# QWTforGithub/CDSegNet

Measured on AMD Instinct MI355X. Metric: points/sec/node (ScanNet ~120k-pt scenes, 1-step), higher is better.
Workload: dtype f16

## Files before the change

### cdsegnet_amd/_lib.py

```python
import ctypes
import os
import threading
from ctypes import POINTER, Structure, c_char_p, c_float, c_int, c_int32, c_int64, c_long, c_size_t, c_uint64, c_void_p

HERE = os.path.dirname(os.path.abspath(__file__))
LIB_PATH = os.path.join(HERE, "libcdseg_hip.so")
LIB_PATH_F16 = os.path.join(HERE, "libcdseg_hip_f16.so")

F32, BF16 = 0, 1
ACT_NONE, ACT_GELU, ACT_SWISH = 0, 1, 2
ORDER_IDS = {"z": 0, "z-trans": 1, "hilbert": 2, "hilbert-trans": 3}
ERRORS = {-1: "CDSEG_ERR_ARG", -2: "CDSEG_ERR_LAUNCH", -3: "CDSEG_ERR_WORKSPACE", -4: "CDSEG_ERR_UNSUPPORTED"}


class CdsegError(RuntimeError):
    pass


class DuplicateVoxelsError(CdsegError):

    def __init__(self, msg, count):
        super().__init__(msg)
        self.count = int(count)


class GemmArgs(Structure):
    _fields_ = [
        ("A", c_void_p), ("W", c_void_p), ("bias", c_void_p), ("scale", c_void_p), ("shift", c_void_p),
        ("res", c_void_p), ("add_src", c_void_p), ("add_idx", c_void_p), ("nbr", c_void_p), ("out_idx", c_void_p),
        ("out", c_void_p), ("out2", c_void_p),
        ("M", c_long),
        ("N", c_int), ("K", c_int), ("kvol", c_int),
        ("lda", c_int), ("ldo", c_int), ("ldo2", c_int), ("ldres", c_int), ("ldadd", c_int),
        ("a_dtype", c_int), ("compute_dtype", c_int), ("out_dtype", c_int), ("out2_dtype", c_int),
        ("act", c_int), ("out2_pre_add", c_int),
        ("ws", c_void_p), ("ws_bytes", c_size_t),
        ("colbias", c_void_p), ("ln_pre_g", c_void_p), ("ln_pre_b", c_void_p), ("ln_post_g", c_void_p),
        ("ln_post_b", c_void_p), ("ln_out", c_void_p), ("ldln", c_int), ("ln_out_dtype", c_int), ("ln_eps", c_float),
        ("nbr_kmajor", c_int),
    ]


class BlockDesc(Structure):
    _fields_ = [
        ("dtype", c_int), ("channels", c_int), ("heads", c_int), ("hidden", c_int),
        ("attn_scale", c_float), ("ln_eps", c_float),
        ("cpe_conv_w", c_void_p), ("cpe_conv_b", c_void_p), ("cpe_lin_w", c_void_p), ("cpe_lin_b", c_void_p),
        ("cpe_ln_g", c_void_p), ("cpe_ln_b", c_void_p), ("norm1_g", c_void_p), ("norm1_b", c_void_p),
        ("qkv_w", c_void_p), ("qkv_b", c_void_p), ("proj_w", c_void_p), ("proj_b", c_void_p),
        ("norm2_g", c_void_p), ("norm2_b", c_void_p), ("fc1_w", c_void_p), ("fc1_b", c_void_p),
        ("fc2_w", c_void_p), ("fc2_b", c_void_p), ("cpe_conv_wimg", c_void_p),
        ("head_img", c_void_p), ("tail_img", c_void_p),
        ("attn_flags", c_int),
    ]


class BlockIO(Structure):
    _fields_ = [
        ("n", c_long), ("x", c_void_p), ("xc_in", c_void_p), ("xc_out", c_void_p), ("tbias", c_void_p),
        ("nbr", c_void_p), ("gidx", c_void_p), ("widx", c_void_p), ("patch_start", c_void_p),
        ("num_patches", c_int), ("max_len", c_int), ("scratch", c_void_p), ("scratch_bytes", c_size_t),
        ("sat_counter", c_void_p),
    ]


class TrainBlockDesc(Structure):
    _fields_ = [
        ("channels", c_int), ("heads", c_int), ("hidden", c_int),
        ("attn_scale", c_float), ("eps_cpe", c_float), ("eps_norm1", c_float), ("eps_norm2", c_float),
        ("mm_dtype", c_int), ("attn_dtype", c_int), ("deterministic", c_int),
        ("param", c_void_p * 18), ("shadow16", c_void_p * 6),
        ("derived", c_void_p), ("derived_bytes", c_size_t),
    ]


class TrainBlockIO(Structure):
    _fields_ = [
        ("n", c_long), ("x_in", c_void_p), ("x_conv", c_void_p), ("t_rows", c_void_p), ("scene_offs", c_void_p),
        ("num_scenes", c_int), ("mask1", c_void_p), ("mask2", c_void_p),
        ("nbr", c_void_p), ("gidx", c_void_p), ("widx", c_void_p), ("patch_start", c_void_p),
        ("num_patches", c_int), ("max_len", c_int), ("num_slots", c_long),
        ("tape", c_void_p), ("tape_bytes", c_size_t), ("scratch", c_void_p), ("scratch_bytes", c_size_t),
        ("x_out", c_void_p),
        ("n_conv", c_long), ("row_vox", c_void_p), ("row_start", c_void_p),
    ]


class PlanSpec(Structure):
    _fields_ = [
        ("nlev", c_int), ("cum", c_int * 9), ("ncurve", c_int), ("curve_rows", c_int * 3),
        ("nslot_curve", c_int), ("slot_curve", c_int * 4),
        ("nlink", c_int), ("link_a", c_int * 16), ("link_b", c_int * 16),
        ("npad", c_int), ("pad_patch", c_int * 4), ("pad_flash", c_int * 4),
    ]


class PlanBeginIO(Structure):
    _fields_ = [
        ("grid", c_void_p), ("grid_elem_bytes", c_int), ("offset", c_void_p), ("nb", c_int), ("n", c_long),
        ("depth", c_int), ("end_bit", c_int), ("i32", c_void_p), ("i64", c_void_p), ("ws", c_void_p),
        ("ws_bytes", c_size_t), ("gmax_host", c_void_p), ("meta_host", c_void_p),
    ]


class PlanFinishIO(Structure):
    _fields_ = [
        ("n", c_long), ("nb", c_int), ("depth", c_int), ("m_host", POINTER(c_long)), ("offs_host", POINTER(c_int)),
        ("grid0", c_void_p), ("bat0", c_void_p), ("code0", c_void_p), ("cluster", c_void_p), ("seg", c_void_p),
        ("orders0", c_void_p), ("i32", c_void_p), ("i64", c_void_p), ("ws", c_void_p), ("ws_bytes", c_size_t),
        ("pads_host", c_void_p),
    ]


class OptTensor(Structure):
    _fields_ = [("p", c_void_p), ("g", c_void_p), ("m", c_void_p), ("v", c_void_p), ("p16", c_void_p), ("step", c_void_p),
                ("n", c_long), ("group", c_int), ("flags", c_int)]


class OptGroup(Structure):
    _fields_ = [("lr", ctypes.c_double), ("beta1", ctypes.c_double), ("beta2", ctypes.c_double), ("eps", ctypes.c_double),
                ("weight_decay", ctypes.c_double)]


OPT_CLIP, OPT_SKIP = 1, 2

SIGNATURES = {
    "cdseg_abi_version": (c_int, []),
    "cdseg_build_info": (c_char_p, []),
    "cdseg_grid_max": (c_int, [c_void_p, c_int, c_long, c_void_p, c_void_p]),
    "cdseg_offset2batch": (c_int, [c_void_p, c_int, c_long, c_void_p, c_void_p]),
    "cdseg_encode": (c_int, [c_void_p, c_int, c_void_p, c_int, c_long, c_int, c_int, c_void_p, c_void_p]),
    "cdseg_encode4": (c_int, [c_void_p, c_void_p, c_long, c_int, c_void_p, c_void_p]),
    "cdseg_sort_ws_bytes": (c_size_t, [c_long]),
    "cdseg_sort_pairs": (c_int, [c_void_p, c_void_p, c_void_p, c_void_p, c_long, c_int, c_void_p, c_size_t, c_void_p]),
    "cdseg_sort_curves_ws_bytes": (c_size_t, [c_long, c_int]),
    "cdseg_sort_curves": (c_int, [c_void_p, POINTER(c_int), c_int, c_long, c_int, c_void_p, c_void_p, c_size_t, c_void_p]),
    "cdseg_invert_perm": (c_int, [c_void_p, c_long, c_void_p, c_void_p]),
    "cdseg_widen_i32": (c_int, [c_void_p, c_long, c_void_p, c_void_p]),
    "cdseg_gather_rows": (c_int, [c_void_p, c_void_p, c_long, c_int, c_void_p, c_void_p]),
    "cdseg_scatter_rows": (c_int, [c_void_p, c_void_p, c_long, c_int, c_void_p, c_void_p]),
    "cdseg_gather_i32": (c_int, [c_void_p, c_void_p, c_long, c_void_p, c_void_p]),
    "cdseg_plan_gather_grid": (c_int, [c_void_p, c_int, c_void_p, c_void_p, c_long, c_int, c_void_p, c_void_p, c_void_p]),
    "cdseg_pool_level": (c_int, [c_void_p, c_long, c_int, c_void_p, c_void_p, c_void_p, c_void_p, c_size_t, c_void_p]),
    "cdseg_pool_gather": (c_int, [c_void_p, c_long, c_long, c_int, c_void_p, c_void_p, c_void_p, c_void_p, c_void_p,
                                  c_void_p, c_void_p]),
    "cdseg_pool_levels_ws_bytes": (c_size_t, [c_long, c_int]),
    "cdseg_pool_levels": (c_int, [c_void_p, c_long, POINTER(c_int), c_int, c_void_p, c_int, c_void_p, c_void_p, c_void_p,
                                  c_void_p, c_size_t, c_void_p]),
    "cdseg_link_derive": (c_int, [c_void_p, c_void_p, c_long, c_void_p, c_void_p, c_long, c_void_p, c_void_p, c_void_p]),
    "cdseg_coarse_orders_ws_bytes": (c_size_t, [c_long, c_int, c_int]),
    "cdseg_coarse_orders": (c_int, [POINTER(c_void_p), c_int, POINTER(c_void_p), c_int, c_long, c_void_p, c_void_p,
                                    c_size_t, c_void_p]),
    "cdseg_nbr_table": (c_int, [c_void_p, c_void_p, c_void_p, c_long, c_int, c_int, c_int, c_void_p, c_void_p]),
    "cdseg_nbr_table_from_parent": (c_int, [c_void_p, c_void_p, c_void_p, c_void_p, c_void_p, c_long, c_long, c_int, c_int,
                                            c_int, c_void_p, c_void_p]),
    "cdseg_nbr_table_from_info": (c_int, [c_void_p, c_void_p, c_void_p, c_void_p, c_long, c_long, c_int, c_int, c_int, c_void_p,
                                          c_void_p]),
    "cdseg_pad_plan": (c_int, [c_void_p, c_void_p, c_void_p, c_int, c_int, c_long, c_void_p, c_void_p, c_void_p]),
    "cdseg_pad_plan_batch": (c_int, [c_int, POINTER(c_void_p), POINTER(c_void_p), POINTER(c_void_p), POINTER(c_int),
                                     POINTER(c_long), c_int, c_void_p, c_void_p, c_void_p]),
    "cdseg_slots_select": (c_int, [POINTER(c_void_p), POINTER(c_void_p), c_int, c_void_p, c_int, c_char_p, c_long, c_void_p,
                                   c_void_p, c_void_p]),
    "cdseg_plan_begin_layout": (c_int, [POINTER(PlanSpec), c_long, c_int, POINTER(c_long), POINTER(c_long)]),
    "cdseg_plan_begin": (c_int, [POINTER(PlanSpec), POINTER(PlanBeginIO), c_int, c_void_p]),
    "cdseg_plan_finish_layout": (c_int, [POINTER(PlanSpec), c_long, c_int, POINTER(c_long), POINTER(c_int), POINTER(c_long),
                                         POINTER(c_long)]),
    "cdseg_plan_finish": (c_int, [POINTER(PlanSpec), POINTER(PlanFinishIO), c_void_p]),
    "cdseg_voxelize": (c_int, [c_void_p, ctypes.c_double, c_long, c_void_p, c_void_p, c_void_p, c_void_p]),
    "cdseg_voxelize_f64": (c_int, [c_void_p, ctypes.c_double, c_long, c_void_p, c_void_p, c_void_p, c_void_p]),
    "cdseg_center_shift": (c_int, [c_void_p, c_int, c_long, c_int, c_void_p, c_void_p, c_void_p]),
    "cdseg_tta_apply": (c_int, [c_void_p, c_long, POINTER(ctypes.c_double), ctypes.c_double, c_int, c_int, c_void_p, c_void_p]),
    "cdseg_div_add": (c_int, [c_void_p, c_float, c_float, c_long, c_void_p, c_void_p]),
    "cdseg_collect_feat": (c_int, [c_void_p, c_int, c_void_p, c_int, c_int, c_long, c_void_p, c_void_p]),
    "cdseg_max_run": (c_int, [c_void_p, c_long, c_void_p, c_void_p]),
    "cdseg_fragment_select": (c_int, [c_void_p, c_void_p, c_long, c_int, c_void_p, c_void_p]),
    "cdseg_softmax_vote": (c_int, [c_void_p, c_int, c_void_p, c_long, c_int, c_void_p, c_int, c_void_p]),
    "cdseg_argmax_rows": (c_int, [c_void_p, c_int, c_long, c_int, c_void_p, c_void_p]),
    "cdseg_fragments_build_ws_bytes": (c_size_t, [c_int]),
    "cdseg_fragments_build": (c_int, [c_void_p, c_void_p, c_long, c_int, c_long, c_void_p, c_void_p, c_int, c_void_p, c_int, c_int,
                                      c_void_p, c_void_p, c_void_p, c_void_p, c_void_p, c_size_t, c_void_p]),
    "cdseg_softmax_vote_fragments": (c_int, [c_void_p, c_int, c_void_p, c_long, c_int, c_int, c_void_p, c_int, c_long, c_void_p]),
    "cdseg_voxel_inverse": (c_int, [c_void_p, c_void_p, c_long, c_void_p, c_void_p]),
    "cdseg_tt_bbox": (c_int, [c_void_p, c_int, c_long, c_void_p, c_void_p]),
    "cdseg_tt_affine": (c_int, [c_void_p, c_int, c_long, c_int, POINTER(ctypes.c_double), c_void_p, POINTER(ctypes.c_double), c_int,
                                ctypes.c_double, c_int, c_int, c_int, c_void_p, c_int, c_void_p]),
    "cdseg_tt_jitter": (c_int, [c_void_p, c_void_p, c_int, ctypes.c_double, ctypes.c_double, c_long, c_void_p]),
    "cdseg_tt_blur3": (c_int, [c_void_p, c_int, c_int, c_int, c_int, c_void_p, c_void_p]),
    "cdseg_tt_elastic": (c_int, [c_void_p, c_long, c_void_p, POINTER(c_int), POINTER(ctypes.c_double), POINTER(ctypes.c_double),
                                 POINTER(ctypes.c_double), ctypes.c_double, c_void_p]),
    "cdseg_tt_color": (c_int, [c_void_p, c_long, c_void_p, ctypes.c_double, c_int, POINTER(ctypes.c_double), c_void_p, c_int,
                               ctypes.c_double, c_void_p]),
    "cdseg_tt_voxel_pick": (c_int, [c_void_p, c_void_p, c_long, c_void_p, c_void_p, c_void_p]),
    "cdseg_tt_dist_key": (c_int, [c_void_p, c_long, c_long, c_void_p, c_void_p]),
    "cdseg_rand_int": (c_int, [c_void_p, c_long, c_uint64, c_uint64, c_void_p, ctypes.c_uint32, c_void_p]),
    "cdseg_knn": (c_int, [c_void_p, c_void_p, c_long, c_void_p, c_void_p, c_long, c_int, c_int, POINTER(c_float), c_float,
                          c_void_p, c_void_p, c_void_p, c_size_t, c_void_p]),
    "cdseg_knn1_ws_bytes": (c_size_t, [c_long]),
    "cdseg_knn1": (c_int, [c_void_p, c_void_p, c_long, c_void_p, c_void_p, c_long, c_int, POINTER(c_float), c_float,
                           c_void_p, c_void_p, c_void_p, c_size_t, c_void_p]),
    "cdseg_iou_counts": (c_int, [c_void_p, c_void_p, c_void_p, c_long, c_int, c_int, c_void_p, c_void_p]),
    "cdseg_gemm": (c_int, [POINTER(GemmArgs), c_void_p]),
    "cdseg_gemm_ws_bytes": (c_size_t, [c_long, c_int, c_int, c_int]),
    "cdseg_mlp_fused": (c_int, [c_void_p, c_int, c_void_p, c_void_p, c_void_p, c_void_p, c_void_p, c_int, c_void_p, c_int,
                                c_long, c_int, c_int, c_void_p]),
    "cdseg_attn_tail_fused": (c_int, [c_void_p, c_int, c_void_p, c_void_p, c_void_p, c_void_p, c_float, c_void_p, c_void_p,
                                      c_void_p, c_void_p, c_void_p, c_int, c_void_p, c_int, c_long, c_int, c_int, c_void_p]),
    "cdseg_cpe_head_fused": (c_int, [c_void_p, c_int, c_void_p, c_void_p, c_void_p, c_void_p, c_void_p, c_int, c_void_p,
                                     c_void_p, c_void_p, c_float, c_void_p, c_void_p, c_void_p, c_int, c_long, c_int, c_int,
                                     c_int, c_void_p]),
    "cdseg_subm_conv3_wimg_bytes": (c_size_t, [c_int]),
    "cdseg_subm_conv3_pack": (c_int, [c_void_p, c_int, c_void_p, c_void_p]),
    "cdseg_subm_conv3": (c_int, [c_void_p, c_int, c_void_p, c_void_p, c_void_p, c_long, c_int, c_void_p, c_int, c_void_p]),
    "cdseg_child_info": (c_int, [c_void_p, c_void_p, c_long, c_void_p, c_void_p]),
    "cdseg_stem5_wimg_bytes": (c_size_t, []),
    "cdseg_stem5_pack": (c_int, [c_void_p, c_void_p, c_void_p]),
    "cdseg_stem5": (c_int, [c_void_p, c_void_p, c_void_p, c_void_p, c_void_p, c_void_p, c_void_p, c_void_p, c_long, c_long,
                            c_int, c_void_p, c_void_p, c_void_p]),
    "cdseg_block_rr_img_bytes": (c_size_t, [c_int, c_int]),
    "cdseg_block_rr_pack": (c_int, [c_int, c_void_p, c_void_p, c_void_p, c_void_p, c_void_p, c_void_p, c_void_p, c_void_p]),
    "cdseg_cpe_head_rr": (c_int, [c_void_p, c_int, c_void_p, c_void_p, c_void_p, c_void_p, c_void_p, c_int, c_void_p, c_void_p,
                                  c_void_p, c_float, c_void_p, c_void_p, c_int, c_long, c_int, c_int, c_void_p]),
    "cdseg_attn_tail_rr": (c_int, [c_void_p, c_int, c_void_p, c_void_p, c_void_p, c_void_p, c_float, c_void_p, c_void_p,
                                   c_void_p, c_int, c_void_p, c_int, c_long, c_int, c_void_p]),
    "cdseg_cpe_head_rr2": (c_int, [c_void_p, c_int, c_void_p, c_void_p, c_void_p, c_void_p, c_void_p, c_int, c_void_p, c_int,
                                   c_void_p, c_void_p, c_void_p, c_float, c_void_p, c_void_p, c_int, c_long, c_int, c_int, c_void_p]),
    "cdseg_attn_tail_rr2": (c_int, [c_void_p, c_int, c_void_p, c_void_p, c_void_p, c_void_p, c_float, c_void_p, c_void_p,
                                    c_void_p, c_int, c_void_p, c_int, c_void_p, c_int, c_long, c_int, c_void_p, c_size_t, c_void_p]),
    "cdseg_block_scratch_bytes": (c_size_t, [POINTER(BlockDesc), c_long]),
    "cdseg_block_forward": (c_int, [POINTER(BlockDesc), POINTER(BlockIO), c_void_p]),
    "cdseg_layernorm": (c_int, [c_void_p, c_int, c_int, c_void_p, c_void_p, c_float, c_void_p, c_int, c_void_p,
                                c_void_p, c_int, c_int, c_void_p, c_int, c_int, c_long, c_int, c_void_p]),
    "cdseg_attention": (c_int, [c_void_p, c_void_p, c_void_p, c_int, c_int, c_int, c_void_p, c_void_p, c_void_p,
                                c_void_p, c_int, c_int, c_int, c_float, c_void_p, c_int, c_int, c_void_p]),
    "cdseg_attention_ex": (c_int, [c_void_p, c_void_p, c_void_p, c_int, c_int, c_int, c_void_p, c_void_p, c_void_p,
                                   c_void_p, c_int, c_int, c_int, c_float, c_void_p, c_int, c_int, c_int, c_void_p]),
    "cdseg_attention_schedule": (c_long, [c_int, c_int, c_int, c_int, c_void_p, c_long]),
    "cdseg_attention_bwd_ws_bytes": (c_size_t, [c_long, c_int]),
    "cdseg_attention_bwd": (c_int, [c_void_p, c_void_p, c_void_p, c_int, c_int, c_int, c_void_p, c_void_p, c_void_p, c_void_p,
                                    c_int, c_int, c_long, c_int, c_float, c_void_p, c_int, c_void_p, c_void_p, c_void_p,
                                    c_int, c_int, c_int, c_int, c_void_p, c_size_t, c_void_p]),
    "cdseg_attention_drop": (c_int, [c_void_p, c_void_p, c_void_p, c_int, c_int, c_int, c_void_p, c_void_p, c_void_p, c_void_p,
                                     c_int, c_int, c_int, c_float, c_void_p, c_int, c_int, ctypes.c_double, c_uint64, c_uint64,
                                     c_void_p]),
    "cdseg_attention_drop_bwd": (c_int, [c_void_p, c_void_p, c_void_p, c_int, c_int, c_int, c_void_p, c_void_p, c_void_p, c_void_p,
                                         c_int, c_int, c_long, c_int, c_float, c_void_p, c_int, c_void_p, c_void_p, c_void_p,
                                         c_int, c_int, c_int, c_int, c_void_p, c_size_t, ctypes.c_double, c_uint64, c_uint64,
                                         c_void_p]),
    "cdseg_dropout": (c_int, [c_void_p, c_int, c_void_p, c_int, c_long, c_int, ctypes.c_double, c_uint64, c_uint64, c_void_p]),
    "cdseg_layernorm_bwd": (c_int, [c_void_p, c_int, c_void_p, c_float, c_void_p, c_int, c_void_p, c_int, c_int, c_void_p,
                                    c_void_p, c_long, c_int, c_void_p]),
    "cdseg_gelu_bwd": (c_int, [c_void_p, c_void_p, c_void_p, c_long, c_void_p]),
    "cdseg_conv_wgrad": (c_int, [c_void_p, c_int, c_void_p, c_int, c_void_p, c_int, c_long, c_int, c_int, c_void_p, c_void_p,
                                 c_void_p]),
    "cdseg_linear_wgrad": (c_int, [c_void_p, c_int, c_void_p, c_void_p, c_int, c_long, c_int, c_int, c_void_p, c_int, c_void_p,
                                   c_void_p]),
    "cdseg_conv_wgrad16": (c_int, [c_void_p, c_int, c_void_p, c_int, c_void_p, c_int, c_long, c_int, c_int, c_void_p, c_void_p,
                                   c_void_p]),
    "cdseg_linear_wgrad16": (c_int, [c_void_p, c_int, c_void_p, c_void_p, c_int, c_long, c_int, c_int, c_void_p, c_int, c_void_p,
                                     c_void_p]),
    "cdseg_wgrad_partition": (c_int, [c_long, c_int, c_int, c_int, c_int, POINTER(c_long), POINTER(c_int)]),
    "cdseg_wgrad_det_ws_bytes": (c_size_t, [c_long, c_int, c_int, c_int, c_int]),
    "cdseg_linear_wgrad_det": (c_int, [c_void_p, c_int, c_void_p, c_void_p, c_int, c_long, c_int, c_int, c_void_p, c_int, c_void_p,
                                       c_int, c_void_p, c_size_t, c_void_p]),
    "cdseg_conv_wgrad_det": (c_int, [c_void_p, c_int, c_void_p, c_int, c_void_p, c_int, c_long, c_int, c_int, c_void_p, c_void_p,
                                     c_int, c_void_p, c_size_t, c_void_p]),
    "cdseg_layernorm_bwd_det_ws_bytes": (c_size_t, [c_long, c_int]),
    "cdseg_layernorm_bwd_det": (c_int, [c_void_p, c_int, c_void_p, c_float, c_void_p, c_int, c_void_p, c_int, c_int, c_void_p,
                                        c_void_p, c_long, c_int, c_void_p, c_size_t, c_void_p]),
    "cdseg_segment_sum": (c_int, [c_void_p, c_int, c_void_p, c_long, c_int, c_void_p, c_int, c_void_p]),
    "cdseg_seg_loss_ws_bytes": (c_size_t, [c_long, c_int]),
    "cdseg_seg_loss_fwd": (c_int, [c_void_p, c_int, c_void_p, c_long, c_int, c_long, c_int, c_void_p, POINTER(c_int32), c_void_p,
                                   c_void_p, c_void_p, c_size_t, c_void_p]),
    "cdseg_seg_loss_bwd": (c_int, [c_void_p, c_int, c_void_p, c_long, c_int, c_long, POINTER(c_int32), c_void_p, c_void_p,
                                   c_void_p, c_void_p, c_int, c_void_p]),
    "cdseg_bn_partition": (c_int, [c_long, c_int, POINTER(c_long), POINTER(c_int)]),
    "cdseg_bn_ws_bytes": (c_size_t, [c_long, c_int]),
    "cdseg_bn_stats": (c_int, [c_void_p, c_int, c_long, c_int, c_void_p, c_void_p, c_size_t, c_void_p]),
    "cdseg_bn_finish": (c_int, [c_void_p, c_int, ctypes.c_double, ctypes.c_double, c_void_p, c_void_p, c_void_p, c_void_p,
                                c_void_p]),
    "cdseg_bn_gelu_fwd": (c_int, [c_void_p, c_int, c_long, c_int, c_void_p, c_void_p, c_void_p, c_void_p, c_void_p, c_int,
                                  c_void_p]),
    "cdseg_bn_gelu_bwd_sums": (c_int, [c_void_p, c_int, c_void_p, c_int, c_long, c_int, c_void_p, c_void_p, c_void_p, c_void_p,
                                       c_void_p, c_void_p, c_size_t, c_void_p]),
    "cdseg_bn_gelu_bwd_dx": (c_int, [c_void_p, c_int, c_void_p, c_int, c_long, c_int, c_void_p, c_void_p, c_void_p, c_void_p,
                                     c_void_p, c_void_p, c_void_p, c_int, c_void_p]),
    "cdseg_segment_max_arg": (c_int, [c_void_p, c_int, c_void_p, c_long, c_int, c_void_p, c_int, c_void_p, c_int, c_void_p]),
    "cdseg_segment_max_bwd": (c_int, [c_void_p, c_int, c_void_p, c_int, c_void_p, c_long, c_int, c_void_p, c_int, c_void_p]),
    "cdseg_fuse_gate_ws_bytes": (c_size_t, [c_long, c_int]),
    "cdseg_fuse_gate_fwd": (c_int, [c_void_p, c_void_p, c_void_p, c_void_p, c_void_p, c_void_p, c_long, c_int, c_void_p]),
    "cdseg_fuse_gate_bwd": (c_int, [c_void_p, c_void_p, c_void_p, c_void_p, c_void_p, c_void_p, c_void_p, c_void_p, c_void_p,
                                    c_long, c_int, c_void_p, c_size_t, c_void_p]),
    "cdseg_skip_partition": (c_int, [c_long, c_int, POINTER(c_long), POINTER(c_int)]),
    "cdseg_skip_stats_ws_bytes": (c_size_t, [c_long, c_int]),
    "cdseg_skip_stats": (c_int, [c_void_p, c_int, c_int, c_long, c_int, c_void_p, c_long, c_void_p, c_void_p, c_size_t, c_void_p]),
    "cdseg_skip_fold": (c_int, [c_void_p, c_int, c_int, c_int, c_int, c_void_p, c_void_p, c_void_p]),
    "cdseg_skip_merge": (c_int, [c_void_p, c_int, c_long, c_int, c_void_p, c_int, ctypes.c_double, c_long, ctypes.c_double,
                                 c_void_p, c_void_p, c_int, c_void_p, c_long, c_void_p]),
    "cdseg_opt_chunks": (c_int, [POINTER(c_long), c_int, POINTER(c_int32), POINTER(c_long)]),
    "cdseg_opt_ws_bytes": (c_size_t, [c_int, c_long]),
    "cdseg_grad_norm": (c_int, [POINTER(OptTensor), c_int, c_void_p, c_long, c_void_p, c_float, c_void_p, c_void_p, c_size_t,
                                c_void_p]),
    "cdseg_adamw_step": (c_int, [POINTER(OptTensor), c_int, POINTER(OptGroup), c_int, c_void_p, c_long, c_void_p, c_void_p,
                                 c_void_p, c_void_p, c_size_t, c_void_p]),
    "cdseg_route_enable": (c_int, [c_int]),
    "cdseg_route_clear": (None, []),
    "cdseg_route_read": (c_int, [POINTER(c_int32), c_int]),
    "cdseg_route_catalog": (c_int, [ctypes.c_char_p, c_size_t]),
    "cdseg_route_note": (c_int, [POINTER(c_int32)]),
    "cdseg_prof_enable": (c_int, [c_int]),
    "cdseg_prof_summary": (c_int, [POINTER(ctypes.c_double), POINTER(c_long)]),
    "cdseg_prof_summary_class": (c_int, [c_int, POINTER(ctypes.c_double), POINTER(c_long)]),
    "cdseg_segment_max": (c_int, [c_void_p, c_int, c_int, c_void_p, c_long, c_int, c_void_p, c_void_p, c_int,
                                  c_void_p, c_int, c_void_p, c_int, c_int, c_void_p]),
    "cdseg_segment_mean": (c_int, [c_void_p, c_int, c_void_p, c_long, c_int, c_void_p, c_int, c_void_p]),
    "cdseg_pool_fused_fold": (c_int, [c_int]),
    "cdseg_pool_fused_n": (c_int, [c_void_p, c_int, c_long, c_void_p, c_void_p, c_void_p, c_long, c_void_p, c_void_p, c_int, c_void_p,
                                   c_int, c_void_p, c_int, c_int, c_int, c_void_p]),
    "cdseg_unpool_fused_img_bytes": (c_size_t, [c_int, c_int]),
    "cdseg_unpool_fused_pack": (c_int, [c_void_p, c_int, c_int, c_void_p, c_void_p]),
    "cdseg_unpool_fused": (c_int, [c_void_p, c_int, c_void_p, c_void_p, c_void_p, c_void_p, c_void_p, c_int, c_void_p, c_void_p,
                                   c_void_p, c_void_p, c_void_p, c_long, c_int, c_void_p, c_int, c_void_p, c_int, c_int, c_int,
                                   c_int, c_void_p]),
    "cdseg_pool_fused_img_bytes": (c_size_t, [c_int, c_int]),
    "cdseg_pool_fused_pack": (c_int, [c_void_p, c_int, c_int, c_void_p, c_void_p]),
    "cdseg_pool_fused": (c_int, [c_void_p, c_int, c_void_p, c_void_p, c_void_p, c_long, c_void_p, c_void_p, c_int, c_void_p, c_int,
                                 c_void_p, c_int, c_int, c_int, c_void_p]),
    "cdseg_gemv": (c_int, [c_void_p, c_void_p, c_void_p, c_int, c_int, c_int, c_void_p, c_void_p]),
    "cdseg_randn": (c_int, [c_void_p, c_long, c_uint64, c_uint64, c_void_p]),
    "cdseg_cast": (c_int, [c_void_p, c_int, c_void_p, c_int, c_long, c_void_p]),
    "cdseg_gather_pad_cast": (c_int, [c_void_p, c_int, c_void_p, c_long, c_int, c_int, c_void_p, c_int, c_void_p]),
    "cdseg_ddim_update": (c_int, [c_void_p, c_void_p, c_float, c_float, c_float, c_float, c_int, c_void_p, c_long,
                                  c_void_p]),
    "cdseg_axpy": (c_int, [c_void_p, c_void_p, c_float, c_void_p, c_long, c_void_p]),
    "cdseg_msi_step": (c_int, [c_void_p, c_void_p, c_long, c_float, c_float, c_float, c_float, c_int, c_void_p, c_void_p, c_long,
                               c_int, c_float, c_void_p]),
    "cdseg_count_saturated": (c_int, [c_void_p, c_long, c_int, c_int, c_void_p, c_void_p]),
    "cdseg_subm_conv3_f32": (c_int, [c_void_p, c_int, c_void_p, c_void_p, c_void_p, c_long, c_int, c_void_p, c_int, c_float, c_int,
                                     c_void_p]),
    "cdseg_split16": (c_int, [c_void_p, c_int, c_long, c_int, c_void_p, c_void_p, c_int, c_float, c_void_p]),
    "cdseg_train_block_bytes": (c_int, [POINTER(TrainBlockDesc), c_long, c_long, POINTER(c_size_t), POINTER(c_size_t),
                                        POINTER(c_size_t), POINTER(c_size_t)]),
    "cdseg_train_block_grad_offsets": (c_int, [POINTER(TrainBlockDesc), POINTER(c_size_t)]),
    "cdseg_train_block_prepare": (c_int, [POINTER(TrainBlockDesc), c_void_p]),
    "cdseg_train_block_forward": (c_int, [POINTER(TrainBlockDesc), POINTER(TrainBlockIO), c_void_p]),
    "cdseg_train_block_backward": (c_int, [POINTER(TrainBlockDesc), POINTER(TrainBlockIO), c_void_p, c_void_p, c_void_p, c_void_p,
                                           c_void_p, c_void_p]),
    "cdseg_residual": (c_int, [c_void_p, c_void_p, c_void_p, c_void_p, c_void_p, c_int, c_void_p, c_long, c_int, c_void_p]),
    "cdseg_gather_first": (c_int, [c_void_p, c_void_p, c_void_p, c_int, c_long, c_int, c_void_p]),
    "cdseg_residual_rows": (c_int, [c_void_p, c_void_p, c_void_p, c_void_p, c_void_p, c_int, c_void_p, c_long, c_int, c_void_p]),
    "cdseg_run_sum": (c_int, [c_void_p, c_void_p, c_void_p, c_long, c_int, c_void_p]),
    "cdseg_scatter_first": (c_int, [c_void_p, c_void_p, c_void_p, c_void_p, c_int, c_long, c_int, c_void_p]),
    "cdseg_scale_cast": (c_int, [c_void_p, c_void_p, c_void_p, c_int, c_long, c_int, c_void_p]),
    "cdseg_add_layernorm": (c_int, [c_void_p, c_void_p, c_void_p, c_void_p, c_void_p, c_float, c_void_p, c_void_p, c_int, c_long,
                                    c_int, c_void_p]),
    "cdseg_gelu_fwd": (c_int, [c_void_p, c_void_p, c_int, c_long, c_void_p]),
    "cdseg_gelu_bwd_cast": (c_int, [c_void_p, c_void_p, c_void_p, c_int, c_long, c_void_p]),
}

_libs = {}
_tls = threading.local()
VARIANTS = ("bf16", "f16")


def active():
    return getattr(_tls, "variant", "bf16")


class use:

    def __init__(self, variant):
        if variant not in VARIANTS:
            raise ValueError(variant)
        self.variant = variant

    def __enter__(self):
        self.prev = active()
# ... 37 lines not shown
```

### cdsegnet_amd/build.py

```python
import os
import subprocess
import sys

HERE = os.path.dirname(os.path.abspath(__file__))
CSRC = os.path.join(HERE, "csrc")
LIB = os.path.join(HERE, "libcdseg_hip.so")
LIB_F16 = os.path.join(HERE, "libcdseg_hip_f16.so")
VARIANTS = [(LIB, "_build", []), (LIB_F16, "_build_f16", ["-DCDSEG_LP_F16"])]
SOURCES = ["serialize.hip", "plan.hip", "gemm.hip", "elementwise.hip", "attention.hip", "attention_drop.hip", "conv.hip", "stem.hip", "mlp.hip", "blockrr.hip", "deep.hip", "pool.hip", "runtime.hip", "testtime.hip", "traintime.hip", "train.hip", "trainblock.hip", "loss.hip", "norm.hip", "fusion.hip", "skip.hip", "optim.hip", "prof.hip", "route.hip", "abi.hip"]
HEADERS = ["common.h", "curves.h", "prof.h", "route.h", "deep.h", "wgrad_partition.h", "workspace.h", "attn_train.h", os.path.join("..", "..", "include", "cdseg.h")]
ARCH = "gfx950"


def _stale():
    deps = [os.path.join(CSRC, f) for f in SOURCES + HEADERS] + [os.path.abspath(__file__)]
    for lib, _, _ in VARIANTS:
        if not os.path.exists(lib):
            return True
        t = os.path.getmtime(lib)
        if any(os.path.getmtime(d) > t for d in deps):
            return True
    return False


def build_library(force=False, verbose=True):
    if not force and not _stale():
        return LIB
    hipcc = os.environ.get("HIPCC", "/opt/rocm/bin/hipcc")
    procs, links = [], []
    for lib, bdir, defs in VARIANTS:
        build_dir = os.path.join(HERE, "csrc", bdir)
        os.makedirs(build_dir, exist_ok=True)
        objs = []
        for src in SOURCES:
            obj = os.path.join(build_dir, src.replace(".hip", ".o"))
            objs.append(obj)
            cmd = [hipcc, f"--offload-arch={ARCH}", "-O3", "-std=c++20", "-fPIC"] + defs + ["-c", os.path.join(CSRC, src), "-o", obj]
            if verbose:
                print(" ".join(cmd), flush=True)
            procs.append((src, subprocess.Popen(cmd, stdout=subprocess.PIPE, stderr=subprocess.STDOUT, text=True)))
        links.append([hipcc, f"--offload-arch={ARCH}", "-shared", "-fPIC", "-o", lib] + objs)
    for src, p in procs:
        out, _ = p.communicate()
        if p.returncode != 0:
            sys.stderr.write(out)
            raise RuntimeError(f"hipcc failed on {src}")
    for cmd in links:
        if verbose:
            print(" ".join(cmd), flush=True)
        subprocess.check_call(cmd)
    return LIB


if __name__ == "__main__":
    print(build_library(force="--force" in sys.argv))
```

### cdsegnet_amd/csrc/blockrr.hip

```cpp
#include <cstdlib>

#include <atomic>

#include "common.h"
#include "deep.h"
#include "route.h"

namespace {

constexpr int RR_WAVES = 8;

enum { OUT_P = 0, OUT_NAT = 1 };
enum { IN_P = 0, IN_HID = 1 };

struct PackP {
  const bf16_t* w;
  uint4* img;
  int nout, k, out_mode, in_mode;
};

__global__ void rr_pack_kernel(PackP p) {
  const int KS = p.k / 32;
  const int u = blockIdx.x * blockDim.x + threadIdx.x;
  if (u >= (p.nout / 16) * KS * 64) return;
  const int lane = u & 63, s = (u >> 6) % KS, ot = (u >> 6) / KS;
  const int q = lane >> 4, i = lane & 15;
  const int row = p.out_mode == OUT_P ? (i >> 2) * (p.nout / 4) + ot * 4 + (i & 3) : 16 * ot + i;
  union { uint4 v; bf16_t h[8]; } o;
#pragma unroll
  for (int e = 0; e < 8; ++e) {
    const int col = p.in_mode == IN_P ? q * (p.k / 4) + 8 * s + e : 32 * s + (e < 4 ? 4 * q + e : 16 + 4 * q + (e - 4));
    o.h[e] = p.w[(long)row * p.k + col];
  }
  p.img[u] = o.v;
}

template <int C>
struct RRCfg {
  static constexpr int KS = C / 32, CT = C / 16, Q = C / 4;
  static constexpr int HEAD_W = 4 * C * C * 2, HEAD_P = 9 * C * 4;
  static constexpr int TAIL_W = 9 * C * C * 2, TAIL_P = 8 * C * 4;
};

__device__ __forceinline__ bf16x8_t pack8(const f32x4_t& a, const f32x4_t& b) {
  union { bf16x8_t v; uint32_t u[4]; } r;
  r.u[0] = pack_bf16x2(a[0], a[1]); r.u[1] = pack_bf16x2(a[2], a[3]);
  r.u[2] = pack_bf16x2(b[0], b[1]); r.u[3] = pack_bf16x2(b[2], b[3]);
  return r.v;
}

template <int CT>
__device__ __forceinline__ void ln_stats(const f32x4_t (&v)[CT], float inv_c, float eps, float& mean, float& rstd) {
  float s = 0.f;
#pragma unroll
  for (int t = 0; t < CT; ++t) s += (v[t][0] + v[t][1]) + (v[t][2] + v[t][3]);
  s += __shfl_xor(s, 16, 64);
  s += __shfl_xor(s, 32, 64);
  mean = s * inv_c;
  float q = 0.f;
#pragma unroll
  for (int t = 0; t < CT; ++t) {
    const float a = v[t][0] - mean, b = v[t][1] - mean, c = v[t][2] - mean, d = v[t][3] - mean;
    q += (a * a + b * b) + (c * c + d * d);
  }
  q += __shfl_xor(q, 16, 64);
  q += __shfl_xor(q, 32, 64);
  rstd = 1.0f / sqrtf(q * inv_c + eps);
}

struct HeadRR {
  const bf16_t* y; const uint4* wimg; const float* bl; const float* lnp_g; const float* lnp_b; float* x;
  const float* colbias; const float* ln1_g; const float* ln1_b; const float* bqkv; bf16_t* qkv;
  long n; int ldy, ldx, ldqkv; float eps;
};

template <int C>
__global__ __launch_bounds__(RR_WAVES * 64, 4) void head_rr_kernel(HeadRR p) {
  using K = RRCfg<C>;
  constexpr int KS = K::KS, CT = K::CT, Q = K::Q, OT = 3 * C / 16, QQ = 3 * C / 4;
  extern __shared__ __attribute__((aligned(16))) char smem[];
  const int tid = threadIdx.x, lane0 = tid & 63;
  const int wave = __builtin_amdgcn_readfirstlane(tid >> 6);
  const int j = lane0 & 15, q = lane0 >> 4;
  {
    uint4* d = reinterpret_cast<uint4*>(smem);
    for (int u = tid; u < K::HEAD_W / 16; u += RR_WAVES * 64) d[u] = p.wimg[u];
    float* pr = reinterpret_cast<float*>(smem + K::HEAD_W);
    for (int c = tid; c < C; c += RR_WAVES * 64) {
      pr[c] = p.bl[c]; pr[C + c] = p.lnp_g[c]; pr[2 * C + c] = p.lnp_b[c]; pr[3 * C + c] = p.colbias ? p.colbias[c] : 0.f;
      pr[4 * C + c] = p.ln1_g[c]; pr[5 * C + c] = p.ln1_b[c];
    }
    for (int c = tid; c < 3 * C; c += RR_WAVES * 64) pr[6 * C + c] = p.bqkv[c];
  }
  __syncthreads();
  const uint4* Wl = reinterpret_cast<const uint4*>(smem);
  const uint4* Wq = reinterpret_cast<const uint4*>(smem + C * C * 2);
  const float* pr = reinterpret_cast<const float*>(smem + K::HEAD_W);
  const float inv_c = 1.0f / C;

  const long tiles = (p.n + 31) / 32;
  for (long tile = (long)blockIdx.x * RR_WAVES + wave; tile < tiles; tile += (long)gridDim.x * RR_WAVES) {
#pragma unroll 1
    for (int g = 0; g < 2; ++g) {
      const long row = tile * 32 + g * 16 + j;
      const bool ok = row < p.n;
      const long rr = ok ? row : p.n - 1;
      int lane = lane0;
      asm volatile("" : "+v"(lane));
      bf16x8_t yf[KS];
#pragma unroll
      for (int s = 0; s < KS; ++s) yf[s] = *reinterpret_cast<const bf16x8_t*>(p.y + rr * p.ldy + q * Q + 8 * s);
      f32x4_t xr[CT];
#pragma unroll
      for (int t = 0; t < CT; ++t) xr[t] = *reinterpret_cast<const f32x4_t*>(p.x + rr * p.ldx + q * Q + 4 * t);
      f32x4_t v[CT];
      {
        uint4 wl[CT][KS];
#pragma unroll
        for (int t = 0; t < CT; ++t)
#pragma unroll
          for (int s = 0; s < KS; ++s) wl[t][s] = Wl[(t * KS + s) * 64 + lane];
#pragma unroll
        for (int t = 0; t < CT; ++t) {
          v[t] = *reinterpret_cast<const f32x4_t*>(pr + q * Q + 4 * t);
#pragma unroll
          for (int s = 0; s < KS; ++s)
            v[t] = mfma_16x16x32_bf16(__builtin_bit_cast(bf16x8_t, wl[t][s]), yf[s], v[t]);
        }
      }
      float mean, rstd;
      ln_stats<CT>(v, inv_c, p.eps, mean, rstd);
#pragma unroll
      for (int t = 0; t < CT; ++t) {
        const f32x4_t ga = *reinterpret_cast<const f32x4_t*>(pr + C + q * Q + 4 * t);
        const f32x4_t be = *reinterpret_cast<const f32x4_t*>(pr + 2 * C + q * Q + 4 * t);
        const f32x4_t tb = *reinterpret_cast<const f32x4_t*>(pr + 3 * C + q * Q + 4 * t);
#pragma unroll
        for (int r = 0; r < 4; ++r) v[t][r] = ((v[t][r] - mean) * rstd * ga[r] + be[r]) + xr[t][r] + tb[r];
        if (ok) *reinterpret_cast<f32x4_t*>(p.x + row * p.ldx + q * Q + 4 * t) = v[t];
      }
      ln_stats<CT>(v, inv_c, p.eps, mean, rstd);
#pragma unroll
      for (int t = 0; t < CT; ++t) {
        const f32x4_t ga = *reinterpret_cast<const f32x4_t*>(pr + 4 * C + q * Q + 4 * t);
        const f32x4_t be = *reinterpret_cast<const f32x4_t*>(pr + 5 * C + q * Q + 4 * t);
#pragma unroll
        for (int r = 0; r < 4; ++r) v[t][r] = (v[t][r] - mean) * rstd * ga[r] + be[r];
      }
      bf16x8_t hf[KS];
#pragma unroll
      for (int s = 0; s < KS; ++s) hf[s] = pack8(v[2 * s], v[2 * s + 1]);
      uint4 wq[2][2][KS];
#pragma unroll
      for (int s = 0; s < KS; ++s) {
        wq[0][0][s] = Wq[(0 * KS + s) * 64 + lane];
        wq[0][1][s] = Wq[(1 * KS + s) * 64 + lane];
      }
#pragma unroll
      for (int ot = 0; ot < OT; ot += 2) {
        const int cur = (ot >> 1) & 1;
        if (ot + 2 < OT) {
#pragma unroll
          for (int s = 0; s < KS; ++s) {
            wq[cur ^ 1][0][s] = Wq[((ot + 2) * KS + s) * 64 + lane];
            wq[cur ^ 1][1][s] = Wq[((ot + 3) * KS + s) * 64 + lane];
          }
        }
        f32x4_t a0 = *reinterpret_cast<const f32x4_t*>(pr + 6 * C + q * QQ + 4 * ot);
        f32x4_t a1 = *reinterpret_cast<const f32x4_t*>(pr + 6 * C + q * QQ + 4 * ot + 4);
#pragma unroll
        for (int s = 0; s < KS; ++s) {
          a0 = mfma_16x16x32_bf16(__builtin_bit_cast(bf16x8_t, wq[cur][0][s]), hf[s], a0);
          a1 = mfma_16x16x32_bf16(__builtin_bit_cast(bf16x8_t, wq[cur][1][s]), hf[s], a1);
        }
        if (ok) *reinterpret_cast<bf16x8_t*>(p.qkv + row * p.ldqkv + q * QQ + 4 * ot) = pack8(a0, a1);
      }
    }
  }
}

struct TailRR {
  const bf16_t* o; const uint4* wimg; const float* bp; const float* ln_g; const float* ln_b; const float* b1;
  const float* b2; float* x; bf16_t* xc;
  long n; int ldo, ldx, ldxc; float eps;
};

template <int C>
__global__ __launch_bounds__(RR_WAVES * 64, 4) void tail_rr_kernel(TailRR p) {
  using K = RRCfg<C>;
  constexpr int KS = K::KS, CT = K::CT, Q = K::Q, HU = 4 * C / 32;
  extern __shared__ __attribute__((aligned(16))) char smem[];
  const int tid = threadIdx.x, lane0 = tid & 63;
  const int wave = __builtin_amdgcn_readfirstlane(tid >> 6);
  const int j = lane0 & 15, q = lane0 >> 4;
  {
    uint4* d = reinterpret_cast<uint4*>(smem);
    for (int u = tid; u < K::TAIL_W / 16; u += RR_WAVES * 64) d[u] = p.wimg[u];
    float* pr = reinterpret_cast<float*>(smem + K::TAIL_W);
    for (int c = tid; c < C; c += RR_WAVES * 64) {
      pr[c] = p.bp[c]; pr[C + c] = p.ln_g[c]; pr[2 * C + c] = p.ln_b[c]; pr[3 * C + c] = p.b2[c];
    }
    for (int c = tid; c < 4 * C; c += RR_WAVES * 64) pr[4 * C + c] = p.b1[c];
  }
  __syncthreads();
  const uint4* Wp = reinterpret_cast<const uint4*>(smem);
  const uint4* W1 = reinterpret_cast<const uint4*>(smem + C * C * 2);
  const uint4* W2 = reinterpret_cast<const uint4*>(smem + 5 * C * C * 2);
  const float* pr = reinterpret_cast<const float*>(smem + K::TAIL_W);
  const float inv_c = 1.0f / C;

  const long tiles = (p.n + 31) / 32;
  for (long tile = (long)blockIdx.x * RR_WAVES + wave; tile < tiles; tile += (long)gridDim.x * RR_WAVES) {
#pragma unroll 1
    for (int g = 0; g < 2; ++g) {
      const long row = tile * 32 + g * 16 + j;
      const bool ok = row < p.n;
      const long rr = ok ? row : p.n - 1;
      int lane = lane0;
      asm volatile("" : "+v"(lane));
      bf16x8_t of[KS];
#pragma unroll
      for (int s = 0; s < KS; ++s) of[s] = *reinterpret_cast<const bf16x8_t*>(p.o + rr * p.ldo + q * Q + 8 * s);
      f32x4_t x1[CT];
      {
        uint4 wp[CT][KS];
#pragma unroll
        for (int t = 0; t < CT; ++t)
#pragma unroll
          for (int s = 0; s < KS; ++s) wp[t][s] = Wp[(t * KS + s) * 64 + lane];
#pragma unroll
        for (int t = 0; t < CT; ++t) {
          f32x4_t a = *reinterpret_cast<const f32x4_t*>(pr + q * Q + 4 * t);
#pragma unroll
          for (int s = 0; s < KS; ++s)
            a = mfma_16x16x32_bf16(__builtin_bit_cast(bf16x8_t, wp[t][s]), of[s], a);
          const f32x4_t r = *reinterpret_cast<const f32x4_t*>(p.x + rr * p.ldx + q * Q + 4 * t);
          x1[t] = a + r;
        }
      }
      float mean, rstd;
      ln_stats<CT>(x1, inv_c, p.eps, mean, rstd);
      bf16x8_t hf[KS];
      {
        f32x4_t h[CT];
#pragma unroll
        for (int t = 0; t < CT; ++t) {
          const f32x4_t ga = *reinterpret_cast<const f32x4_t*>(pr + C + q * Q + 4 * t);
          const f32x4_t be = *reinterpret_cast<const f32x4_t*>(pr + 2 * C + q * Q + 4 * t);
#pragma unroll
          for (int r = 0; r < 4; ++r) h[t][r] = (x1[t][r] - mean) * rstd * ga[r] + be[r];
        }
#pragma unroll
        for (int s = 0; s < KS; ++s) hf[s] = pack8(h[2 * s], h[2 * s + 1]);
      }
      f32x4_t acc2[CT];
#pragma unroll
      for (int t = 0; t < CT; ++t) acc2[t] = f32x4_t{0.f, 0.f, 0.f, 0.f};
#pragma unroll 1
      for (int u = 0; u < HU; ++u) {
        uint4 w1[2][KS], w2[CT];
#pragma unroll
        for (int s = 0; s < KS; ++s) {
          w1[0][s] = W1[((2 * u) * KS + s) * 64 + lane];
          w1[1][s] = W1[((2 * u + 1) * KS + s) * 64 + lane];
        }
#pragma unroll
        for (int t = 0; t < CT; ++t) w2[t] = W2[(t * HU + u) * 64 + lane];
        f32x4_t h0 = *reinterpret_cast<const f32x4_t*>(pr + 4 * C + 32 * u + 4 * q);
        f32x4_t h1 = *reinterpret_cast<const f32x4_t*>(pr + 4 * C + 32 * u + 16 + 4 * q);
#pragma unroll
        for (int s = 0; s < KS; ++s) {
          h0 = mfma_16x16x32_bf16(__builtin_bit_cast(bf16x8_t, w1[0][s]), hf[s], h0);
          h1 = mfma_16x16x32_bf16(__builtin_bit_cast(bf16x8_t, w1[1][s]), hf[s], h1);
        }
        gelu_lp4(h0);
        gelu_lp4(h1);
        const bf16x8_t Hf = pack8(h0, h1);
#pragma unroll
        for (int t = 0; t < CT; ++t)
          acc2[t] = mfma_16x16x32_bf16(__builtin_bit_cast(bf16x8_t, w2[t]), Hf, acc2[t]);
      }
      if (ok) {
#pragma unroll
        for (int t = 0; t < CT; ++t) {
          const f32x4_t b2 = *reinterpret_cast<const f32x4_t*>(pr + 3 * C + q * Q + 4 * t);
          acc2[t] = acc2[t] + (b2 + x1[t]);
          *reinterpret_cast<f32x4_t*>(p.x + row * p.ldx + q * Q + 4 * t) = acc2[t];
        }
        if (p.xc) {
#pragma unroll
          for (int t = 0; t < CT; t += 2)
            *reinterpret_cast<bf16x8_t*>(p.xc + row * p.ldxc + q * Q + 4 * t) = pack8(acc2[t], acc2[t + 1]);
        }
      }
    }
  }
}

int pack_one(const void* w, int nout, int k, int out_mode, int in_mode, void* img, hipStream_t s) {
  PackP p;
  p.w = (const bf16_t*)w; p.img = (uint4*)img; p.nout = nout; p.k = k; p.out_mode = out_mode; p.in_mode = in_mode;
  const int units = (nout / 16) * (k / 32) * 64;
  hipLaunchKernelGGL(rr_pack_kernel, dim3((units + 255) / 256), dim3(256), 0, s, p);
  return hipGetLastError() == hipSuccess ? CDSEG_OK : CDSEG_ERR_LAUNCH;
}

int rr_grid(long n, int lds_bytes) {
  const long tiles = (n + 31) / 32;
  const int per_cu = lds_bytes > 80 * 1024 ? 1 : (lds_bytes > 40 * 1024 ? 2 : 3);
  long blocks = (tiles + RR_WAVES - 1) / RR_WAVES;
  if (blocks > 256 * per_cu) blocks = 256 * per_cu;
  return (int)blocks;
}

}

extern "C" size_t cdseg_block_rr_img_bytes(int channels, int which) {
  if (channels != 32 && channels != 64 && !deep_supported(channels)) return 0;
  return (size_t)(which == 0 ? 4 : 9) * channels * channels * 2;
}

extern "C" int cdseg_block_rr_pack(int channels, const void* wl, const void* wqkv, void* head_img, const void* wp,
                                   const void* w1, const void* w2, void* tail_img, void* stream) {
  if (deep_supported(channels)) return deep_pack(channels, wl, wqkv, head_img, wp, w1, w2, tail_img, (hipStream_t)stream);
  if (channels != 32 && channels != 64) return CDSEG_ERR_UNSUPPORTED;
  const int C = channels;
  hipStream_t s = (hipStream_t)stream;
  int rc;
  if (head_img) {
    if (!wl || !wqkv) return CDSEG_ERR_ARG;
    if ((rc = pack_one(wl, C, C, OUT_P, IN_P, head_img, s)) != CDSEG_OK) return rc;
    if ((rc = pack_one(wqkv, 3 * C, C, OUT_P, IN_P, (char*)head_img + C * C * 2, s)) != CDSEG_OK) return rc;
  }
  if (tail_img) {
    if (!wp || !w1 || !w2) return CDSEG_ERR_ARG;
    if ((rc = pack_one(wp, C, C, OUT_P, IN_P, tail_img, s)) != CDSEG_OK) return rc;
    if ((rc = pack_one(w1, 4 * C, C, OUT_NAT, IN_P, (char*)tail_img + C * C * 2, s)) != CDSEG_OK) return rc;
    if ((rc = pack_one(w2, C, 4 * C, OUT_P, IN_HID, (char*)tail_img + 5 * C * C * 2, s)) != CDSEG_OK) return rc;
  }
  return CDSEG_OK;
}

extern "C" int cdseg_cpe_head_rr(const void* y, int ldy, const void* head_img, const float* bl, const float* lnp_g,
                                 const float* lnp_b, float* x, int ldx, const float* colbias, const float* ln1_g,
                                 const float* ln1_b, float eps, const float* bqkv, void* qkv, int ldqkv, long n,
                                 int channels, int qkv_flags, void* stream) {
  if (n <= 0) return CDSEG_OK;
  if (qkv_flags & ~CDSEG_ATTN_V_BF16) return CDSEG_ERR_ARG;
  if (qkv_flags && !deep_supported(channels)) return CDSEG_ERR_UNSUPPORTED;
  if (!y || !head_img || !bl || !lnp_g || !lnp_b || !x || !ln1_g || !ln1_b || !bqkv || !qkv) return CDSEG_ERR_ARG;
  if (channels != 32 && channels != 64 && !deep_supported(channels)) return CDSEG_ERR_UNSUPPORTED;
  if ((ldy & 7) || (ldx & 3) || (ldqkv & 7) || (((uintptr_t)y | (uintptr_t)x | (uintptr_t)qkv | (uintptr_t)head_img) & 15))
    return CDSEG_ERR_ARG;
  if (deep_supported(channels))
    return deep_head(y, ldy, head_img, bl, lnp_g, lnp_b, x, ldx, x, ldx, colbias, ln1_g, ln1_b, eps, bqkv, qkv, ldqkv, n,
                     channels, qkv_flags, (hipStream_t)stream);
  HeadRR p;
  p.y = (const bf16_t*)y; p.wimg = (const uint4*)head_img; p.bl = bl; p.lnp_g = lnp_g; p.lnp_b = lnp_b; p.x = x;
  p.colbias = colbias; p.ln1_g = ln1_g; p.ln1_b = ln1_b; p.bqkv = bqkv; p.qkv = (bf16_t*)qkv;
  p.n = n; p.ldy = ldy; p.ldx = ldx; p.ldqkv = ldqkv; p.eps = eps;
  hipStream_t s = (hipStream_t)stream;
  if (channels == 32) {
    constexpr int lds = RRCfg<32>::HEAD_W + RRCfg<32>::HEAD_P;
    cdseg_route_rec(CDSEG_RK_HEAD_RR_32, 0, 0, 1, 0, 0, 0, 0);
    hipLaunchKernelGGL(head_rr_kernel<32>, dim3(rr_grid(n, lds)), dim3(RR_WAVES * 64), lds, s, p);
  } else {
    constexpr int lds = RRCfg<64>::HEAD_W + RRCfg<64>::HEAD_P;
    cdseg_route_rec(CDSEG_RK_HEAD_RR_64, 0, 0, 1, 0, 0, 0, 0);
    hipLaunchKernelGGL(head_rr_kernel<64>, dim3(rr_grid(n, lds)), dim3(RR_WAVES * 64), lds, s, p);
  }
  CDSEG_CHECK_LAUNCH();
  return CDSEG_OK;
}

extern "C" int cdseg_attn_tail_rr(const void* o, int ldo, const void* tail_img, const float* bp, const float* ln_g,
                                  const float* ln_b, float eps, const float* b1, const float* b2, float* x, int ldx,
                                  void* xc, int ldxc, long n, int channels, void* stream) {
  if (n <= 0) return CDSEG_OK;
  if (!o || !tail_img || !bp || !ln_g || !ln_b || !b1 || !b2 || !x) return CDSEG_ERR_ARG;
  if (channels != 32 && channels != 64 && !deep_supported(channels)) return CDSEG_ERR_UNSUPPORTED;
  if ((ldo & 7) || (ldx & 3) || (xc && (ldxc & 7)) || (((uintptr_t)o | (uintptr_t)x | (uintptr_t)xc | (uintptr_t)tail_img) & 15))
    return CDSEG_ERR_ARG;
  if (deep_supported(channels))
    return deep_tail(o, ldo, tail_img, bp, ln_g, ln_b, eps, b1, b2, x, ldx, x, ldx, xc, ldxc, n, channels, nullptr, 0,
                     (hipStream_t)stream);
  TailRR p;
  p.o = (const bf16_t*)o; p.wimg = (const uint4*)tail_img; p.bp = bp; p.ln_g = ln_g; p.ln_b = ln_b; p.b1 = b1; p.b2 = b2;
  p.x = x; p.xc = (bf16_t*)xc; p.n = n; p.ldo = ldo; p.ldx = ldx; p.ldxc = ldxc; p.eps = eps;
  hipStream_t s = (hipStream_t)stream;
  if (channels == 32) {
    constexpr int lds = RRCfg<32>::TAIL_W + RRCfg<32>::TAIL_P;
    cdseg_route_rec(CDSEG_RK_TAIL_RR_32, 0, 0, 1, 0, 0, 0, 0);
    hipLaunchKernelGGL(tail_rr_kernel<32>, dim3(rr_grid(n, lds)), dim3(RR_WAVES * 64), lds, s, p);
  } else {
    constexpr int lds = RRCfg<64>::TAIL_W + RRCfg<64>::TAIL_P;
    static std::atomic<bool> attr_done{false};
    if (!attr_done) {
      if (hipFuncSetAttribute((const void*)tail_rr_kernel<64>, hipFuncAttributeMaxDynamicSharedMemorySize, lds) != hipSuccess)
        return CDSEG_ERR_LAUNCH;
      attr_done = true;
    }
    cdseg_route_rec(CDSEG_RK_TAIL_RR_64, 0, 0, 1, 0, 0, 0, 0);
    hipLaunchKernelGGL(tail_rr_kernel<64>, dim3(rr_grid(n, lds)), dim3(RR_WAVES * 64), lds, s, p);
  }
  CDSEG_CHECK_LAUNCH();
  return CDSEG_OK;
}

extern "C" int cdseg_cpe_head_rr2(const void* y, int ldy, const void* head_img, const float* bl, const float* lnp_g,
                                  const float* lnp_b, const float* x, int ldx, float* x_out, int ldx_out, const float* colbias,
                                  const float* ln1_g, const float* ln1_b, float eps, const float* bqkv, void* qkv, int ldqkv,
                                  long n, int channels, int qkv_flags, void* stream) {
  if (n <= 0) return CDSEG_OK;
  if (qkv_flags & ~CDSEG_ATTN_V_BF16) return CDSEG_ERR_ARG;
  if (!deep_supported(channels)) return CDSEG_ERR_UNSUPPORTED;
  if (!y || !head_img || !bl || !lnp_g || !lnp_b || !x || !x_out || !ln1_g || !ln1_b || !bqkv || !qkv) return CDSEG_ERR_ARG;
  if ((ldy & 7) || (ldx & 3) || (ldx_out & 3) || (ldqkv & 7) ||
      (((uintptr_t)y | (uintptr_t)x | (uintptr_t)x_out | (uintptr_t)qkv | (uintptr_t)head_img) & 15))
    return CDSEG_ERR_ARG;
  return deep_head(y, ldy, head_img, bl, lnp_g, lnp_b, x, ldx, x_out, ldx_out, colbias, ln1_g, ln1_b, eps, bqkv, qkv, ldqkv, n,
                   channels, qkv_flags, (hipStream_t)stream);
}

extern "C" int cdseg_attn_tail_rr2(const void* o, int ldo, const void* tail_img, const float* bp, const float* ln_g,
                                   const float* ln_b, float eps, const float* b1, const float* b2, const float* x_in, int ldx_in,
                                   float* x, int ldx, void* xc, int ldxc, long n, int channels, void* ws, size_t ws_bytes,
                                   void* stream) {
  if (n <= 0) return CDSEG_OK;
  if (!deep_supported(channels)) return CDSEG_ERR_UNSUPPORTED;
  if (!o || !tail_img || !bp || !ln_g || !ln_b || !b1 || !b2 || !x || !x_in) return CDSEG_ERR_ARG;
  if ((ldo & 7) || (ldx & 3) || (ldx_in & 3) || (xc && (ldxc & 7)) ||
      (((uintptr_t)o | (uintptr_t)x | (uintptr_t)x_in | (uintptr_t)xc | (uintptr_t)tail_img) & 15))
    return CDSEG_ERR_ARG;
  return deep_tail(o, ldo, tail_img, bp, ln_g, ln_b, eps, b1, b2, x_in, ldx_in, x, ldx, xc, ldxc, n, channels, ws, ws_bytes,
                   (hipStream_t)stream);
}
```

### cdsegnet_amd/csrc/runtime.hip

```cpp
#include <algorithm>
#include <cstdlib>
#include <cstring>

#include "common.h"
#include "deep.h"
#include "workspace.h"

namespace {

constexpr int FUSE_LN_MAX_C = 512;

inline int storage_dtype(int dtype) { return dtype == CDSEG_F32X3 ? CDSEG_F32 : dtype; }

struct Layout {
  void *y, *h, *qkv, *o, *u, *y2, *ws, *xs;
  size_t ws_bytes, total;
};

Layout carve(const cdseg_block_desc* d, long n, void* scratch) {
  Carver c{(char*)scratch, 0};
  const size_t e = esz(d->dtype);
  const size_t C = d->channels;
  Layout L;
  L.y = c.take(n * C * e);
  L.h = c.take(n * C * e);
  L.qkv = c.take(n * 3 * C * e);
  L.o = c.take(n * C * e);
  L.u = c.take(n * (size_t)d->hidden * e);
  L.y2 = d->channels > FUSE_LN_MAX_C ? c.take(n * C * 4) : nullptr;
  const long wide = std::max<long>(3 * C, d->hidden);
  L.ws_bytes = std::min(GEMM_WS_CAP, std::max(gemm_ws_rule(n, C, wide, false, true), gemm_ws_rule(n, C, C, true, false)));
  L.ws = L.ws_bytes ? c.take(L.ws_bytes) : nullptr;
  L.xs = (d->dtype == CDSEG_BF16 && C >= 128 && d->head_img && d->tail_img) ? c.take(n * C * 4) : nullptr;
  L.total = align_up(c.off, 256);
  return L;
}

cdseg_gemm_args base_args(const cdseg_block_desc* d, const Layout& L, long n) {
  cdseg_gemm_args a;
  std::memset(&a, 0, sizeof(a));
  a.M = n;
  a.kvol = 1;
  a.a_dtype = storage_dtype(d->dtype);
  a.compute_dtype = d->dtype;
  a.ws = L.ws;
  a.ws_bytes = L.ws_bytes;
  a.ln_eps = d->ln_eps;
  return a;
}

}

extern "C" size_t cdseg_block_scratch_bytes(const cdseg_block_desc* d, long n) {
  if (!d || n <= 0) return 0;
  return carve(d, n, nullptr).total;
}

static int block_forward_impl(const cdseg_block_desc* d, const cdseg_block_io* io, void* stream);

extern "C" int cdseg_block_forward(const cdseg_block_desc* d, const cdseg_block_io* io, void* stream) {
  const int rc = block_forward_impl(d, io, stream);
  if (rc != CDSEG_OK || !io->sat_counter || io->n <= 0 || d->dtype != CDSEG_BF16) return rc;
  const Layout L = carve(d, io->n, io->scratch);
  const int C = d->channels;
  int r;
  if ((r = cdseg_count_saturated(L.y, io->n, C, C, io->sat_counter, stream)) != CDSEG_OK) return r;
  if ((r = cdseg_count_saturated(L.qkv, io->n, 2 * C, 3 * C, io->sat_counter, stream)) != CDSEG_OK) return r;
  if ((r = cdseg_count_saturated(L.o, io->n, C, C, io->sat_counter, stream)) != CDSEG_OK) return r;
  if ((const void*)io->xc_out != (const void*)io->x)
    if ((r = cdseg_count_saturated(io->xc_out, io->n, C, C, io->sat_counter, stream)) != CDSEG_OK) return r;
  return CDSEG_OK;
}

static int block_forward_impl(const cdseg_block_desc* d, const cdseg_block_io* io, void* stream) {
  if (!d || !io || !io->x || !io->xc_in || !io->xc_out || !io->nbr || !io->gidx || !io->widx || !io->patch_start)
    return CDSEG_ERR_ARG;
  const long n = io->n;
  if (n <= 0) return CDSEG_OK;
  const int C = d->channels, T = storage_dtype(d->dtype);
  if (C != d->heads * CDSEG_HEAD_DIM) return CDSEG_ERR_UNSUPPORTED;
  const Layout L = carve(d, n, io->scratch);
  if (!io->scratch || io->scratch_bytes < L.total) return CDSEG_ERR_WORKSPACE;
  const bool fuse = C <= FUSE_LN_MAX_C;
  int rc;
  int attn_flags = d->attn_flags & CDSEG_ATTN_Q_PRESCALED;

  const bool conv_fits = n * 27 * 4 < (1l << 31) && n * (long)C * 2 < (1l << 31) - 65536;
  const bool deep_head_next = cdseg_knob("CDSEG_DEEP_FUSED", 1) != 0 && T == CDSEG_BF16 && (C == 128 || C == 256) &&
                              d->hidden == 4 * C && d->head_img;
  int ysplits = 1;
  const float* ypart = nullptr;
  if (d->cpe_conv_wimg && T == CDSEG_BF16 && (C == 32 || C == 64) && conv_fits) {
    rc = cdseg_subm_conv3(io->xc_in, C, d->cpe_conv_wimg, (const float*)d->cpe_conv_b, io->nbr, n, C, L.y, C, stream);
    if (rc != CDSEG_OK) return rc;
  } else {
    cdseg_gemm_args a = base_args(d, L, n);
    a.A = io->xc_in; a.lda = C; a.W = d->cpe_conv_w; a.bias = d->cpe_conv_b; a.nbr = io->nbr; a.nbr_kmajor = 1; a.kvol = 27;
    a.N = C; a.K = C; a.out = L.y; a.ldo = C; a.out_dtype = T;
    static const bool partials_on = cdseg_knob("CDSEG_CONV_PARTIALS", 1) != 0;
    if (partials_on && deep_head_next && (C == 128 || C == 256) && !io->sat_counter && a.ws && a.bias) {
      if ((rc = gemm_leave_partials(&a, &ysplits, stream)) != CDSEG_OK) return rc;
      if (ysplits > 1) ypart = (const float*)a.ws;
    } else if ((rc = cdseg_gemm(&a, stream)) != CDSEG_OK) {
      return rc;
    }
  }
  static const bool fused_head = cdseg_knob("CDSEG_FUSED_HEAD", 1) != 0;
  static const bool deep_on = cdseg_knob("CDSEG_DEEP_FUSED", 1) != 0;
  static const long deep512_min = cdseg_knob("CDSEG_DEEP512_MIN_ROWS", CDSEG_DEEP512_MIN_ROWS);
  static const bool deep512_split = cdseg_knob("CDSEG_DEEP_SPLIT", 1) != 0;
  const bool deep = deep_on && T == CDSEG_BF16 &&
                    (C == 128 || C == 256 || (C == 512 && (n >= deep512_min || (deep512_split && L.xs)))) && d->hidden == 4 * C;
  const bool head = (fused_head && T == CDSEG_BF16 && (C == 32 || C == 64)) || (deep && d->head_img);
  const bool pingpong = deep && d->head_img && d->tail_img && L.xs;
  if (ypart) {
    float* xo = pingpong ? (float*)L.xs : (float*)io->x;
    if ((rc = deep_head(L.y, C, d->head_img, (const float*)d->cpe_lin_b, (const float*)d->cpe_ln_g, (const float*)d->cpe_ln_b,
                        (const float*)io->x, C, xo, C, (const float*)io->tbias, (const float*)d->norm1_g,
                        (const float*)d->norm1_b, d->ln_eps, (const float*)d->qkv_b, L.qkv, 3 * C, n, C, CDSEG_ATTN_V_BF16,
                        (hipStream_t)stream, ypart, ysplits, (const float*)d->cpe_conv_b)) != CDSEG_OK)
      return rc;
    attn_flags |= CDSEG_ATTN_V_BF16;
  } else if (pingpong) {
    if ((rc = cdseg_cpe_head_rr2(L.y, C, d->head_img, (const float*)d->cpe_lin_b, (const float*)d->cpe_ln_g,
                                 (const float*)d->cpe_ln_b, (const float*)io->x, C, (float*)L.xs, C, (const float*)io->tbias,
                                 (const float*)d->norm1_g, (const float*)d->norm1_b, d->ln_eps, (const float*)d->qkv_b, L.qkv,
                                 3 * C, n, C, CDSEG_ATTN_V_BF16, stream)) != CDSEG_OK)
      return rc;
    attn_flags |= CDSEG_ATTN_V_BF16;
  } else if (head && d->head_img) {
    if ((rc = cdseg_cpe_head_rr(L.y, C, d->head_img, (const float*)d->cpe_lin_b, (const float*)d->cpe_ln_g,
                                (const float*)d->cpe_ln_b, (float*)io->x, C, (const float*)io->tbias,
                                (const float*)d->norm1_g, (const float*)d->norm1_b, d->ln_eps, (const float*)d->qkv_b, L.qkv,
                                3 * C, n, C, deep ? CDSEG_ATTN_V_BF16 : 0, stream)) != CDSEG_OK)
      return rc;
    if (deep) attn_flags |= CDSEG_ATTN_V_BF16;
  } else if (head) {
    if ((rc = cdseg_cpe_head_fused(L.y, C, d->cpe_lin_w, (const float*)d->cpe_lin_b, (const float*)d->cpe_ln_g,
                                   (const float*)d->cpe_ln_b, (float*)io->x, C, (const float*)io->tbias,
                                   (const float*)d->norm1_g, (const float*)d->norm1_b, d->ln_eps, d->qkv_w,
                                   (const float*)d->qkv_b, L.qkv, 3 * C, n, C, T, CDSEG_ATTN_V_BF16, stream)) != CDSEG_OK)
      return rc;
    attn_flags |= CDSEG_ATTN_V_BF16;
  } else if (fuse) {
    cdseg_gemm_args a = base_args(d, L, n);
    a.A = L.y; a.lda = C; a.W = d->cpe_lin_w; a.bias = d->cpe_lin_b; a.N = C; a.K = C;
    a.ln_pre_g = d->cpe_ln_g; a.ln_pre_b = d->cpe_ln_b; a.res = io->x; a.ldres = C; a.colbias = io->tbias;
    a.out = io->x; a.ldo = C; a.out_dtype = CDSEG_F32;
    a.ln_post_g = d->norm1_g; a.ln_post_b = d->norm1_b; a.ln_out = L.h; a.ldln = C; a.ln_out_dtype = T;
    if ((rc = cdseg_gemm(&a, stream)) != CDSEG_OK) return rc;
  } else {
    cdseg_gemm_args a = base_args(d, L, n);
    a.A = L.y; a.lda = C; a.W = d->cpe_lin_w; a.bias = d->cpe_lin_b; a.N = C; a.K = C;
    a.out = L.y2; a.ldo = C; a.out_dtype = CDSEG_F32;
    if ((rc = cdseg_gemm(&a, stream)) != CDSEG_OK) return rc;
    if ((rc = cdseg_layernorm(L.y2, CDSEG_F32, C, d->cpe_ln_g, d->cpe_ln_b, d->ln_eps, io->x, C, io->tbias, io->x,
                              CDSEG_F32, C, nullptr, 0, 0, n, C, stream)) != CDSEG_OK)
      return rc;
    if ((rc = cdseg_layernorm(io->x, CDSEG_F32, C, d->norm1_g, d->norm1_b, d->ln_eps, nullptr, 0, nullptr, L.h, T, C,
                              nullptr, 0, 0, n, C, stream)) != CDSEG_OK)
      return rc;
  }
  if (!head) {
    cdseg_gemm_args a = base_args(d, L, n);
    a.A = L.h; a.lda = C; a.W = d->qkv_w; a.bias = d->qkv_b; a.N = 3 * C; a.K = C;
    a.out = L.qkv; a.ldo = 3 * C; a.out_dtype = T;
    if ((rc = cdseg_gemm(&a, stream)) != CDSEG_OK) return rc;
  }
  {
    const size_t e = esz(T);
    const char* q = (const char*)L.qkv;
    if ((rc = cdseg_attention_ex(q, q + (size_t)C * e, q + (size_t)2 * C * e, 3 * C, 3 * C, 3 * C, io->gidx, io->gidx,
                                 io->widx, io->patch_start, io->num_patches, d->heads, io->max_len, d->attn_scale, L.o, C,
                                 d->dtype, attn_flags, stream)) != CDSEG_OK)
      return rc;
  }
  static const bool fused_tail = cdseg_knob("CDSEG_FUSED_TAIL", 1) != 0 && cdseg_knob("CDSEG_FUSED_MLP", 1) != 0;
  if (pingpong) {
    void* xc = (const void*)io->xc_out != (const void*)io->x ? io->xc_out : nullptr;
    return cdseg_attn_tail_rr2(L.o, C, d->tail_img, (const float*)d->proj_b, (const float*)d->norm2_g, (const float*)d->norm2_b,
                               d->ln_eps, (const float*)d->fc1_b, (const float*)d->fc2_b, (const float*)L.xs, C, (float*)io->x,
                               C, xc, C, n, C, L.ws, L.ws_bytes, stream);
  }
  if (deep && d->tail_img) {
    void* xc = (const void*)io->xc_out != (const void*)io->x ? io->xc_out : nullptr;
    return cdseg_attn_tail_rr(L.o, C, d->tail_img, (const float*)d->proj_b, (const float*)d->norm2_g, (const float*)d->norm2_b,
                              d->ln_eps, (const float*)d->fc1_b, (const float*)d->fc2_b, (float*)io->x, C, xc, C, n, C, stream);
  }
  if (fused_tail && T == CDSEG_BF16 && (C == 32 || C == 64) && d->hidden == 4 * C) {
    void* xc = (const void*)io->xc_out != (const void*)io->x ? io->xc_out : nullptr;
    if (d->tail_img)
      return cdseg_attn_tail_rr(L.o, C, d->tail_img, (const float*)d->proj_b, (const float*)d->norm2_g,
                                (const float*)d->norm2_b, d->ln_eps, (const float*)d->fc1_b, (const float*)d->fc2_b,
                                (float*)io->x, C, xc, C, n, C, stream);
    return cdseg_attn_tail_fused(L.o, C, d->proj_w, (const float*)d->proj_b, (const float*)d->norm2_g,
                                 (const float*)d->norm2_b, d->ln_eps, d->fc1_w, (const float*)d->fc1_b, d->fc2_w,
                                 (const float*)d->fc2_b, (float*)io->x, C, xc, C, n, C, T, stream);
  }
  {
    cdseg_gemm_args a = base_args(d, L, n);
    a.A = L.o; a.lda = C; a.W = d->proj_w; a.bias = d->proj_b; a.N = C; a.K = C;
    a.res = io->x; a.ldres = C; a.out = io->x; a.ldo = C; a.out_dtype = CDSEG_F32;
    if (fuse) {
      a.ln_post_g = d->norm2_g; a.ln_post_b = d->norm2_b; a.ln_out = L.h; a.ldln = C; a.ln_out_dtype = T;
    }
    if ((rc = cdseg_gemm(&a, stream)) != CDSEG_OK) return rc;
    if (!fuse &&
        (rc = cdseg_layernorm(io->x, CDSEG_F32, C, d->norm2_g, d->norm2_b, d->ln_eps, nullptr, 0, nullptr, L.h, T, C,
                              nullptr, 0, 0, n, C, stream)) != CDSEG_OK)
      return rc;
  }
  static const bool fused_mlp = cdseg_knob("CDSEG_FUSED_MLP", 1) != 0;
  static const int fused_maxc = cdseg_knob("CDSEG_FUSED_MLP_MAXC", 128);
  if (fused_mlp && T == CDSEG_BF16 && (C == 32 || C == 64 || C == 128) && C <= fused_maxc && d->hidden == 4 * C) {
    void* xc = (const void*)io->xc_out != (const void*)io->x ? io->xc_out : nullptr;
    if ((rc = cdseg_mlp_fused(L.h, C, d->fc1_w, (const float*)d->fc1_b, d->fc2_w, (const float*)d->fc2_b, (float*)io->x, C,
                              xc, C, n, C, T, stream)) != CDSEG_OK)
      return rc;
    return CDSEG_OK;
  }
  {
    cdseg_gemm_args a = base_args(d, L, n);
    a.A = L.h; a.lda = C; a.W = d->fc1_w; a.bias = d->fc1_b; a.N = d->hidden; a.K = C; a.act = CDSEG_ACT_GELU;
    a.out = L.u; a.ldo = d->hidden; a.out_dtype = T;
    if ((rc = cdseg_gemm(&a, stream)) != CDSEG_OK) return rc;
  }
  {
    cdseg_gemm_args a = base_args(d, L, n);
    a.A = L.u; a.lda = d->hidden; a.W = d->fc2_w; a.bias = d->fc2_b; a.N = C; a.K = d->hidden;
    a.res = io->x; a.ldres = C; a.out = io->x; a.ldo = C; a.out_dtype = CDSEG_F32;
    if ((const void*)io->xc_out != (const void*)io->x) {
      a.out2 = io->xc_out; a.ldo2 = C; a.out2_dtype = T;
    }
    if ((rc = cdseg_gemm(&a, stream)) != CDSEG_OK) return rc;
  }
  return CDSEG_OK;
}
```

### cdsegnet_amd/engine.py

```python
import math
import struct
import os
import threading

import numpy as np
import torch

from . import _lib, ops
from ._lib import CdsegError, DuplicateVoxelsError
from .models import fusion_gate

CURVES = ("z", "z-trans", "hilbert", "hilbert-trans")
POOL_LONG_MIN_ROWS = 960_000


def _pooling_depth(stride):
    return (math.ceil(stride) - 1).bit_length()


class _ShareEvents(threading.local):
    on = False


SHARE_EVENTS = _ShareEvents()


def _shared(cache, key, build, force=False):
    ent = cache.get(key)
    cur = ops.current_stream_id()
    if ent is None:
        val = build()
        ent = cache[key] = (val, cur, ops.record_event() if (cur is not None and (SHARE_EVENTS.on or force)) else None)
    elif ent[1] != cur and ent[2] is not None:
        ops.wait_event(ent[2])
    return ent[0]


def _cut(lazy, cache, key):
    lz = lazy.pop(key, None)
    if lz is not None:
        sid, parts = lz
        vals = tuple(A[o:o + c] if shape is None else A[o:o + c].view(shape) for A, o, c, shape in parts)
        cache[key] = (vals[0] if len(vals) == 1 else vals, sid, None)


FUSED_CURVE_SORT = True

class Level:

    def __init__(self, cum, depth, n, grid, batch, code4, offs_host, lazy=None):
        self.cum, self.depth, self.n = cum, depth, n
        self._gbc = (grid, batch, code4) if lazy is None else None
        self._gbc_lazy = lazy
        self.offs_host = offs_host
        self.parent = None
        self.shared = False
        self._order = {}
        self._nbr = {}
        self._pad = {}
        self._slots = {}
        self._pad_lazy = {}
        self._slot_lazy = {}
        self._order_lazy = {}
        self._nbr_lazy = {}

    def _cut_gbc(self):
        A, go, bo, Q, co = self._gbc_lazy
        n = self.n
        self._gbc = (A[go:go + 3 * n].view(n, 3), A[bo:bo + n], Q[co:co + 4 * n].view(4, n))
        self._gbc_lazy = None
        return self._gbc

    @property
    def grid(self):
        return (self._gbc or self._cut_gbc())[0]

    @property
    def batch(self):
        return (self._gbc or self._cut_gbc())[1]

    @property
    def code4(self):
        return (self._gbc or self._cut_gbc())[2]

    def order(self, curve):
        if curve == 0:
            return None
        if self._order_lazy:
            _cut(self._order_lazy, self._order, curve)

        def build():
            nb = len(self.offs_host) - 1
            end_bit = min(64, 3 * self.depth + max(1, nb.bit_length()))
            return ops.sort_pairs(self.code4[curve], None, end_bit=end_bit)[1]
        return _shared(self._order, curve, build, self.shared)

    def ref_of_row(self, curve):
        order = self.order(curve)
        if order is None:
            return None
        return _shared(self._order, ("inverse", curve), lambda: ops.invert_perm(order), self.shared)

    def nbr(self, ksize, kmajor=False):
        if self._nbr_lazy:
            _cut(self._nbr_lazy, self._nbr, (ksize, kmajor))

        def build():
            if self.parent is not None:
                par, (cluster, seg) = self.parent
                return ops.nbr_table_from_info(self.grid, cluster, par.nbr(3, True), self.child_info(), par.n, self.depth,
                                               ksize, kmajor)
            return ops.nbr_table(self.code4[0], self.grid, self.batch, self.depth, ksize, kmajor)
        return _shared(self._nbr, (ksize, kmajor), build, self.shared)

    def child_info(self):
        if self._nbr_lazy:
            _cut(self._nbr_lazy, self._nbr, "child_info")

        def build():
            par, (_, seg) = self.parent
            return ops.child_info(self.code4[0], seg, par.n)
        return _shared(self._nbr, "child_info", build, self.shared)

    def pad_host_py(self, patch_size, enable_flash):
        offs = self.offs_host
        counts = [b - a for a, b in zip(offs[:-1], offs[1:])]
        K = int(patch_size) if enable_flash else int(min(min(counts), patch_size))
        offs_pad, patch_start = [0], []
        for c in counts:
            pc = (c + K - 1) // K * K if c > K else c
            patch_start.extend(range(offs_pad[-1], offs_pad[-1] + pc, K))
            offs_pad.append(offs_pad[-1] + pc)
        patch_start.append(offs_pad[-1])
        return K, offs, offs_pad, patch_start

    def pad_host(self, patch_size, enable_flash):
        K, offs, offs_pad, patch_start = self.pad_host_py(patch_size, enable_flash)
        return (K, np.asarray(offs, dtype=np.int32), np.asarray(offs_pad, dtype=np.int32),
                np.asarray(patch_start, dtype=np.int32))

    def set_pad(self, key, K, offs_pad, patch_start, offs_dev, offs_pad_dev, patch_start_dev):
        lens = [int(b) - int(a) for a, b in zip(patch_start[:-1], patch_start[1:])]
        self._pad[key] = (K, int(offs_pad[-1]), offs_dev, offs_pad_dev, patch_start_dev,
                          max(lens), float(sum(v * v for v in lens)))

    def pad(self, patch_size, enable_flash):
        key = (patch_size, enable_flash)
        lz = self._pad_lazy.pop(key, None) if self._pad_lazy else None
        if lz is not None:
            K, n_pad, max_len, sum_l2, A, oo, op, ot, nb, npatch = lz
            self._pad[key] = (K, n_pad, A[oo:oo + nb + 1], A[op:op + nb + 1], A[ot:ot + npatch + 1], max_len, sum_l2)
        if key not in self._pad:
            K, offs, offs_pad, patch_start = self.pad_host(patch_size, enable_flash)
            dev = self.grid.device
            up = torch.tensor(np.concatenate([offs, offs_pad, patch_start]), device=dev)
            a, b = len(offs), len(offs) + len(offs_pad)
            self.set_pad(key, K, offs_pad, patch_start, up[:a], up[a:b], up[b:])
        return self._pad[key]

    def attn_l2(self, patch_size, enable_flash):
        K, n_pad, _, _, _, _, sum_l2 = self.pad(patch_size, enable_flash)
        return sum_l2 - float(K) * (n_pad - self.n)

    def slots(self, curve, patch_size, enable_flash):
        if isinstance(curve, tuple):
            if len(curve) != len(self.offs_host) - 1:
# ... 8 lines not shown
                return ops.slots_select(srcs, offs_pad, curve, n_pad)
            return _shared(self._slots, (curve, patch_size, enable_flash), compose, self.shared)
        lz = self._slot_lazy.pop((curve, patch_size, enable_flash), None) if self._slot_lazy else None
        if lz is not None:
            A, go, wo, n_pad, sid = lz
            self._slots[(curve, patch_size, enable_flash)] = ((A[go:go + n_pad], A[wo:wo + n_pad]), sid, None)

        def build():
            K, n_pad, offs, offs_pad = self.pad(patch_size, enable_flash)[:4]
            return ops.pad_plan(self.order(curve), offs, offs_pad, K, n_pad)
        return _shared(self._slots, (curve, patch_size, enable_flash), build, self.shared)


class RowLevel(Level):

    def __init__(self, voxels, keys, offs_host):
        n, nv = int(keys.numel()), voxels.n
        row_vox, perm_rows = ops.sort_pairs(keys, None, end_bit=max(1, nv.bit_length()))
        _, seg, _ = ops.pool_level(row_vox, 0)
        idx = row_vox
        super().__init__(0, voxels.depth, n, voxels.grid[idx], voxels.batch[idx], voxels.code4[:, idx].contiguous(), offs_host)
        self.voxels, self.perm_rows = voxels, perm_rows
        self.row_vox, self.row_start = row_vox.to(torch.int32), seg[:nv + 1]

    def nbr(self, ksize, kmajor=False):
        raise CdsegError("the row level of a Mix3D batch has no kernel map: sparse convs run on its voxel level (RowLevel.voxels)")

    def child_info(self):
        raise CdsegError("the row level of a Mix3D batch has no kernel map: sparse convs run on its voxel level (RowLevel.voxels)")


class Plan:
    def __init__(self):
        self.levels = {}
        self.links = {}
        self.rows = None
        self._row_links = {}
        self._finish = None
        self._link_lazy = {}
        self.shared = False
        self.ready = self.stream = self.source = None
        self._waited = set()

    def share(self, source):
        self.shared = True
        for lv in self.levels.values():
            lv.shared = True
        self.source = source
        self.stream = ops.current_stream_id()
        self.ready = ops.record_event() if self.stream is not None else None

    def join(self):
        cur = ops.current_stream_id()
        if self.ready is not None and cur != self.stream and cur not in self._waited:
            ops.wait_event(self.ready)
            self._waited.add(cur)

    def finish_pads(self):
        fin, self._finish = self._finish, None
        if fin is not None:
            fin()

    def link(self, a, b):
        if self._link_lazy:
            _cut(self._link_lazy, self.links, (a, b))

        def build():
            la, lb = self.levels[a], self.levels[b]
            if a > 0 and (0, a) in self.links and (0, b) in self.links:
                (cl0a, seg0a), (cl0b, seg0b) = self.link(0, a), self.link(0, b)
                return ops.link_derive(cl0a, seg0a, la.n, cl0b, seg0b, lb.n)
            cluster, seg, _ = ops.pool_level(la.code4[0], 3 * (lb.cum - la.cum))
            return (cluster, seg)
        return _shared(self.links, (a, b), build, self.shared)

    def link_from(self, fine, b):
        if fine is not self.rows:
            return self.link(fine.cum, b)

        def build():
            cluster, seg = self.link(0, b)
            m = self.levels[b].n
            return (cluster[fine.row_vox.long()], fine.row_start[seg[:m + 1].long()])
        return _shared(self._row_links, b, build, self.shared)


def skip_modules(bb):
    for name in ("_n_dec", "_c_dec"):
        if hasattr(bb, name):
            for dec in getattr(bb, name)._modules.values():
                yield dec.up


def _per_element(perm):
    return perm is not None and len(perm) > 0 and hasattr(perm[0], "__len__") and np.ndim(perm[0]) == 1


def reshuffle_curves(curves, perm, nb):
    if perm is None:
        return curves
    if not _per_element(perm):
        return [curves[int(j)] for j in perm]
    if len(perm) != nb:
        raise ValueError(f"{len(perm)} permutations for a batch of {nb} elements")
    return [tuple(c[b] if isinstance(c, tuple) else c for b, c in ((b, curves[int(perm[b][i])]) for b in range(nb)))
            for i in range(len(curves))]


class State:

    def __init__(self, level, x, xc, curves):
        self.level, self.x, self.xc, self.curves = level, x, xc, curves
        self.parent = None


class _HeadsInFp32:
    T = torch.float32

    def __init__(self, eng):
        bb, self.device, self.w = eng.model.backbone, eng.device, {}
        for name in ("n_head", "c_head"):
            mod = getattr(bb, "_" + name, None)
            if isinstance(mod, torch.nn.Linear):
                self.w[name + ".w"] = mod.weight.detach().to(device=eng.device, dtype=torch.float32).contiguous()
                self.w[name + ".b"] = (mod.bias.detach().to(device=eng.device, dtype=torch.float32).contiguous()
                                       if mod.bias is not None else None)

    def prepare(self, device):
        assert device == self.device

    def _fit(self, st, exact=False):
        return Engine._fit(self, st, exact)


class Engine:
    PRECISIONS = ("bf16", "bf16+head", "fp16", "fp16+head", "fp32", "fp32x3")

    def __init__(self, model, precision="bf16", variant=None):
        if precision not in self.PRECISIONS:
            raise ValueError(precision)
        self.model, self.precision = model, precision
        bb = model.backbone
        if getattr(bb, "condition", False) and not (bb.c_num_stages == 3 and bb.n_num_stages == 5):
            raise ValueError(f"conditional PT-v3m1 needs 3 c-branch and 5 n-branch stages (ptv3.py:1785-1794), got "
                             f"{bb.c_num_stages} / {bb.n_num_stages}")
        self.variant = variant or ("f16" if precision.startswith("fp16") or precision == "fp32x3" else "bf16")
        self.x3 = precision == "fp32x3"
        self.T = torch.float32 if precision in ("fp32", "fp32x3") else ops.LP_DTYPES[self.variant]
        self.device = None
        self.w = None
        self.rng_offset = 0
        self._rng_seed = None
        self.use_native_blocks = True
        self.fold_attn_scale = True
        self.speculate_depth = True
        self._depth_hint = {}
        self.count_saturation = False
        self.saturation_count = None
        self.saturation_checked = 0
        self._sat = None
        self.exact_attention_core = False
        self._pad_keys = None
        self.plans_built = 0
        self.native_plan = True
        self._plan_specs = {}
        self._tb_cache = {}
        self.eager_kernel_maps = True
        self._side = {}
        self.fork_stage = int(os.environ["CDSEG_FORK_STAGE"]) if os.environ.get("CDSEG_FORK_STAGE") else 2
        self._work_lock = threading.Lock()
        self._tls = threading.local()
        self.attn_work = 0.0
        self.conv_bytes = 0.0
        self.conv_deep_bytes = 0.0
        self.attn_bytes = 0.0
        self.hi = frozenset(("n_head", "c_head")) if precision.endswith("+head") else frozenset()
        self._twin = None

    def prepare(self, device):
        if self.w is not None and self.device == device:
            return
        with _lib.use(self.variant):
            self._prepare(device)

    def _prepare(self, device):
        self.device = device
        T = self.T
        w = {}
        self._blocks_to_describe = []

        def f32(t):
            return t.detach().to(device=device, dtype=torch.float32).contiguous()

        def lin(mod, pre):
            w[pre + ".w"] = mod.weight.detach().to(device=device, dtype=T).contiguous()
            w[pre + ".b"] = f32(mod.bias) if mod.bias is not None else None

        self.q_prescaled = T != torch.float32 and self.fold_attn_scale

        def lin_q(mod, pre, scale, rows):
            if not self.q_prescaled:
                return lin(mod, pre)
            f = float(scale) * 1.4426950408889634
            wt = mod.weight.detach().to(device=device, dtype=torch.float32).clone()
            wt[:rows] *= f
            w[pre + ".w"] = wt.to(T).contiguous()
            if mod.bias is not None:
                b = f32(mod.bias).clone()
                b[:rows] *= f
                w[pre + ".b"] = b
            else:
                w[pre + ".b"] = None

        def conv(mod, pre):
            w[pre + ".w"] = mod.weight.detach().reshape(mod.weight.shape[0], -1).to(device=device, dtype=T).contiguous()
            w[pre + ".b"] = f32(mod.bias) if mod.bias is not None else None
            if self.x3 and mod.kernel_size == 3 and hasattr(ops, "split16"):
                w[pre + ".w_hi"], w[pre + ".w_lo"] = ops.split16(w[pre + ".w"])
                cout = w[pre + ".w"].shape[0]
                if mod.in_channels == cout and cout in (32, 64) and hasattr(ops, "subm_conv3_f32"):
                    w[pre + ".wimg_hi"] = ops.subm_conv3_pack(w[pre + ".w_hi"])
                    w[pre + ".wimg_lo"] = ops.subm_conv3_pack(w[pre + ".w_lo"])
                if ("x3.scale", cout) not in w:
                    w[("x3.scale", cout)] = torch.full((cout,), 1.0 / 2048.0, dtype=torch.float32, device=device)
                    w[("x3.zero", cout)] = torch.zeros(cout, dtype=torch.float32, device=device)
            k, cin, cout = mod.kernel_size, mod.in_channels, mod.out_channels
            if (k == 3 and cin == cout and hasattr(ops, "subm_conv3_pack") and
                    ops.subm_conv3_ok(torch.empty((1, cin), dtype=T, device="meta"))):
                w[pre + ".wimg"] = ops.subm_conv3_pack(w[pre + ".w"])

        def ln(mod, pre):
            w[pre + ".g"], w[pre + ".b"] = f32(mod.weight), f32(mod.bias)

        def bn(mod, pre):
            scale = mod.weight.detach().double() / torch.sqrt(mod.running_var.detach().double() + mod.eps)
            shift = mod.bias.detach().double() - mod.running_mean.detach().double() * scale
            w[pre + ".scale"], w[pre + ".shift"] = f32(scale), f32(shift)

        self.block_desc = {}

        def block(mod, pre):
            self._blocks_to_describe.append((mod, pre))
            conv(mod.cpe[0], pre + ".cpe0")
            lin(mod.cpe[1], pre + ".cpe1")
            ln(mod.cpe[2], pre + ".cpe2")
            ln(mod.norm1[0], pre + ".norm1")
            lin_q(mod.attn.qkv, pre + ".qkv", mod.attn.scale, mod.channels)
            lin(mod.attn.proj, pre + ".proj")
            ln(mod.norm2[0], pre + ".norm2")
            lin(mod.mlp[0].fc1, pre + ".fc1")
            lin(mod.mlp[0].fc2, pre + ".fc2")

        def stem(mod, pre):
            cw = mod.stem.conv.weight.detach()
            cout, cin = cw.shape[0], cw.shape[-1]
            cpad = (cin + 7) // 8 * 8
            wp = torch.zeros(cout, cw.shape[1] ** 3, cpad, dtype=torch.float32)
            wp[:, :, :cin] = cw.reshape(cout, -1, cin).float().cpu()
            w[pre + ".w"] = wp.reshape(cout, -1).to(device=device, dtype=T).contiguous()
            w[pre + ".cpad"] = cpad
            if cw.shape[1] == 5 and cpad == 8 and hasattr(ops, "stem5_pack") and ops.stem5_ok(cout, T):
                w[pre + ".wimg"] = ops.stem5_pack(w[pre + ".w"])
            bn(mod.stem.norm, pre + ".bn")

        def pool(mod, pre):
            lin(mod.proj, pre + ".proj")
            bn(mod.norm[0], pre + ".bn")
            pw = w[pre + ".proj.w"]
            if hasattr(ops, "pool_fused_ok") and ops.pool_fused_ok(pw.shape[1], pw.shape[0], T):
                w[pre + ".proj.wimg"] = ops.pool_fused_pack(pw)

        def unpool(mod, pre):
            lin(mod.proj[0], pre + ".proj")
            bn(mod.proj[1], pre + ".proj_bn")
            lin(mod.proj_skip[0], pre + ".skip")
            bn(mod.proj_skip[1], pre + ".skip_bn")
            if mod.skip_connection_mode == "cat":
                f = mod.skip_scale
                wc = mod.proj_cat[0].weight.detach().float()
                c = wc.shape[0]
                w[pre + ".cat_a.w"] = (wc[:, :c] * f).to(device=device, dtype=T).contiguous()
                w[pre + ".cat_b.w"] = wc[:, c:].to(device=device, dtype=T).contiguous()
                w[pre + ".cat.b"] = f32(mod.proj_cat[0].bias)
            else:
                sw, pw = w[pre + ".skip.w"], w[pre + ".proj.w"]
                if hasattr(ops, "unpool_fused_ok") and ops.unpool_fused_ok(sw.shape[1], pw.shape[1], pw.shape[0], T, device):
                    w[pre + ".skip.wimg"] = ops.unpool_fused_pack(sw)
                    w[pre + ".proj.wimg"] = ops.unpool_fused_pack(pw)

        bb = self.model.backbone
        stem(bb._n_embedding, "n_emb")
        for s in range(bb.n_num_stages):
            enc = getattr(bb._n_enc, f"enc{s}")
            if s > 0:
                pool(enc.down, f"n_enc{s}.down")
            for name, mod in enc._modules.items():
                if name.startswith("block"):
                    block(mod, f"n_enc{s}.{name}")
        for s in range(bb.n_num_stages - 1):
            dec = getattr(bb._n_dec, f"dec{s}")
            unpool(dec.up, f"n_dec{s}.up")
            for name, mod in dec._modules.items():
                if name.startswith("block"):
                    block(mod, f"n_dec{s}.{name}")
        if isinstance(bb._n_head, torch.nn.Linear):
            lin(bb._n_head, "n_head")
# ... 469 lines not shown
            plan._finish = finish_pads
        else:
            finish_pads()
        return plan

    def shared_plan(self, input_dict):
        grid, offset = input_dict["grid_coord"], input_dict["offset"]
        dev = grid.device
        try:
            with _lib.use(self.variant):
                self.prepare(dev)
                if dev.type == "cuda" and hasattr(ops, "bind_stream"):
                    ops.bind_stream()
                n = grid.shape[0]
                offset_host = [int(v) for v in input_dict["offset_host"]] if "offset_host" in input_dict else None
                plan = self.build_plan(grid, offset.to(torch.int64), offset_host, n)
                share, SHARE_EVENTS.on = SHARE_EVENTS.on, False
                try:
                    self._touch_plan(plan)
                finally:
                    SHARE_EVENTS.on = share
                plan.share((grid, offset))
        finally:
            if hasattr(ops, "unbind_stream"):
                ops.unbind_stream()
        return plan

    def _touch_plan(self, plan):
        bb, w = self.model.backbone, self.w
        plan.finish_pads()
        curves = sorted({CURVES.index(o) for o in bb.order})
        lv0 = plan.levels[0]
        stems = ["n_emb"] + (["c_emb"] if bb.condition else [])
        if any((pre + ".wimg") in w for pre in stems) and lv0.parent is not None and lv0.n < (1 << 24):
            lv0.parent[0].nbr(3, True)
            lv0.child_info()
        if not all((pre + ".wimg") in w for pre in stems) or lv0.parent is None or lv0.n >= (1 << 24):
            lv0.nbr(5, True)

        def attn(lv, patch, flash):
            lv.pad(patch, flash)
            for c in curves:
                lv.slots(c, patch, flash)

        def stage(mods, lv):
            lv.nbr(3, True)
            for name, mod in mods._modules.items():
                if name.startswith("block"):
                    attn(lv, mod.attn.patch_size, mod.attn.enable_flash)

        for branch, cum, ns in (("n", plan.n_cum, bb.n_num_stages),) + ((("c", plan.c_cum, bb.c_num_stages),) if bb.condition else ()):
            for s in range(ns):
                if s > 0:
                    plan.link(cum[s - 1], cum[s])
                stage(getattr(getattr(bb, f"_{branch}_enc"), f"enc{s}"), plan.levels[cum[s]])
            for s in range(ns - 1):
                stage(getattr(getattr(bb, f"_{branch}_dec"), f"dec{s}"), plan.levels[cum[s]])
        if bb.condition:
            tm = bb._tm_dec0
            for cb in ([tm.cross_block1] if tm.tm_bidirectional else []) + [tm.cross_block2]:
                att = cb.attn
                for lv in (plan.levels[plan.n_cum[-1]], plan.levels[plan.c_cum[-1]]):
                    lv.nbr(3, True)
                    attn(lv, att.q_patch_size, att.enable_flash)

    def _check_plan(self, plan, input_dict, n, offset_host):
        lv0 = plan.levels[0]
        if lv0.n != n:
            raise CdsegError(f"the plan was built for {lv0.n} points, the input has {n}")
        if offset_host is not None and list(lv0.offs_host[1:]) != list(offset_host):
            raise CdsegError(f"the plan was built for batch offsets {list(lv0.offs_host[1:])}, the input has {list(offset_host)}")
        if getattr(self.model, "check_shared_geometry", False):
            if plan.source is None:
                raise CdsegError("check_shared_geometry: the plan does not come from shared_plan")
            grid, offset = input_dict["grid_coord"], input_dict["offset"]
            src_grid, src_offset = plan.source
            same = (grid.shape == src_grid.shape and offset.shape == src_offset.shape and
                    bool(torch.equal(grid.to(src_grid.dtype), src_grid)) and
                    bool(torch.equal(offset.to(src_offset.dtype), src_offset)))
            if not same:
                raise CdsegError("check_shared_geometry: grid_coord / offset differ from the ones the plan was built from")

    def _buf(self, rows, cols, dtype):
        return torch.empty((rows, cols), dtype=dtype, device=self.device)

    FUSE_LN_MAX_C = 512

    def _count_conv(self, n, c, esz):
        if c <= 64 and esz == 2:
            self.conv_bytes += 2.0 * n * c * esz + 27.0 * 4 * n + 27.0 * c * c * esz
        else:
            self.conv_deep_bytes += 2.0 * n * c * esz + 27.0 * 4 * n + 27.0 * c * c * esz

    def _conv3(self, xc, pre, lv, y):
        w = self.w
        self._count_conv(lv.n, xc.shape[1], xc.element_size())
        if (pre + ".w_hi") in w and y.dtype == torch.float32:
            cout = w[pre + ".w"].shape[0]
            sc, ze = w[("x3.scale", cout)], w[("x3.zero", cout)]
            xh, xl = ops.split16(xc)
            nbr = lv.nbr(3, True)
            if (pre + ".wimg_hi") in w and ops.subm_conv3_ok(xh) and y.stride(0) == y.shape[1]:
                ops.subm_conv3_f32(xh, w[pre + ".wimg_hi"], w[pre + ".b"], nbr, y)
                ops.subm_conv3_f32(xh, w[pre + ".wimg_lo"], None, nbr, y, out_scale=1.0 / 2048.0, accumulate=True)
                ops.subm_conv3_f32(xl, w[pre + ".wimg_hi"], None, nbr, y, out_scale=1.0 / 2048.0, accumulate=True)
                return
            ops.gemm(xh, w[pre + ".w_hi"], y, bias=w[pre + ".b"], nbr=nbr, nbr_kmajor=True, kvol=27)
            ops.gemm(xh, w[pre + ".w_lo"], y, scale=sc, shift=ze, res=y, nbr=nbr, nbr_kmajor=True, kvol=27)
            ops.gemm(xl, w[pre + ".w_hi"], y, scale=sc, shift=ze, res=y, nbr=nbr, nbr_kmajor=True, kvol=27)
            return
        if (pre + ".wimg") in w and ops.subm_conv3_ok(xc):
            ops.subm_conv3(xc, w[pre + ".wimg"], w[pre + ".b"], lv.nbr(3, True), y)
        else:
            ops.gemm(xc, w[pre + ".w"], y, bias=w[pre + ".b"], nbr=lv.nbr(3, True), nbr_kmajor=True, kvol=27)

    def _cpe(self, st, pre, xc, tbias=None, next_norm=None):
        w, lv = self.w, st.level
        c = st.x.shape[1]
        y = self._buf(lv.n, c, self.T)
        self._conv3(xc, pre + "0", lv, y)
        h = self._buf(lv.n, c, self.T) if next_norm else None
        if c <= self.FUSE_LN_MAX_C:
            ops.gemm(y, w[pre + "1.w"], st.x, bias=w[pre + "1.b"], ln_pre=(w[pre + "2.g"], w[pre + "2.b"]), res=st.x,
                     colbias=tbias, ln_post=(w[next_norm + ".g"], w[next_norm + ".b"]) if next_norm else None,
                     ln_out=h)
            return h
        y2 = self._buf(lv.n, c, torch.float32)
        ops.gemm(y, w[pre + "1.w"], y2, bias=w[pre + "1.b"])
        ops.layernorm(y2, w[pre + "2.g"], w[pre + "2.b"], st.x, res=st.x, colbias=tbias)
        if next_norm:
            ops.layernorm(st.x, w[next_norm + ".g"], w[next_norm + ".b"], h)
        return h

    def _mlp(self, st, pre_norm, pre_fc, h=None):
        w = self.w
        n, c = st.x.shape
        if h is None:
            h = self._buf(n, c, self.T)
            ops.layernorm(st.x, w[pre_norm + ".g"], w[pre_norm + ".b"], h)
        hid = w[pre_fc + "1.w"].shape[0]
        if ops.mlp_fused_ok(h, hid):
            st.xc = self._buf(n, c, self.T)
            ops.mlp_fused(h, w[pre_fc + "1.w"], w[pre_fc + "1.b"], w[pre_fc + "2.w"], w[pre_fc + "2.b"], st.x, st.xc)
            return
        u = self._buf(n, hid, self.T)
        ops.gemm(h, w[pre_fc + "1.w"], u, bias=w[pre_fc + "1.b"], act=ops.ACT_GELU)
        if self.T == torch.float32:
            ops.gemm(u, w[pre_fc + "2.w"], st.x, bias=w[pre_fc + "2.b"], res=st.x)
            st.xc = st.x
        else:
            st.xc = self._buf(n, c, self.T)
            ops.gemm(u, w[pre_fc + "2.w"], st.x, bias=w[pre_fc + "2.b"], res=st.x, out2=st.xc)

    def run_block(self, st, mod, pre, tbias=None):
        w, lv = self.w, st.level
        n, c = st.x.shape
        if self.native_blocks:
            att = mod.attn
            gidx, widx = lv.slots(st.curves[att.order_index], att.patch_size, att.enable_flash)
            _, _, _, _, patch_start, max_len, sum_l2 = lv.pad(att.patch_size, att.enable_flash)
            self.attn_work += 64.0 * att.num_heads * lv.attn_l2(att.patch_size, att.enable_flash)
            self.attn_bytes += 4.0 * n * c * st.xc.element_size()
            self._count_conv(n, c, st.xc.element_size())
            desc = self.block_desc[pre]
            xc_out = st.x if self.T == torch.float32 else self._buf(n, c, self.T)
            sb = self._scratch_bytes.get((pre, n))
            if sb is None:
                if len(self._scratch_bytes) > 4096:
                    self._scratch_bytes.clear()
                sb = self._scratch_bytes[(pre, n)] = ops.block_scratch_bytes(desc, n)
            ops.block_forward(desc, n, st.x, st.xc, xc_out, tbias, lv.nbr(3, True), gidx, widx, patch_start,
                              patch_start.numel() - 1, max_len, self.scratch(sb), sat_counter=self._sat)
            if self._sat is not None:
                self.saturation_checked += n * c * (5 if xc_out is not st.x else 4)
            st.xc = xc_out
            return
        qkv = self._buf(n, 3 * c, self.T)
        aflags = ops.ATTN_Q_PRESCALED if self.q_prescaled else 0
        deep_rr = ((pre + ".head_img") in w and (pre + ".tail_img") in w and not ops.cpe_head_fused_ok(st.xc)
                   and hasattr(ops, "cpe_head_rr2"))
        xs = None
        if deep_rr:
            y = self._buf(n, c, self.T)
            self._conv3(st.xc, pre + ".cpe0", lv, y)
            xs = self._buf(n, c, torch.float32)
            ops.cpe_head_rr2(y, w[pre + ".head_img"], w[pre + ".cpe1.b"], (w[pre + ".cpe2.g"], w[pre + ".cpe2.b"]), st.x, xs,
                             tbias, (w[pre + ".norm1.g"], w[pre + ".norm1.b"]), w[pre + ".qkv.b"], qkv,
                             qkv_flags=ops.ATTN_V_BF16)
            aflags |= ops.ATTN_V_BF16
        elif ops.cpe_head_fused_ok(st.xc):
            y = self._buf(n, c, self.T)
            self._conv3(st.xc, pre + ".cpe0", lv, y)
            if (pre + ".head_img") in w:
                ops.cpe_head_rr(y, w[pre + ".head_img"], w[pre + ".cpe1.b"], (w[pre + ".cpe2.g"], w[pre + ".cpe2.b"]), st.x,
                                tbias, (w[pre + ".norm1.g"], w[pre + ".norm1.b"]), w[pre + ".qkv.b"], qkv)
            else:
                ops.cpe_head_fused(y, w[pre + ".cpe1.w"], w[pre + ".cpe1.b"], (w[pre + ".cpe2.g"], w[pre + ".cpe2.b"]), st.x,
                                   tbias, (w[pre + ".norm1.g"], w[pre + ".norm1.b"]), w[pre + ".qkv.w"], w[pre + ".qkv.b"], qkv,
                                   qkv_flags=ops.ATTN_V_BF16)
                aflags |= ops.ATTN_V_BF16
        else:
            h = self._cpe(st, pre + ".cpe", st.xc, tbias, next_norm=pre + ".norm1")
            ops.gemm(h, w[pre + ".qkv.w"], qkv, bias=w[pre + ".qkv.b"])
        att = mod.attn
        curve = st.curves[att.order_index]
        gidx, widx = lv.slots(curve, att.patch_size, att.enable_flash)
        _, _, _, _, patch_start, max_len, sum_l2 = lv.pad(att.patch_size, att.enable_flash)
        work = 64.0 * att.num_heads * lv.attn_l2(att.patch_size, att.enable_flash)
        self._add_work(work, 4.0 * n * c * qkv.element_size())
        o = self._buf(n, c, self.T)
        if self.exact_attention_core and self.T != torch.float32:
            q32 = qkv.float()
            o32 = self._buf(n, c, torch.float32)
            if aflags & ops.ATTN_V_BF16 and self.T == torch.float16:
                q32[:, 2 * c:] = qkv[:, 2 * c:].view(torch.bfloat16).float()
            ops.attention(q32[:, :c], q32[:, c:2 * c], q32[:, 2 * c:], gidx, gidx, widx, patch_start, att.num_heads,
                          max_len, att.scale, o32, work=0.0, flags=aflags & ops.ATTN_Q_PRESCALED)
            o.copy_(o32)
        else:
            ops.attention(qkv[:, :c], qkv[:, c:2 * c], qkv[:, 2 * c:], gidx, gidx, widx, patch_start, att.num_heads,
                          max_len, att.scale, o, work=work, flags=aflags)
        hid = w[pre + ".fc1.w"].shape[0]
        if xs is not None:
            st.xc = self._buf(n, c, self.T)
            ops.attn_tail_rr2(o, w[pre + ".tail_img"], w[pre + ".proj.b"], w[pre + ".norm2.g"], w[pre + ".norm2.b"],
                              w[pre + ".fc1.b"], w[pre + ".fc2.b"], xs, st.x, st.xc, ws=self.scratch(4 * n * c * 4 + 256))
            return
        if ops.attn_tail_fused_ok(o, hid):
            st.xc = self._buf(n, c, self.T)
            if (pre + ".tail_img") in w:
                ops.attn_tail_rr(o, w[pre + ".tail_img"], w[pre + ".proj.b"], w[pre + ".norm2.g"], w[pre + ".norm2.b"],
                                 w[pre + ".fc1.b"], w[pre + ".fc2.b"], st.x, st.xc)
            else:
                ops.attn_tail_fused(o, w[pre + ".proj.w"], w[pre + ".proj.b"], w[pre + ".norm2.g"], w[pre + ".norm2.b"],
                                    w[pre + ".fc1.w"], w[pre + ".fc1.b"], w[pre + ".fc2.w"], w[pre + ".fc2.b"], st.x, st.xc)
            return
        if c <= self.FUSE_LN_MAX_C:
            h2 = self._buf(n, c, self.T)
            ops.gemm(o, w[pre + ".proj.w"], st.x, bias=w[pre + ".proj.b"], res=st.x,
                     ln_post=(w[pre + ".norm2.g"], w[pre + ".norm2.b"]), ln_out=h2)
        else:
            h2 = None
            ops.gemm(o, w[pre + ".proj.w"], st.x, bias=w[pre + ".proj.b"], res=st.x)
        self._mlp(st, pre + ".norm2", pre + ".fc", h2)

    def run_embedding(self, plan, feat, perm, pre, curves):
        w, lv = self.w, plan.levels[0]
        cout = w[pre + ".w"].shape[0]
        a = ops.gather_pad_cast(feat, perm, w[pre + ".cpad"], self.T)
        x = self._buf(lv.n, cout, torch.float32)
        xc = x if self.T == torch.float32 else self._buf(lv.n, cout, self.T)
        if (pre + ".wimg") in w and lv.parent is not None and lv.n < (1 << 24):
            par, (cluster, seg) = lv.parent
            ops.stem5(a, w[pre + ".wimg"], w[pre + ".bn.scale"], w[pre + ".bn.shift"], lv.grid, cluster, par.nbr(3, True),
                      lv.child_info(), lv.depth, x, None if xc is x else xc)
        else:
            ops.gemm(a, w[pre + ".w"], x, scale=w[pre + ".bn.scale"], shift=w[pre + ".bn.shift"], act=ops.ACT_GELU,
                     nbr=lv.nbr(5, True), nbr_kmajor=True, kvol=125, out2=None if xc is x else xc)
        self._sat_note(xc)
        return State(lv, x, xc, curves)

    def run_pooling(self, plan, st, pre, cum_to, perm):
        w = self.w
        fine, coarse = st.level, plan.levels[cum_to]
        _, seg = plan.link(fine.cum, cum_to)
        cout = w[pre + ".proj.w"].shape[0]
        x = self._buf(coarse.n, cout, torch.float32)
        xc = x if self.T == torch.float32 else self._buf(coarse.n, cout, self.T)
        if (pre + ".proj.wimg") in w and st.xc.stride(0) == st.xc.shape[1] and (
                fine.n <= 5 * coarse.n or fine.n >= POOL_LONG_MIN_ROWS):
            ops.pool_fused(st.xc, w[pre + ".proj.wimg"], w[pre + ".proj.b"], seg, coarse.n, w[pre + ".bn.scale"],
                           w[pre + ".bn.shift"], ops.ACT_GELU, x, xc)
        else:
            y = self._buf(fine.n, cout, self.T)
            ops.gemm(st.xc, w[pre + ".proj.w"], y, bias=w[pre + ".proj.b"])
            ops.segment_max(y, seg, coarse.n, w[pre + ".bn.scale"], w[pre + ".bn.shift"], ops.ACT_GELU, x,
                            None if xc is x else xc)
        self._sat_note(xc)
        curves = reshuffle_curves(st.curves, perm, len(coarse.offs_host) - 1)
        out = State(coarse, x, xc, curves)
        out.parent = st
        return out

    def _skip_ref(self, plan, parent):
        if parent.parent is None:
            return plan.perm0
        curve = parent.parent.curves[0]
        if isinstance(curve, tuple):
            if len(set(curve)) != 1:
                raise ValueError("a model that filters its skip features (s_factor != 1) has no per-fragment draws: the "
                                 "reference's filter runs over the rows of the whole batch in ONE order")
            curve = curve[0]
        return parent.level.ref_of_row(curve)

    def run_unpooling(self, plan, st, pre, mod):
        w = self.w
        parent = st.parent
        fine, coarse = parent.level, st.level
        cluster, seg = plan.link(fine.cum, coarse.cum)
        cout = w[pre + ".proj.w"].shape[0]
        f = mod.skip_scale
        s = mod.skip_filter
        x = self._buf(fine.n, cout, torch.float32)
        xc = self._buf(fine.n, cout, self.T)
        if (mod.skip_connection_mode == "add" and f == 1.0 and s is None and (pre + ".skip.wimg") in w and st.xc.is_cuda
                and parent.xc.stride(0) == parent.xc.shape[1] and st.xc.stride(0) == st.xc.shape[1]):
            ops.unpool_fused(parent.xc, w[pre + ".skip.wimg"], w[pre + ".skip.b"], w[pre + ".skip_bn.scale"],
                             w[pre + ".skip_bn.shift"], st.xc, w[pre + ".proj.wimg"], w[pre + ".proj.b"],
                             w[pre + ".proj_bn.scale"], w[pre + ".proj_bn.shift"], seg, coarse.n, ops.ACT_GELU, x, xc)
        elif mod.skip_connection_mode == "add":
            child = self._buf(coarse.n, cout, torch.float32)
            ops.gemm(st.xc, w[pre + ".proj.w"], child, bias=w[pre + ".proj.b"], scale=w[pre + ".proj_bn.scale"],
                     shift=w[pre + ".proj_bn.shift"], act=ops.ACT_GELU)
            if f == 1.0 and s is None:
                ops.gemm(parent.xc, w[pre + ".skip.w"], x, bias=w[pre + ".skip.b"], scale=w[pre + ".skip_bn.scale"],
                         shift=w[pre + ".skip_bn.shift"], act=ops.ACT_GELU, add_src=child, add_idx=cluster, out2=xc,
                         out2_pre_add=True)
            else:
                ops.gemm(parent.xc, w[pre + ".skip.w"], x, bias=w[pre + ".skip.b"], scale=w[pre + ".skip_bn.scale"],
                         shift=w[pre + ".skip_bn.shift"], act=ops.ACT_GELU, out2=xc)
                if s is None:
                    ops.skip_merge(x, f=f, child=child, cluster=cluster)
                else:
                    ref = self._skip_ref(plan, parent)
                    ops.skip_merge(x, ops.skip_stats(x, ref, fine.n), s, f, ref, fine.n, child, cluster)
        else:
            child = self._buf(coarse.n, cout, self.T)
            ops.gemm(st.xc, w[pre + ".proj.w"], child, bias=w[pre + ".proj.b"], scale=w[pre + ".proj_bn.scale"],
                     shift=w[pre + ".proj_bn.shift"], act=ops.ACT_GELU)
# ... 260 lines not shown
        self._tls.rng_frag = draws.get("rng_bases")
        per_fragment = draws.get("per_fragment") or (bb.shuffle_orders and any(_per_element(p) for p in draws["perms"]))
        if per_fragment and not input_dict.get("shared_geometry"):
            raise ValueError("per-fragment draws are defined for a batch whose elements share geometry (the fragments of one "
                             "test-time augmentation: TestScene.collated marks them)")
        feat = feat.float().contiguous()
        if noise_level is not None:
            fn = draws.get("feat_noise")
            fn = self._device_randn(tuple(feat.shape)) if fn is None else fn.to(dev, torch.float32)
            feat = ops.axpy(feat, fn.contiguous(), noise_level)
            input_dict["feat"] = feat
        perms = list(draws["perms"]) if bb.shuffle_orders else [None] * (per_call * n_backbone_calls)
        self.last_plan = plan
        return feat, draws, perms, plan, per_call

    def _t_bias(self, t):
        w = self.w
        if self.model.backbone.T_dim == -1 or "t.table" not in w:
            return {}
        ent = self._tb_cache.get(t)
        if ent is None:
            v = ops.gemv(w["t.fc1.w"], w["t.fc1.b"], w["t.table"][t + 1], ops.ACT_SWISH)
            v = ops.gemv(w["t.fc2.w"], w["t.fc2.b"], v, ops.ACT_SWISH)
            tall = ops.gemv(w["t.mlp.w"], w["t.mlp.b"], v, ops.ACT_NONE)
            if tall.is_cuda:
                torch.cuda.current_stream(tall.device).synchronize()
            ent = self._tb_cache[t] = {k: tall[a:b] for k, (a, b) in self.t_slices.items()}
        return ent

    def _sat_begin(self, dev):
        self._sat = None
        self.saturation_count, self.saturation_checked = None, 0
        if self.count_saturation and self.T == torch.float16:
            self._sat = torch.zeros(1, dtype=torch.int64, device=dev)

    def _sat_note(self, t):
        if self._sat is not None and t is not None and t.dtype == torch.float16:
            ops.count_saturated(t, self._sat)
            self.saturation_checked += t.numel()

    def _sat_end(self):
        if self._sat is not None:
            self.saturation_count = int(self._sat.item())
            self._sat = None

    def _inference(self, input_dict, noise_level=None, draws=None, plan=None):
        m, bb = self.model, self.model.backbone
        feat, draws, perms, plan, _ = self._setup(input_dict, noise_level, draws, 1, plan=plan)
        n, dev = feat.shape[0], feat.device
        c_ch = m.c_in_channels
        c_feat = c_perm = None
        t = 0
        if bb.condition:
            if m.dm and m.dm_input == "xt":
                nz = draws.get("noise")
                if nz is None:
                    c_feat, c_perm = self._device_randn((n, c_ch)), None
                else:
                    c_feat, c_perm = nz.to(dev, torch.float32).contiguous(), plan.perm0
                t = m.T - 1
            else:
                c_feat = feat if c_ch == feat.shape[1] else input_dict["coord"].float().contiguous()
                c_perm = plan.perm0
        self._sat_begin(dev)
        self._msi_begin()
        logits, _ = self.backbone(plan, feat, c_feat, c_perm, t, perms, want_c=False)
        self._msi_end()
        self._sat_end()
        return logits

    def _msi_begin(self):
        self._tls.msi = dict(backbone_calls=0, n_encoders=0, c_decoders=0)

    def _msi_count(self, key):
        st = getattr(self._tls, "msi", None)
        if st is not None:
            st[key] += 1

    def _msi_end(self):
        self.msi_stats, self._tls.msi = self._tls.msi, None

    def _inference_ddim(self, input_dict, step, mode, noise_level, draws, plan=None, reuse_encoder=False):
        m, bb = self.model, self.model.backbone
        if not bb.condition:
            return self._inference(input_dict, noise_level, draws, plan)
        if m.dm_target != "noise":
            raise NotImplementedError("dm_target other than 'noise'")
        schedule = np.linspace(-1, m.T - 1, num=step + 1, dtype=int)[::-1]
        feat, draws, perms, plan, per_call = self._setup(input_dict, noise_level, draws, len(schedule), always_noise=True,
                                                         plan=plan)
        n, dev = feat.shape[0], feat.device
        nz = draws.get("noise")
        c_xt = self._device_randn((n, m.c_in_channels)) if nz is None else \
            ops.gather_rows(nz.to(dev, torch.float32).contiguous(), plan.perm0)
        ab = m.Alpha_bar
        n_pred = None
        hoist = {} if reuse_encoder else None
        one_launch = hasattr(ops, "msi_step")
        self._msi_begin()
        for k, t in enumerate(schedule):
            t = int(t)
            last = t <= 0
            logits, eps = self.backbone(plan, feat, c_xt, None, t, perms[per_call * k:per_call * (k + 1)], want_c=not last,
                                        hoist=hoist)
            coef = None
            if not last:
                coef = (float(torch.sqrt(ab[t - 1])), float(torch.sqrt(1 - ab[t])), float(torch.sqrt(ab[t])),
                        float(torch.sqrt(1 - ab[t - 1])), False)
            if one_launch:
                acc = n_pred if (mode == "avg" and n_pred is not None) else None
                if coef is not None or acc is not None:
                    ops.msi_step(c_xt if coef else None, eps if coef else None, *(coef or (0.0, 0.0, 1.0, 0.0, False)),
                                 acc=acc, logits=logits if acc is not None else None,
                                 acc_mode=ops.MSI_MEAN if last else ops.MSI_ADD,
                                 scale=float(1.0 / len(schedule)) if last else 1.0)
                if acc is None:
                    n_pred = logits
                    if mode == "avg" and last:
                        n_pred = ops.axpy(torch.zeros_like(n_pred), n_pred, 1.0 / len(schedule))
            else:
                if coef is not None:
                    c_xt = ops.ddim_update(c_xt, eps, *coef[:4], final=coef[4])
                if mode == "avg":
                    n_pred = logits if n_pred is None else ops.axpy(n_pred, logits, 1.0)
                else:
                    n_pred = logits
            if last:
                break
        if mode == "avg" and not one_launch:
            n_pred = ops.axpy(torch.zeros_like(n_pred), n_pred, 1.0 / len(schedule))
        self._msi_end()
        return n_pred

    def backbone(self, plan, feat, c_feat, c_perm, t, perms, want_c, hoist=None):
        bb = self.model.backbone
        w = self.w
        cond = bb.condition
        n = feat.shape[0]
        dev = feat.device
        pi = iter(perms)
        base_curves = [CURVES.index(o) for o in bb.order]

        nb = len(plan.levels[0].offs_host) - 1

        def shuffled(perm):
            return reshuffle_curves(list(base_curves), perm, nb)

        n_cum, c_cum = plan.n_cum, plan.c_cum
        if cond:
            c_curves = shuffled(next(pi))
        n_curves = shuffled(next(pi))
        tb = self._t_bias(t) if cond else {}

        def enc_stage(st, branch, s, cum, perm):
            enc = getattr(getattr(bb, f"_{branch}_enc"), f"enc{s}")
            e = self._eng(f"{branch}_enc{s}")
            e._fit(st)
            if s > 0:
                st = e.run_pooling(plan, st, f"{branch}_enc{s}.down", cum[s], perm)
            for name, mod in enc._modules.items():
                if name.startswith("block"):
                    key = f"{branch}_enc{s}.{name}"
                    e.run_block(st, mod, key, tb.get(key))
            return st

        def dec_stage(st, branch, s):
            dec = getattr(getattr(bb, f"_{branch}_dec"), f"dec{s}")
            e = self._eng(f"{branch}_dec{s}")
            e._fit(st)
            e._fit(st.parent)
            st = e.run_unpooling(plan, st, f"{branch}_dec{s}.up", dec.up)
            for name, mod in dec._modules.items():
                if name.startswith("block"):
                    key = f"{branch}_dec{s}.{name}"
                    e.run_block(st, mod, key, tb.get(key))
            return st

        if cond:
            p_c1, p_n1, p_n2, p_c2, p_n3, p_n4 = (next(pi) for _ in range(6))
            n_perms = [None, p_n1, p_n2, p_n3, p_n4]

            def c_branch():
                st = self._eng("c_emb").run_embedding(plan, c_feat, c_perm, "c_emb", c_curves)
                st = enc_stage(st, "c", 0, c_cum, None)
                st = enc_stage(st, "c", 1, c_cum, p_c1)
                return enc_stage(st, "c", 2, c_cum, p_c2)

            fork = self.fork_stage if (dev.type == "cuda" and self.fork_stage is not None) else None
            if hoist:
                fork = None
            SHARE_EVENTS.on = fork is not None
            if fork is None:
                plan.finish_pads()
            cst = c_branch() if fork is None else None
            if hoist:
                nst = hoist["nst"]
            else:
                nst = self._eng("n_emb").run_embedding(plan, feat, plan.perm0, "n_emb", n_curves)
                plan.finish_pads()
                join = None
                for s in range(bb.n_num_stages):
                    if fork is not None and s == fork:
                        cst, join = self._on_side_stream(c_branch)
                    nst = enc_stage(nst, "n", s, n_cum, n_perms[s])
                if join is not None:
                    ops.wait_event(join)
                self._msi_count("n_encoders")
            if hoist is not None:
                hoist["nst"] = nst
                x = ops.gather_pad_cast(nst.x, None, nst.x.shape[1], torch.float32)
                work = State(nst.level, x, x if nst.xc is nst.x else nst.xc, nst.curves)
                work.parent = nst.parent
                nst = work
            e = self._eng("x")
            e._fit(nst)
            e._fit(cst)
            tm = bb._tm_dec0
            if tm.tm_bidirectional:
                e.run_cross_block(cst, nst, tm.cross_block1, "x1", keep_kv_x=True)
            e.run_cross_block(nst, cst, tm.cross_block2, "x")
        else:
            nst = self._eng("n_emb").run_embedding(plan, feat, plan.perm0, "n_emb", n_curves)
            plan.finish_pads()
            for s in range(bb.n_num_stages):
                nst = enc_stage(nst, "n", s, n_cum, next(pi) if s > 0 else None)
            self._msi_count("n_encoders")
        self.trace = {"n_bottleneck": nst.x}
        c_out = None
        self._msi_count("backbone_calls")
        if cond and want_c:
            self._msi_count("c_decoders")
            for s in reversed(range(bb.c_num_stages - 1)):
                cst = dec_stage(cst, "c", s)
            e = self._eng("c_head")
            e._fit(cst, exact=True)
            c_out = torch.empty((n, w["c_head.w"].shape[0]), dtype=torch.float32, device=dev)
            ops.gemm(cst.xc, e.w["c_head.w"], c_out, bias=e.w["c_head.b"])
        for s in reversed(range(bb.n_num_stages - 1)):
            nst = dec_stage(nst, "n", s)
        if "n_head.w" in w:
            e = self._eng("n_head")
            e._fit(nst, exact=True)
            logits = torch.empty((n, w["n_head.w"].shape[0]), dtype=torch.float32, device=dev)
            ops.gemm(nst.xc, e.w["n_head.w"], logits, bias=e.w["n_head.b"], out_idx=plan.perm0)
        else:
            logits = torch.empty((n, nst.x.shape[1]), dtype=torch.float32, device=dev)
            ops.scatter_rows(nst.x, plan.perm0, logits)
        return logits, c_out
```

### cdsegnet_amd/ops.py

```python
import collections
import ctypes
import math
import os
import threading

import torch

from . import _lib
from ._lib import ACT_GELU, ACT_NONE, ACT_SWISH, BF16, F32, GemmArgs, check

__all__ = ["ACT_NONE", "ACT_GELU", "ACT_SWISH", "F32", "BF16"]

LP_DTYPES = {"bf16": torch.bfloat16, "f16": torch.float16}


class _Dtypes:

    def __getitem__(self, dtype):
        if dtype == torch.float32:
            return F32
        if dtype == LP_DTYPES[_lib.active()]:
            return BF16
        raise _lib.CdsegError(f"{dtype} tensors do not belong to the active build of the library ({_lib.active()})")

# ... 560 lines not shown
        a.act = int(act)
        ent = (a, ctypes.byref(a), W)
        if cache:
            if len(cache_d) > 4096:
                cache_d.clear()
            cache_d[key] = ent
    a = ent[0]
    if (res is not None and res.dtype != torch.float32) or (add_src is not None and add_src.dtype != torch.float32):
        raise _lib.CdsegError("gemm residuals are float32")
    a.A = A.data_ptr()
    a.res, a.add_src, a.add_idx, a.nbr, a.out_idx = _dp(res), _dp(add_src), _dp(add_idx), _dp(nbr), _dp(out_idx)
    a.out, a.out2 = out.data_ptr(), _dp(out2)
    m = int(M if M is not None else (nbr.shape[1 if nbr_kmajor else 0] if nbr is not None else A.shape[0]))
    a.nbr_kmajor = 1 if nbr_kmajor else 0
    a.M = m
    a.lda = A.stride(0)
    a.ldo = out.stride(0)
    a.ldo2 = out2.stride(0) if out2 is not None else 0
    a.ldres = res.stride(0) if res is not None else 0
    a.ldadd = add_src.stride(0) if add_src is not None else 0
    a.a_dtype = _DT[A.dtype]
    a.out_dtype = _DT[out.dtype]
    a.out2_dtype = _DT[out2.dtype] if out2 is not None else 0
    a.out2_pre_add = 1 if out2_pre_add else 0
    a.colbias = _dp(colbias)
    if ln_pre is not None:
        a.ln_pre_g, a.ln_pre_b = ln_pre[0].data_ptr(), ln_pre[1].data_ptr()
    else:
        a.ln_pre_g = a.ln_pre_b = None
    if ln_post is not None:
        a.ln_post_g, a.ln_post_b = ln_post[0].data_ptr(), ln_post[1].data_ptr()
        a.ln_out, a.ldln, a.ln_out_dtype = ln_out.data_ptr(), ln_out.stride(0), _DT[ln_out.dtype]
    else:
        a.ln_post_g = a.ln_post_b = a.ln_out = None
    a.ln_eps = float(ln_eps)
    wkey = (m, a.N, nbr is not None, ln_pre is not None or ln_post is not None)
    want = _GEMM_WS_BYTES.get(wkey)
    if want is None:
        if len(_GEMM_WS_BYTES) > 4096:
            _GEMM_WS_BYTES.clear()
        want = _GEMM_WS_BYTES[wkey] = int(_lib.load().cdseg_gemm_ws_bytes(*wkey))
    if want:
        ws = workspace(want, out.device)
        a.ws, a.ws_bytes = ws.data_ptr(), ws.numel()
    else:
        a.ws, a.ws_bytes = None, 0
    tok = TIMER.begin("conv" if nbr is not None else "gemm") if TIMER is not None else None
    check(_lib.load().cdseg_gemm(ent[1], _stream()), "gemm")
    if tok is not None:
        TIMER.end(tok, 2.0 * a.M * a.N * a.K * a.kvol)
    return out


FUSED_MLP_CHANNELS = (32, 64, 128)


def mlp_fused_ok(h, hidden):
    c = h.shape[1]
    return (is_lp(h.dtype) and c in FUSED_MLP_CHANNELS and hidden == 4 * c and
            c <= 128)


def mlp_fused(h, w1, b1, w2, b2, x, xc=None):
    _need_gpu(h, x)
    check(_lib.load().cdseg_mlp_fused(_ptr(h), h.stride(0), _ptr(w1), _ptr(b1), _ptr(w2), _ptr(b2), _ptr(x), x.stride(0),
                                       _ptr(xc), xc.stride(0) if xc is not None else 0, h.shape[0], h.shape[1], _DT[h.dtype],
                                       _stream()), "mlp_fused")
    return x


def cpe_head_fused_ok(y):
    return is_lp(y.dtype) and y.shape[1] in (32, 64)


def cpe_head_fused(y, wl, bl, lnp, x, colbias, ln1, wqkv, bqkv, qkv, eps=1e-5, qkv_flags=0):
    _need_gpu(y, x)
    check(_lib.load().cdseg_cpe_head_fused(_ptr(y), y.stride(0), _ptr(wl), _ptr(bl), _ptr(lnp[0]), _ptr(lnp[1]), _ptr(x),
                                            x.stride(0), _ptr(colbias), _ptr(ln1[0]), _ptr(ln1[1]), float(eps), _ptr(wqkv),
                                            _ptr(bqkv), _ptr(qkv), qkv.stride(0), y.shape[0], y.shape[1], _DT[y.dtype],
                                            int(qkv_flags), _stream()), "cpe_head_fused")
    return qkv


def attn_tail_fused_ok(o, hidden):
    c = o.shape[1]
    return is_lp(o.dtype) and c in (32, 64) and hidden == 4 * c


def attn_tail_fused(o, wp, bp, ln_g, ln_b, w1, b1, w2, b2, x, xc=None, eps=1e-5):
    _need_gpu(o, x)
    check(_lib.load().cdseg_attn_tail_fused(_ptr(o), o.stride(0), _ptr(wp), _ptr(bp), _ptr(ln_g), _ptr(ln_b), float(eps),
                                             _ptr(w1), _ptr(b1), _ptr(w2), _ptr(b2), _ptr(x), x.stride(0), _ptr(xc),
                                             xc.stride(0) if xc is not None else 0, o.shape[0], o.shape[1], _DT[o.dtype],
                                             _stream()), "attn_tail_fused")
    return x


DEEP512_MIN_ROWS = int(os.environ.get("CDSEG_DEEP512_MIN_ROWS", 2560))
DEEP512_ROWS64_MIN = 256 * 32 + 1
DEEP_CHANNELS = (128, 256, 512)


def block_rr_ok(channels, dtype):
    return is_lp(dtype) and (channels in (32, 64) or channels in DEEP_CHANNELS)


def block_rr_head_on(channels=32):
    return channels in DEEP_CHANNELS


def block_rr_pack(channels, wl, wqkv, wp, w1, w2):
    _need_gpu(wl, wqkv, wp, w1, w2)
    lib = _lib.load()
    dev = wp.device
    head = _scratch(lib.cdseg_block_rr_img_bytes(channels, 0), dev) if wl is not None else None
    tail = _scratch(lib.cdseg_block_rr_img_bytes(channels, 1), dev)
    check(lib.cdseg_block_rr_pack(int(channels), _ptr(wl), _ptr(wqkv), _ptr(head), _ptr(wp), _ptr(w1), _ptr(w2), _ptr(tail),
                                  _stream()), "block_rr_pack")
    return head, tail


def cpe_head_rr(y, head_img, bl, lnp, x, colbias, ln1, bqkv, qkv, eps=1e-5, qkv_flags=0):
    check(_lib.load().cdseg_cpe_head_rr(_ptr(y), y.stride(0), _ptr(head_img), _ptr(bl), _ptr(lnp[0]), _ptr(lnp[1]), _ptr(x),
                                        x.stride(0), _ptr(colbias), _ptr(ln1[0]), _ptr(ln1[1]), float(eps), _ptr(bqkv),
                                        _ptr(qkv), qkv.stride(0), y.shape[0], y.shape[1], int(qkv_flags), _stream()),
          "cpe_head_rr")
    return qkv


def cpe_head_rr2(y, head_img, bl, lnp, x, x_out, colbias, ln1, bqkv, qkv, eps=1e-5, qkv_flags=0):
    check(_lib.load().cdseg_cpe_head_rr2(_ptr(y), y.stride(0), _ptr(head_img), _ptr(bl), _ptr(lnp[0]), _ptr(lnp[1]), _ptr(x),
                                         x.stride(0), _ptr(x_out), x_out.stride(0), _ptr(colbias), _ptr(ln1[0]), _ptr(ln1[1]),
                                         float(eps), _ptr(bqkv), _ptr(qkv), qkv.stride(0), y.shape[0], y.shape[1],
                                         int(qkv_flags), _stream()), "cpe_head_rr2")
    return qkv


def attn_tail_rr2(o, tail_img, bp, ln_g, ln_b, b1, b2, x_in, x, xc=None, ws=None, eps=1e-5):
    check(_lib.load().cdseg_attn_tail_rr2(_ptr(o), o.stride(0), _ptr(tail_img), _ptr(bp), _ptr(ln_g), _ptr(ln_b), float(eps),
                                          _ptr(b1), _ptr(b2), _ptr(x_in), x_in.stride(0), _ptr(x), x.stride(0), _ptr(xc),
                                          xc.stride(0) if xc is not None else 0, o.shape[0], o.shape[1], _ptr(ws),
                                          0 if ws is None else ws.numel() * ws.element_size(), _stream()), "attn_tail_rr2")
    return x


def attn_tail_rr(o, tail_img, bp, ln_g, ln_b, b1, b2, x, xc=None, eps=1e-5):
    check(_lib.load().cdseg_attn_tail_rr(_ptr(o), o.stride(0), _ptr(tail_img), _ptr(bp), _ptr(ln_g), _ptr(ln_b), float(eps),
                                         _ptr(b1), _ptr(b2), _ptr(x), x.stride(0), _ptr(xc),
                                         xc.stride(0) if xc is not None else 0, o.shape[0], o.shape[1], _stream()),
          "attn_tail_rr")
    return x


def _dp(t):
    return None if t is None else t.data_ptr()


def make_block_desc(dtype, channels, heads, hidden, attn_scale, ln_eps, tensors, attn_flags=0, x3=False):
    d = _lib.BlockDesc()
    d.dtype, d.channels, d.heads, d.hidden = (F32X3 if (x3 and dtype == torch.float32) else _DT[dtype]), int(channels), int(heads), int(hidden)
    d.attn_scale, d.ln_eps = float(attn_scale), float(ln_eps)
    d.attn_flags = int(attn_flags)
    for k, t in tensors.items():
        setattr(d, k, t.data_ptr())
    return (d, ctypes.byref(d), dict(tensors))


def block_scratch_bytes(desc, n):
    return _lib.load().cdseg_block_scratch_bytes(desc[1], int(n))


def count_saturated(x, counter):
    _need_gpu(x, counter)
    check(_lib.load().cdseg_count_saturated(_ptr(x), x.shape[0], x.shape[1], x.stride(0), _ptr(counter), _stream()),
          "count_saturated")


def split16(x, lo_scale=2048.0):
    _need_gpu(x)
    T = LP_DTYPES[_lib.active()]
    hi = torch.empty(x.shape, dtype=T, device=x.device)
    lo = torch.empty(x.shape, dtype=T, device=x.device)
    check(_lib.load().cdseg_split16(_ptr(x), x.stride(0), x.shape[0], x.shape[1], _ptr(hi), _ptr(lo), hi.stride(0),
                                    float(lo_scale), _stream()), "split16")
    return hi, lo


def block_forward(desc, n, x, xc_in, xc_out, tbias, nbr, gidx, widx, patch_start, num_patches, max_len, scratch,
                  sat_counter=None):
    if _TLS.block_io is None:
        io = _lib.BlockIO()
        _TLS.block_io = (io, ctypes.byref(io))
    io, ref = _TLS.block_io
    io.n = int(n)
    io.x, io.xc_in, io.xc_out, io.tbias = x.data_ptr(), xc_in.data_ptr(), xc_out.data_ptr(), _dp(tbias)
    io.nbr, io.gidx, io.widx, io.patch_start = nbr.data_ptr(), gidx.data_ptr(), widx.data_ptr(), patch_start.data_ptr()
    io.num_patches, io.max_len = int(num_patches), int(max_len)
    io.scratch, io.scratch_bytes = scratch.data_ptr(), scratch.numel()
    io.sat_counter = sat_counter.data_ptr() if sat_counter is not None else None
    check(_lib.load().cdseg_block_forward(desc[1], ref, _stream()), "block_forward")


def stem5_ok(cout, dtype):
    return cout == 32 and is_lp(dtype)


def child_info(zcode_sorted, seg_start, m):
    _need_gpu(zcode_sorted, seg_start)
    info = torch.empty(int(m), dtype=torch.int64, device=zcode_sorted.device)
    check(_lib.load().cdseg_child_info(_ptr(zcode_sorted), _ptr(seg_start), int(m), _ptr(info), _stream()), "child_info")
    return info


def stem5_pack(w):
    _need_gpu(w)
    assert is_lp(w.dtype) and tuple(w.shape) == (32, 1000)
    img = _scratch(_lib.load().cdseg_stem5_wimg_bytes(), w.device)
    check(_lib.load().cdseg_stem5_pack(_ptr(w), _ptr(img), _stream()), "stem5_pack")
    return img


def stem5(x8, wimg, scale, shift, grid, cluster, parent_nbr3, cinfo, depth, out, out2=None):
    _need_gpu(x8, wimg, grid, cluster, parent_nbr3, cinfo, out)
    n, m = x8.shape[0], cinfo.numel()
    check(_lib.load().cdseg_stem5(_ptr(x8), _ptr(wimg), _ptr(scale), _ptr(shift), _ptr(grid), _ptr(cluster),
                                  _ptr(parent_nbr3), _ptr(cinfo), n, m, int(depth), _ptr(out), _ptr(out2), _stream()), "stem5")
    return out


def subm_conv3_ok(x):
    n = x.shape[0]
    return (is_lp(x.dtype) and x.dim() == 2 and x.shape[1] in (32, 64) and x.stride(0) == x.shape[1] and
            n * 27 * 4 < 2 ** 31 and n * x.shape[1] * 2 < 2 ** 31 - 65536)


def subm_conv3_pack(w):
    _need_gpu(w)
    c = w.shape[0]
    img = _scratch(_lib.load().cdseg_subm_conv3_wimg_bytes(c), w.device)
    check(_lib.load().cdseg_subm_conv3_pack(_ptr(w), c, _ptr(img), _stream()), "subm_conv3_pack")
    return img


def subm_conv3(x, wimg, bias, nbr_kmajor, out):
    _need_gpu(x, wimg, nbr_kmajor, out)
    n, c = x.shape
    check(_lib.load().cdseg_subm_conv3(_ptr(x), x.stride(0), _ptr(wimg), _ptr(bias), _ptr(nbr_kmajor), n, c, _ptr(out),
                                       out.stride(0), _stream()), "subm_conv3")
    return out


def subm_conv3_f32(x, wimg, bias, nbr_kmajor, out, out_scale=1.0, accumulate=False):
    _need_gpu(x, wimg, nbr_kmajor, out)
    n, c = x.shape
    check(_lib.load().cdseg_subm_conv3_f32(_ptr(x), x.stride(0), _ptr(wimg), _ptr(bias), _ptr(nbr_kmajor), n, c, _ptr(out),
                                           out.stride(0), float(out_scale), 1 if accumulate else 0, _stream()),
          "subm_conv3_f32")
    return out


def layernorm(x, gamma, beta, out, *, eps=1e-5, res=None, colbias=None, out2=None):
    m, c = x.shape
    check(_lib.load().cdseg_layernorm(_ptr(x), dt(x), x.stride(0), _ptr(gamma), _ptr(beta), float(eps), _ptr(res),
                                      res.stride(0) if res is not None else 0, _ptr(colbias), _ptr(out), dt(out),
                                      out.stride(0), _ptr(out2), dt(out2) if out2 is not None else 0,
                                      out2.stride(0) if out2 is not None else 0, m, c, _stream()), "layernorm")
    return out


ATTN_Q_PRESCALED, ATTN_V_BF16 = 1, 2


def attention(q, k, v, q_gidx, kv_gidx, widx, patch_start, num_heads, max_len, scale, out, work=0.0, flags=0):
    num_patches = patch_start.numel() - 1
    if not (q.dtype == k.dtype == out.dtype) or (v.dtype != q.dtype and not (flags & ATTN_V_BF16)):
        raise _lib.CdsegError("attention: q, k, v, out must share a dtype")
    tok = TIMER.begin("attention") if TIMER is not None else None
    check(_lib.load().cdseg_attention_ex(_ptr(q), _ptr(k), _ptr(v), q.stride(0), k.stride(0), v.stride(0), _ptr(q_gidx),
                                         _ptr(kv_gidx), _ptr(widx), _ptr(patch_start), num_patches, int(num_heads),
                                         int(max_len), float(scale), _ptr(out), out.stride(0),
                                         F32X3 if (_TLS.f32x3 and q.dtype == torch.float32) else dt(q), int(flags), _stream()),
          "attention")
    if tok is not None:
        TIMER.end(tok, work)
    return out


def segment_max(y, seg_start, m, scale, shift, act, out, out2=None):
    c = y.shape[1]
    check(_lib.load().cdseg_segment_max(_ptr(y), dt(y), y.stride(0), _ptr(seg_start), m, c, _ptr(scale), _ptr(shift),
                                        int(act), _ptr(out), out.stride(0), _ptr(out2),
                                        dt(out2) if out2 is not None else 0, out2.stride(0) if out2 is not None else 0,
                                        _stream()), "segment_max")
    return out


def pool_fused_ok(cin, cout, dtype):
    return is_lp(dtype) and (int(cin), int(cout)) in ((32, 64), (64, 128))


def pool_fused_pack(w):
    _need_gpu(w)
    cout, cin = w.shape
    lib = _lib.load()
    img = _scratch(lib.cdseg_pool_fused_img_bytes(cin, cout), w.device)
    check(lib.cdseg_pool_fused_pack(_ptr(w), cin, cout, _ptr(img), _stream()), "pool_fused_pack")
    return img


def pool_fused(x, wimg, bias, seg_start, m, scale, shift, act, out, out2=None):
    _need_gpu(x, out)
    cin, cout = x.shape[1], out.shape[1]
    check(_lib.load().cdseg_pool_fused_n(_ptr(x), x.stride(0), x.shape[0], _ptr(wimg), _ptr(bias), _ptr(seg_start), int(m),
                                         _ptr(scale), _ptr(shift), int(act), _ptr(out), out.stride(0), _ptr(out2),
                                         out2.stride(0) if out2 is not None else 0, cin, cout, _stream()), "pool_fused")
    return out


POOL_FOLD_AUTO, POOL_FOLD_WALK, POOL_FOLD_SCAN = 0, 1, 2


class pool_fused_fold:

    def __init__(self, fold):
        self.fold, self.lib = int(fold), _lib.load()

    def __enter__(self):
        self.prev = self.lib.cdseg_pool_fused_fold(self.fold)
        if self.prev < 0:
            check(self.prev, "pool_fused_fold")
        return self

    def __exit__(self, *exc):
        self.lib.cdseg_pool_fused_fold(self.prev)
        return False


def unpool_fused_ok(k_skip, k_child, c, dtype, device):
    return (is_lp(dtype) and torch.device(device).type == "cuda"
            and (int(k_skip), int(k_child), int(c)) in ((32, 64, 64), (64, 128, 64)))


def unpool_fused_pack(w):
    _need_gpu(w)
    cout, cin = w.shape
    lib = _lib.load()
    img = _scratch(lib.cdseg_unpool_fused_img_bytes(cin, cout), w.device)
    check(lib.cdseg_unpool_fused_pack(_ptr(w), cin, cout, _ptr(img), _stream()), "unpool_fused_pack")
    return img


def unpool_fused(skip_x, wimg_skip, bias_skip, scale_skip, shift_skip, coarse_x, wimg_child, bias_child, scale_child, shift_child,
                 seg_start, m, act, out, out2):
    _need_gpu(skip_x, coarse_x, out, out2)
    check(_lib.load().cdseg_unpool_fused(_ptr(skip_x), skip_x.stride(0), _ptr(wimg_skip), _ptr(bias_skip), _ptr(scale_skip),
                                         _ptr(shift_skip), _ptr(coarse_x), coarse_x.stride(0), _ptr(wimg_child), _ptr(bias_child),
                                         _ptr(scale_child), _ptr(shift_child), _ptr(seg_start), int(m), int(act), _ptr(out),
                                         out.stride(0), _ptr(out2), out2.stride(0), skip_x.shape[1], coarse_x.shape[1],
                                         out.shape[1], _stream()), "unpool_fused")
    return out


def segment_mean(x, seg_start, m):
    out = torch.empty((m, x.shape[1]), dtype=torch.float32, device=x.device)
    check(_lib.load().cdseg_segment_mean(_ptr(x), x.stride(0), _ptr(seg_start), m, x.shape[1], _ptr(out),
                                         out.stride(0), _stream()), "segment_mean")
    return out


def gemv(w, b, x, act=ACT_NONE):
    n, k = w.shape
    y = torch.empty(n, dtype=torch.float32, device=w.device)
    check(_lib.load().cdseg_gemv(_ptr(w), _ptr(b), _ptr(x), n, k, int(act), _ptr(y), _stream()), "gemv")
    return y


def randn(shape, seed, offset, device, out=None):
    if out is None:
        out = torch.empty(shape, dtype=torch.float32, device=device)
    elif tuple(out.shape) != tuple(shape) or out.dtype != torch.float32 or not out.is_contiguous():
        raise _lib.CdsegError("randn: `out` is a contiguous float32 tensor of the requested shape")
    check(_lib.load().cdseg_randn(_ptr(out), out.numel(), int(seed) & (2 ** 64 - 1), int(offset), _stream()), "randn")
    return out


def cast(src, dtype):
    src = src.contiguous()
    out = torch.empty(src.shape, dtype=dtype, device=src.device)
    check(_lib.load().cdseg_cast(_ptr(src), dt(src), _ptr(out), _DT[dtype], src.numel(), _stream()), "cast")
    return out


def gather_pad_cast(src, idx, cpad, dtype):
    src = src.contiguous()
    n = idx.numel() if idx is not None else src.shape[0]
    out = torch.empty((n, cpad), dtype=dtype, device=src.device)
    check(_lib.load().cdseg_gather_pad_cast(_ptr(src), src.stride(0), _ptr(idx), n, src.shape[1], int(cpad), _ptr(out),
                                            _DT[dtype], _stream()), "gather_pad_cast")
    return out


def ddim_update(xt, eps, sqrt_ab_prev, sqrt_1m_ab, sqrt_ab, sqrt_1m_ab_prev, final=False):
    out = torch.empty_like(xt)
    check(_lib.load().cdseg_ddim_update(_ptr(xt), _ptr(eps), float(sqrt_ab_prev), float(sqrt_1m_ab), float(sqrt_ab),
                                 float(sqrt_1m_ab_prev), 1 if final else 0, _ptr(out), xt.numel(), _stream()),
          "ddim_update")
    return out


def axpy(a, b, alpha):
    out = torch.empty_like(a)
    check(_lib.load().cdseg_axpy(_ptr(a), _ptr(b), float(alpha), _ptr(out), a.numel(), _stream()), "axpy")
    return out


MSI_SET, MSI_ADD, MSI_MEAN = 0, 1, 2


def msi_step(c_xt=None, eps=None, sqrt_ab_prev=0.0, sqrt_1m_ab=0.0, sqrt_ab=1.0, sqrt_1m_ab_prev=0.0, final=False,
             acc=None, logits=None, acc_mode=MSI_ADD, scale=1.0):
    for name, a, b in (("c_xt / eps", c_xt, eps), ("acc / logits", acc, logits)):
        for t in (a, b):
            if t is not None:
# ... 984 lines not shown
```

### include/cdseg.h

```cpp
#ifndef CDSEG_H
#define CDSEG_H

#include <stddef.h>
#include <stdint.h>

#ifdef __cplusplus
extern "C" {
#endif

#define CDSEG_OK 0
#define CDSEG_ERR_ARG (-1)
#define CDSEG_ERR_LAUNCH (-2)
#define CDSEG_ERR_WORKSPACE (-3)
#define CDSEG_ERR_UNSUPPORTED (-4)

#define CDSEG_F32 0
#define CDSEG_BF16 1
#define CDSEG_F32X3 2

#define CDSEG_ORDER_Z 0
#define CDSEG_ORDER_Z_TRANS 1
#define CDSEG_ORDER_HILBERT 2
#define CDSEG_ORDER_HILBERT_TRANS 3

// ... 110 lines not shown
#define CDSEG_ATTN_V_BF16 2
int cdseg_attention_ex(const void* q, const void* k, const void* v, int ldq, int ldk, int ldv, const int32_t* q_gidx,
                       const int32_t* kv_gidx, const int32_t* widx, const int32_t* patch_start, int num_patches,
                       int num_heads, int max_len, float scale, void* out, int ldo, int dtype, int flags, void* stream);

long cdseg_attention_schedule(int num_patches, int num_heads, int max_len, int dtype, int32_t* table, long capacity);

#define CDSEG_ROUTE_WORDS 8
#define CDSEG_ROUTE_F_VEC_OK 1
#define CDSEG_ROUTE_F_GATHER 2
#define CDSEG_ROUTE_F_PARTIALS 4
#define CDSEG_ROUTE_F_KDIV 8
#define CDSEG_ROUTE_F_KSHIFT_LT6 16
#define CDSEG_ROUTE_F_CT_SHIFT 5
int cdseg_route_enable(int on);
void cdseg_route_clear(void);
int cdseg_route_read(int32_t* rec_host, int capacity);
int cdseg_route_catalog(char* buf_host, size_t bytes);
int cdseg_route_note(const int32_t* rec_host);

int cdseg_prof_enable(int on);
int cdseg_prof_summary(double* total_ms, long* launches);
#define CDSEG_PROF_ATTENTION 0
#define CDSEG_PROF_CONV 1
#define CDSEG_PROF_CONV_DEEP 2
int cdseg_prof_summary_class(int cls, double* total_ms, long* launches);

int cdseg_segment_max(const void* y, int y_dtype, int ldy, const int32_t* seg_start, long m, int c,
                      const float* scale, const float* shift, int act, float* out, int ldo, void* out2,
                      int out2_dtype, int ldo2, void* stream);
int cdseg_pool_fused_fold(int fold);
int cdseg_pool_fused_n(const void* x, int ldx, long n_fine, const void* wimg, const float* bias, const int32_t* seg_start, long m,
                       const float* scale, const float* shift, int act, float* out, int ldo, void* out2, int ldo2,
                       int cin, int cout, void* stream);
size_t cdseg_pool_fused_img_bytes(int cin, int cout);
int cdseg_pool_fused_pack(const void* w, int cin, int cout, void* wimg, void* stream);
int cdseg_pool_fused(const void* x, int ldx, const void* wimg, const float* bias, const int32_t* seg_start, long m,
                     const float* scale, const float* shift, int act, float* out, int ldo, void* out2, int ldo2,
                     int cin, int cout, void* stream);
size_t cdseg_unpool_fused_img_bytes(int cin, int cout);
int cdseg_unpool_fused_pack(const void* w, int cin, int cout, void* wimg, void* stream);
int cdseg_unpool_fused(const void* skip_x, int ld_skip, const void* wimg_skip, const float* bias_skip,
                       const float* scale_skip, const float* shift_skip, const void* coarse_x, int ld_coarse,
                       const void* wimg_child, const float* bias_child, const float* scale_child,
                       const float* shift_child, const int32_t* seg_start, long m, int act, float* out, int ldo,
                       void* out2, int ldo2, int k_skip, int k_child, int c, void* stream);
int cdseg_segment_mean(const float* x, int ldx, const int32_t* seg_start, long m, int c, float* out, int ldo,
                       void* stream);

int cdseg_gemv(const float* w, const float* b, const float* x, int n, int k, int act, float* y, void* stream);
int cdseg_randn(float* out, long n, uint64_t seed, uint64_t offset, void* stream);
int cdseg_cast(const void* src, int src_dtype, void* dst, int dst_dtype, long n, void* stream);
int cdseg_gather_pad_cast(const float* src, int ld_src, const int32_t* idx, long n, int cin, int cpad, void* dst,
                          int dst_dtype, void* stream);
int cdseg_ddim_update(const float* xt, const float* eps, float sqrt_ab_prev, float sqrt_1m_ab, float sqrt_ab,
                      float sqrt_1m_ab_prev, int final_step, float* out, long n, void* stream);
int cdseg_count_saturated(const void* x, long rows, int cols, int ld, unsigned long long* counter, void* stream);
int cdseg_subm_conv3_f32(const void* x, int ldx, const void* wimg, const float* bias, const int32_t* nbr_kmajor, long n,
                         int channels, float* yf, int ldyf, float out_scale, int accumulate, void* stream);
int cdseg_split16(const float* x, int ldx, long rows, int cols, void* hi, void* lo, int ld16, float lo_scale, void* stream);
int cdseg_axpy(const float* a, const float* b, float alpha, float* out, long n, void* stream);
int cdseg_msi_step(float* c_xt, const float* eps, long n_c, float sqrt_ab_prev, float sqrt_1m_ab, float sqrt_ab,
                   float sqrt_1m_ab_prev, int final_step, float* acc, const float* logits, long n_l, int acc_mode,
                   float scale, void* stream);

int cdseg_voxelize(const float* coord, double grid_size, long n, int32_t* grid, int64_t* key, int32_t* min3_dev,
                   void* stream);
int cdseg_voxelize_f64(const double* coord, double grid_size, long n, int32_t* grid, int64_t* key, int32_t* min3_dev,
                       void* stream);
int cdseg_center_shift(const void* xyz, int is_f64, long n, int apply_z, void* out, void* ws12, void* stream);
int cdseg_tta_apply(const float* in, long n, const double* rot9_host, double scale, int apply_scale, int flip, void* out,
                    void* stream);
int cdseg_div_add(const float* in, float div, float add, long n, float* out, void* stream);
int cdseg_collect_feat(const float* a, int ca, const void* b, int b_is_f64, int cb, long n, float* out, void* stream);
int cdseg_max_run(const int32_t* seg_start, long m, int32_t* out_dev, void* stream);
int cdseg_fragment_select(const int32_t* idx_sort, const int32_t* seg_start, long m, int frag, int32_t* idx_part,
                          void* stream);
int cdseg_softmax_vote(const float* logits, int ldl, const int32_t* idx, long m, int c, float* pred, int ldp,
                       void* stream);
int cdseg_argmax_rows(const float* x, int ldx, long n, int c, int32_t* out, void* stream);
size_t cdseg_fragments_build_ws_bytes(int F);
int cdseg_fragments_build(const int32_t* idx_sort, const int32_t* seg_start, long m, int F, long n, const int32_t* grid,
                          const float* feat, int c, const void* coord, int coord_f64, int center_shift, int32_t* index,
                          int32_t* grid_out, float* feat_out, float* coord_out, void* ws, size_t ws_bytes, void* stream);
int cdseg_softmax_vote_fragments(const float* logits, int ldl, const int32_t* index, long m, int k, int c, float* pred,
                                 int ldp, long n, void* stream);
int cdseg_voxel_inverse(const int32_t* idx_sort, const int32_t* cluster, long n, int32_t* inverse, void* stream);

#define CDSEG_TT_CENTER_NONE 0
#define CDSEG_TT_CENTER_HOST 1
#define CDSEG_TT_CENTER_BBOX 2
#define CDSEG_TT_CENTER_SHIFT_Z 3
#define CDSEG_TT_CENTER_SHIFT_XY 4
int cdseg_tt_bbox(const void* xyz, int is_f64, long n, void* ws12, void* stream);
int cdseg_tt_affine(const void* in, int in_f64, long n, int center, const double* center3_host, const double* bbox6_dev,
                    const double* rot9_host, int add_back, double scale, int apply_scale, int flipx, int flipy, void* out,
                    int out_f64, void* stream);
int cdseg_tt_jitter(double* coord, const void* z, int z_f64, double sigma, double clip, long n, void* stream);
int cdseg_tt_blur3(const float* in, int d0, int d1, int d2, int axis, float* out, void* stream);
int cdseg_tt_elastic(double* coord, long n, const float* noise, const int* dims3_host, const double* start3_host,
                     const double* step3_host, const double* stop3_host, double magnitude, void* stream);
int cdseg_tt_color(float* color, long n, const double* bbox6_dev, double blend, int contrast, const double* tr3_host,
                   const void* noise, int noise_f64, double noise_mul, void* stream);
int cdseg_tt_voxel_pick(const int32_t* idx_sort, const int32_t* seg_start, long m, const int64_t* r, int32_t* out,
                        void* stream);
int cdseg_tt_dist_key(const double* coord, long n, long center, int64_t* key, void* stream);
int cdseg_rand_int(int64_t* out, long n, uint64_t seed, uint64_t offset, const int32_t* bound_dev, uint32_t bound,
                   void* stream);

int cdseg_knn(const float* ref_xyz, const int32_t* ref_offset, long n, const float* qry_xyz, const int32_t* qry_offset,
              long m, int nb, int k, const float* origin, float cell, int32_t* idx, float* dist2, void* ws, size_t ws_bytes,
              void* stream);
size_t cdseg_knn1_ws_bytes(long n);
int cdseg_knn1(const float* ref_xyz, const int32_t* ref_offset, long n, const float* qry_xyz, const int32_t* qry_offset,
               long m, int nb, const float* origin, float cell, int32_t* idx, float* dist2, void* ws, size_t ws_bytes,
               void* stream);
int cdseg_iou_counts(const int32_t* pred, const int32_t* pred_idx, const int32_t* target, long n, int k, int ignore_index,
                     int64_t* out, void* stream);

int cdseg_mlp_fused(const void* h, int ldh, const void* w1, const float* b1, const void* w2, const float* b2, float* x,
                    int ldx, void* xc, int ldxc, long n, int channels, int dtype, void* stream);

int cdseg_attn_tail_fused(const void* o, int ldo, const void* wp, const float* bp, const float* ln_g, const float* ln_b,
                          float ln_eps, const void* w1, const float* b1, const void* w2, const float* b2, float* x, int ldx,
                          void* xc, int ldxc, long n, int channels, int dtype, void* stream);

int cdseg_cpe_head_fused(const void* y, int ldy, const void* wl, const float* bl, const float* lnp_g, const float* lnp_b,
                         float* x, int ldx, const float* colbias, const float* ln1_g, const float* ln1_b, float eps,
                         const void* wqkv, const float* bqkv, void* qkv, int ldqkv, long n, int channels, int dtype,
                         int qkv_flags, void* stream);

size_t cdseg_subm_conv3_wimg_bytes(int channels);
int cdseg_subm_conv3_pack(const void* w, int channels, void* wimg, void* stream);
int cdseg_subm_conv3(const void* x, int ldx, const void* wimg, const float* bias, const int32_t* nbr_kmajor, long n,
                     int channels, void* y, int ldy, void* stream);

int cdseg_child_info(const int64_t* zcode_sorted, const int32_t* seg_start, long m, int64_t* info, void* stream);
size_t cdseg_stem5_wimg_bytes(void);
int cdseg_stem5_pack(const void* w, void* wimg, void* stream);
int cdseg_stem5(const void* x8, const void* wimg, const float* scale, const float* shift, const int32_t* grid,
                const int32_t* cluster, const int32_t* parent_nbr3, const int64_t* child_info, long n, long m, int depth,
                float* out, void* out2, void* stream);

size_t cdseg_block_rr_img_bytes(int channels, int which);
int cdseg_block_rr_pack(int channels, const void* wl, const void* wqkv, void* head_img, const void* wp, const void* w1,
                        const void* w2, void* tail_img, void* stream);
int cdseg_cpe_head_rr(const void* y, int ldy, const void* head_img, const float* bl, const float* lnp_g, const float* lnp_b,
                      float* x, int ldx, const float* colbias, const float* ln1_g, const float* ln1_b, float eps,
                      const float* bqkv, void* qkv, int ldqkv, long n, int channels, int qkv_flags ,
                      void* stream);
int cdseg_attn_tail_rr(const void* o, int ldo, const void* tail_img, const float* bp, const float* ln_g, const float* ln_b,
                       float eps, const float* b1, const float* b2, float* x, int ldx, void* xc, int ldxc, long n,
                       int channels, void* stream);
int cdseg_cpe_head_rr2(const void* y, int ldy, const void* head_img, const float* bl, const float* lnp_g, const float* lnp_b,
                       const float* x, int ldx, float* x_out, int ldx_out, const float* colbias, const float* ln1_g,
                       const float* ln1_b, float eps, const float* bqkv, void* qkv, int ldqkv, long n, int channels,
                       int qkv_flags, void* stream);
int cdseg_attn_tail_rr2(const void* o, int ldo, const void* tail_img, const float* bp, const float* ln_g, const float* ln_b,
                        float eps, const float* b1, const float* b2, const float* x_in, int ldx_in, float* x, int ldx, void* xc,
                        int ldxc, long n, int channels, void* ws, size_t ws_bytes, void* stream);

typedef struct cdseg_block_desc {
  int dtype;
  int channels;
  int heads;
  int hidden;
  float attn_scale;
  float ln_eps;
  const void* cpe_conv_w;
  const float* cpe_conv_b;
  const void* cpe_lin_w;
  const float* cpe_lin_b;
  const float* cpe_ln_g;
  const float* cpe_ln_b;
  const float* norm1_g;
  const float* norm1_b;
  const void* qkv_w;
  const float* qkv_b;
  const void* proj_w;
  const float* proj_b;
  const float* norm2_g;
  const float* norm2_b;
  const void* fc1_w;
  const float* fc1_b;
  const void* fc2_w;
  const float* fc2_b;
  const void* cpe_conv_wimg;
  const void* head_img;
  const void* tail_img;
  int attn_flags;
} cdseg_block_desc;

typedef struct cdseg_block_io {
  long n;
  float* x;
  const void* xc_in;
  void* xc_out;
  const float* tbias;
  const int32_t* nbr;
  const int32_t* gidx;
  const int32_t* widx;
  const int32_t* patch_start;
  int num_patches;
  int max_len;
  void* scratch;
  size_t scratch_bytes;
  unsigned long long* sat_counter;
} cdseg_block_io;

size_t cdseg_block_scratch_bytes(const cdseg_block_desc* desc, long n);
int cdseg_block_forward(const cdseg_block_desc* desc, const cdseg_block_io* io, void* stream);

#define CDSEG_PLAN_MAX_LEVELS 8
#define CDSEG_PLAN_MAX_LINKS 16
#define CDSEG_PLAN_MAX_PADS 4
typedef struct cdseg_plan_spec {
  int nlev;
  int cum[9];
  int ncurve;
  int curve_rows[3];
  int nslot_curve;
  int slot_curve[4];
  int nlink;
  int link_a[CDSEG_PLAN_MAX_LINKS];
  int link_b[CDSEG_PLAN_MAX_LINKS];
  int npad;
  int pad_patch[CDSEG_PLAN_MAX_PADS];
  int pad_flash[CDSEG_PLAN_MAX_PADS];
} cdseg_plan_spec;

typedef struct cdseg_plan_begin_io {
  const void* grid;
  int grid_elem_bytes;
  const int64_t* offset;
  int nb;
  long n;
  int depth;
  int end_bit;
  int32_t* i32;
  int64_t* i64;
  void* ws;
  size_t ws_bytes;
  int64_t* gmax_host;
  int32_t* meta_host;
} cdseg_plan_begin_io;

int cdseg_plan_begin_layout(const cdseg_plan_spec* spec, long n, int nb, long* off_out, long* totals_out);
int cdseg_plan_begin(const cdseg_plan_spec* spec, const cdseg_plan_begin_io* io, int phase, void* stream);

typedef struct cdseg_plan_finish_io {
  long n;
  int nb;
  int depth;
  const long* m_host;
  const int* offs_host;
  const int32_t* grid0;
  const int32_t* bat0;
  const int64_t* code0;
  const int32_t* cluster;
  const int32_t* seg;
  const int32_t* orders0;
  int32_t* i32;
  int64_t* i64;
  void* ws;
  size_t ws_bytes;
  int32_t* pads_host;
} cdseg_plan_finish_io;

int cdseg_plan_finish_layout(const cdseg_plan_spec* spec, long n, int nb, const long* m_host, const int* offs_host,
                             long* off_out, long* info_out);
int cdseg_plan_finish(const cdseg_plan_spec* spec, const cdseg_plan_finish_io* io, void* stream);

size_t cdseg_attention_bwd_ws_bytes(long num_slots, int num_heads);
int cdseg_attention_bwd(const void* q, const void* k, const void* v, int ldq, int ldk, int ldv, const int32_t* q_gidx,
                        const int32_t* kv_gidx, const int32_t* widx, const int32_t* patch_start, int num_patches,
                        int num_heads, long num_slots, int max_len, float scale, const void* dout, int lddo, void* dq,
                        void* dk, void* dv, int lddq, int lddk, int lddv, int dtype, void* ws, size_t ws_bytes, void* stream);
int cdseg_layernorm_bwd(const float* x, int ldx, const float* gamma, float eps, const float* dy, int lddy, float* dx, int lddx,
                        int accumulate, float* dgamma, float* dbeta, long m, int c, void* stream);
int cdseg_gelu_bwd(const float* u, const float* dy, float* dx, long n, void* stream);
int cdseg_linear_wgrad(const float* x, int ldx, const int32_t* xidx, const float* dy, int lddy, long m, int k, int n, float* dw,
                       int lddw, float* db, void* stream);
int cdseg_conv_wgrad(const float* x, int ldx, const int32_t* nbr_kmajor, int kvol, const float* dy, int lddy, long m, int cin,
                     int cout, float* dw, float* db, void* stream);
int cdseg_linear_wgrad16(const void* x, int ldx, const int32_t* xidx, const void* dy, int lddy, long m, int k, int n, float* dw,
                         int lddw, float* db, void* stream);
int cdseg_conv_wgrad16(const void* x, int ldx, const int32_t* nbr_kmajor, int kvol, const void* dy, int lddy, long m, int cin,
                       int cout, float* dw, float* db, void* stream);

int cdseg_attention_drop(const void* q, const void* k, const void* v, int ldq, int ldk, int ldv, const int32_t* q_gidx,
                         const int32_t* kv_gidx, const int32_t* widx, const int32_t* patch_start, int num_patches, int num_heads,
                         int max_len, float scale, void* out, int ldo, int dtype, double rate, uint64_t seed, uint64_t offset,
                         void* stream);
int cdseg_attention_drop_bwd(const void* q, const void* k, const void* v, int ldq, int ldk, int ldv, const int32_t* q_gidx,
                             const int32_t* kv_gidx, const int32_t* widx, const int32_t* patch_start, int num_patches,
                             int num_heads, long num_slots, int max_len, float scale, const void* dout, int lddo, void* dq,
                             void* dk, void* dv, int lddq, int lddk, int lddv, int dtype, void* ws, size_t ws_bytes, double rate,
                             uint64_t seed, uint64_t offset, void* stream);
int cdseg_dropout(const float* x, int ldx, float* y, int ldy, long m, int c, double rate, uint64_t seed, uint64_t offset,
                  void* stream);

int cdseg_wgrad_partition(long m, int n, int k, int kvol, int dtype, long* rows_per_split, int* splits);
size_t cdseg_wgrad_det_ws_bytes(long m, int n, int k, int kvol, int dtype);
int cdseg_linear_wgrad_det(const void* x, int ldx, const int32_t* xidx, const void* dy, int lddy, long m, int k, int n, float* dw,
                           int lddw, float* db, int dtype, void* ws, size_t ws_bytes, void* stream);
int cdseg_conv_wgrad_det(const void* x, int ldx, const int32_t* nbr_kmajor, int kvol, const void* dy, int lddy, long m, int cin,
                         int cout, float* dw, float* db, int dtype, void* ws, size_t ws_bytes, void* stream);
size_t cdseg_layernorm_bwd_det_ws_bytes(long m, int c);
int cdseg_layernorm_bwd_det(const float* x, int ldx, const float* gamma, float eps, const float* dy, int lddy, float* dx, int lddx,
                            int accumulate, float* dgamma, float* dbeta, long m, int c, void* ws, size_t ws_bytes, void* stream);
int cdseg_segment_sum(const float* src, int ld, const int32_t* seg_start, long m, int c, float* out, int ldo, void* stream);

size_t cdseg_seg_loss_ws_bytes(long n, int c);
int cdseg_seg_loss_fwd(const float* logits, int ldl, const int64_t* labels, long n, int c, long ignore_index, int phase,
                       int32_t* hist, const int32_t* hist_host, float* out, float* coef, void* ws, size_t ws_bytes,
                       void* stream);
int cdseg_seg_loss_bwd(const float* logits, int ldl, const int64_t* labels, long n, int c, long ignore_index,
                       const int32_t* hist_host, const float* coef, const float* g_ce, const float* g_lovasz, float* dlogits,
                       int lddl, void* stream);

int cdseg_bn_partition(long m, int c, long* rows_per_block, int* blocks);
size_t cdseg_bn_ws_bytes(long m, int c);
int cdseg_bn_stats(const float* x, int ldx, long m, int c, double* stats, void* ws, size_t ws_bytes, void* stream);
int cdseg_bn_finish(const double* stats, int c, double eps, double momentum, float* mean, float* invstd, float* running_mean,
                    float* running_var, void* stream);
int cdseg_bn_gelu_fwd(const float* x, int ldx, long m, int c, const float* mean, const float* invstd, const float* gamma,
                      const float* beta, float* y, int ldy, void* stream);
int cdseg_bn_gelu_bwd_sums(const float* x, int ldx, const float* dy, int lddy, long m, int c, const float* mean,
                           const float* invstd, const float* gamma, const float* beta, double* gsums, void* ws, size_t ws_bytes,
                           void* stream);
int cdseg_bn_gelu_bwd_dx(const float* x, int ldx, const float* dy, int lddy, long m, int c, const float* mean, const float* invstd,
                         const float* gamma, const float* beta, const double* gsums, const double* count, float* dx, int lddx,
                         void* stream);
int cdseg_segment_max_arg(const float* y, int ldy, const int32_t* seg_start, long m, int c, float* out, int ldo, int32_t* arg,
                          int lda, void* stream);
int cdseg_segment_max_bwd(const float* dout, int lddo, const int32_t* arg, int lda, const int32_t* cluster, long n, int c,
                          float* dy, int lddy, void* stream);

size_t cdseg_fuse_gate_ws_bytes(long rows, int c);
int cdseg_fuse_gate_fwd(const float* s, const float* a, const float* m, const float* alpha, const float* gamma, float* y,
                        long rows, int c, void* stream);
int cdseg_fuse_gate_bwd(const float* dy, const float* s, const float* a, const float* m, const float* alpha, const float* gamma,
                        float* ds, float* da, double* sums, long rows, int c, void* ws, size_t ws_bytes, void* stream);

int cdseg_skip_partition(long n, int c, long* rows_per_chunk, int* chunks);
size_t cdseg_skip_stats_ws_bytes(long n, int c);
int cdseg_skip_stats(const void* x, int dtype, int ldx, long n, int c, const int32_t* ref_of_row, long n_total, double* stats,
                     void* ws, size_t ws_bytes, void* stream);
int cdseg_skip_fold(const void* w, int dtype, int ldw, int cout, int cin, const double* stats, double* u, void* stream);
int cdseg_skip_merge(float* x, int ldx, long n, int c, const double* stats, int folded, double s, long n_total, double f,
                     const int32_t* ref_of_row, const float* child, int ldchild, const int32_t* cluster, long n_child, void* stream);

#define CDSEG_OPT_CHUNK 8192
#define CDSEG_OPT_MAX_GROUPS 16
#define CDSEG_OPT_CLIP 1
#define CDSEG_OPT_SKIP 2
typedef struct cdseg_opt_tensor {
  float* p;
  const float* g;
  float* m;
// ... 102 lines not shown
```

Before: 82.60 million.

## Fuse segmentation head into last decoder block tail and skip dead outputs

Adds a templated LOGITS variant of the fused attention-tail kernel. It computes the final classifier head with fp32 MFMA directly from the MLP output and scatters the logits through perm0, so the separate head GEMM and the re-read of xc are skipped. It also adds a BLOCK_X_DEAD flag and liveness analysis in the engine, so final blocks whose fp32 x (or xc) output is never consumed skip those stores. The cost is extra LDS for the head weights, possibly lower occupancy, and more complex routing with fallback when the path is unsupported.

Result: faster. 83.59 million (median of 6 runs) (+1.2%).

```diff
diff --git a/cdsegnet_amd/_lib.py b/cdsegnet_amd/_lib.py
--- a/cdsegnet_amd/_lib.py
+++ b/cdsegnet_amd/_lib.py
@@ -61,6 +61,8 @@
         ("nbr", c_void_p), ("gidx", c_void_p), ("widx", c_void_p), ("patch_start", c_void_p),
         ("num_patches", c_int), ("max_len", c_int), ("scratch", c_void_p), ("scratch_bytes", c_size_t),
         ("sat_counter", c_void_p),
+        ("flags", c_int), ("logits", c_void_p), ("head_w", c_void_p), ("head_b", c_void_p), ("out_idx", c_void_p),
+        ("num_classes", c_int), ("ld_logits", c_int),
     ]
 
 
@@ -222,6 +224,9 @@
                                   c_void_p, c_float, c_void_p, c_void_p, c_int, c_long, c_int, c_int, c_void_p]),
     "cdseg_attn_tail_rr": (c_int, [c_void_p, c_int, c_void_p, c_void_p, c_void_p, c_void_p, c_float, c_void_p, c_void_p,
                                    c_void_p, c_int, c_void_p, c_int, c_long, c_int, c_void_p]),
+    "cdseg_attn_tail_rr_ex": (c_int, [c_void_p, c_int, c_void_p, c_void_p, c_void_p, c_void_p, c_float, c_void_p, c_void_p,
+                                      c_void_p, c_int, c_void_p, c_int, c_long, c_int, c_int, c_void_p, c_int, c_void_p,
+                                      c_void_p, c_void_p, c_int, c_void_p]),
     "cdseg_cpe_head_rr2": (c_int, [c_void_p, c_int, c_void_p, c_void_p, c_void_p, c_void_p, c_void_p, c_int, c_void_p, c_int,
                                    c_void_p, c_void_p, c_void_p, c_float, c_void_p, c_void_p, c_int, c_long, c_int, c_int, c_void_p]),
     "cdseg_attn_tail_rr2": (c_int, [c_void_p, c_int, c_void_p, c_void_p, c_void_p, c_void_p, c_float, c_void_p, c_void_p,
diff --git a/cdsegnet_amd/build.py b/cdsegnet_amd/build.py
--- a/cdsegnet_amd/build.py
+++ b/cdsegnet_amd/build.py
@@ -8,7 +8,7 @@
 LIB_F16 = os.path.join(HERE, "libcdseg_hip_f16.so")
 VARIANTS = [(LIB, "_build", []), (LIB_F16, "_build_f16", ["-DCDSEG_LP_F16"])]
 SOURCES = ["serialize.hip", "plan.hip", "gemm.hip", "elementwise.hip", "attention.hip", "attention_drop.hip", "conv.hip", "stem.hip", "mlp.hip", "blockrr.hip", "deep.hip", "pool.hip", "runtime.hip", "testtime.hip", "traintime.hip", "train.hip", "trainblock.hip", "loss.hip", "norm.hip", "fusion.hip", "skip.hip", "optim.hip", "prof.hip", "route.hip", "abi.hip"]
-HEADERS = ["common.h", "curves.h", "prof.h", "route.h", "deep.h", "wgrad_partition.h", "workspace.h", "attn_train.h", os.path.join("..", "..", "include", "cdseg.h")]
+HEADERS = ["common.h", "curves.h", "prof.h", "route.h", "deep.h", "wgrad_partition.h", "workspace.h", "attn_train.h", "tail_outputs.h", os.path.join("..", "..", "include", "cdseg.h")]
 ARCH = "gfx950"
 
 
diff --git a/cdsegnet_amd/csrc/blockrr.hip b/cdsegnet_amd/csrc/blockrr.hip
--- a/cdsegnet_amd/csrc/blockrr.hip
+++ b/cdsegnet_amd/csrc/blockrr.hip
@@ -5,6 +5,7 @@
 #include "common.h"
 #include "deep.h"
 #include "route.h"
+#include "tail_outputs.h"
 
 namespace {
 
@@ -183,9 +184,12 @@
   const bf16_t* o; const uint4* wimg; const float* bp; const float* ln_g; const float* ln_b; const float* b1;
   const float* b2; float* x; bf16_t* xc;
   long n; int ldo, ldx, ldxc; float eps;
+  int store_x;
+  float* logits; const float* head_w; const float* head_b; const int32_t* out_idx; int classes, ld_logits;
 };
 
-template <int C>
+static_assert(tail_rr_lds_bytes(32) == RRCfg<32>::TAIL_W + RRCfg<32>::TAIL_P && tail_rr_lds_bytes(64) == RRCfg<64>::TAIL_W + RRCfg<64>::TAIL_P);
+template <int C, bool LOGITS>
 __global__ __launch_bounds__(RR_WAVES * 64, 4) void tail_rr_kernel(TailRR p) {
   using K = RRCfg<C>;
   constexpr int KS = K::KS, CT = K::CT, Q = K::Q, HU = 4 * C / 32;
@@ -201,6 +205,11 @@
       pr[c] = p.bp[c]; pr[C + c] = p.ln_g[c]; pr[2 * C + c] = p.ln_b[c]; pr[3 * C + c] = p.b2[c];
     }
     for (int c = tid; c < 4 * C; c += RR_WAVES * 64) pr[4 * C + c] = p.b1[c];
+    if constexpr (LOGITS) {
+      float* hw = pr + 8 * C;
+      for (int u = tid; u < p.classes * C; u += RR_WAVES * 64) hw[(u / C) * (C + 4) + (u % C)] = p.head_w[u];
+      for (int k = tid; k < p.classes; k += RR_WAVES * 64) hw[p.classes * (C + 4) + k] = p.head_b ? p.head_b[k] : 0.f;
+    }
   }
   __syncthreads();
   const uint4* Wp = reinterpret_cast<const uint4*>(smem);
@@ -280,12 +289,38 @@
         for (int t = 0; t < CT; ++t)
           acc2[t] = mfma_16x16x32_bf16(__builtin_bit_cast(bf16x8_t, w2[t]), Hf, acc2[t]);
       }
-      if (ok) {
+      if constexpr (LOGITS) {
 #pragma unroll
         for (int t = 0; t < CT; ++t) {
           const f32x4_t b2 = *reinterpret_cast<const f32x4_t*>(pr + 3 * C + q * Q + 4 * t);
           acc2[t] = acc2[t] + (b2 + x1[t]);
-          *reinterpret_cast<f32x4_t*>(p.x + row * p.ldx + q * Q + 4 * t) = acc2[t];
+        }
+        const float* hw = pr + 8 * C;
+        const float* hb = hw + p.classes * (C + 4);
+        const long orow = ok ? (p.out_idx ? (long)p.out_idx[row] : row) : -1;
+#pragma unroll 1
+        for (int ot = 0; 16 * ot < p.classes; ++ot) {
+          const int ka = min(16 * ot + j, p.classes - 1);
+          const int kd = min(16 * ot + 4 * q, p.classes - 4);
+          f32x4_t lg = *reinterpret_cast<const f32x4_t*>(hb + kd);
+#pragma unroll
+          for (int t = 0; t < CT; ++t) {
+            const f32x4_t a = *reinterpret_cast<const f32x4_t*>(hw + ka * (C + 4) + q * Q + 4 * t);
+#pragma unroll
+            for (int r = 0; r < 4; ++r) lg = __builtin_amdgcn_mfma_f32_16x16x4f32(a[r], acc2[t][r], lg, 0, 0, 0);
+          }
+          if (orow >= 0 && 16 * ot + 4 * q < p.classes)
+            *reinterpret_cast<f32x4_t*>(p.logits + orow * p.ld_logits + 16 * ot + 4 * q) = lg;
+        }
+      } else if (ok) {
+#pragma unroll
+        for (int t = 0; t < CT; ++t) {
+          const f32x4_t b2 = *reinterpret_cast<const f32x4_t*>(pr + 3 * C + q * Q + 4 * t);
+          acc2[t] = acc2[t] + (b2 + x1[t]);
+        }
+        if (p.store_x) {
+#pragma unroll
+          for (int t = 0; t < CT; ++t) *reinterpret_cast<f32x4_t*>(p.x + row * p.ldx + q * Q + 4 * t) = acc2[t];
         }
         if (p.xc) {
 #pragma unroll
@@ -373,9 +408,18 @@
   return CDSEG_OK;
 }
 
-extern "C" int cdseg_attn_tail_rr(const void* o, int ldo, const void* tail_img, const float* bp, const float* ln_g,
-                                  const float* ln_b, float eps, const float* b1, const float* b2, float* x, int ldx,
-                                  void* xc, int ldxc, long n, int channels, void* stream) {
+extern "C" int cdseg_attn_tail_rr_ex(const void* o, int ldo, const void* tail_img, const float* bp, const float* ln_g,
+                                     const float* ln_b, float eps, const float* b1, const float* b2, float* x, int ldx,
+                                     void* xc, int ldxc, long n, int channels, int flags, float* logits, int ld_logits,
+                                     const float* head_w, const float* head_b, const int32_t* out_idx, int num_classes,
+                                     void* stream) {
+  if (flags & ~CDSEG_BLOCK_X_DEAD) return CDSEG_ERR_ARG;
+  const bool want_logits = logits || head_w || head_b || out_idx || num_classes || ld_logits;
+  if (want_logits) {
+    if (channels != 32 && channels != 64) return CDSEG_ERR_UNSUPPORTED;
+    const int rc = tail_logits_status(channels, num_classes, ld_logits, logits, head_w, out_idx);
+    if (rc != CDSEG_OK) return rc;
+  }
   if (n <= 0) return CDSEG_OK;
   if (!o || !tail_img || !bp || !ln_g || !ln_b || !b1 || !b2 || !x) return CDSEG_ERR_ARG;
   if (channels != 32 && channels != 64 && !deep_supported(channels)) return CDSEG_ERR_UNSUPPORTED;
@@ -387,24 +431,47 @@
   TailRR p;
   p.o = (const bf16_t*)o; p.wimg = (const uint4*)tail_img; p.bp = bp; p.ln_g = ln_g; p.ln_b = ln_b; p.b1 = b1; p.b2 = b2;
   p.x = x; p.xc = (bf16_t*)xc; p.n = n; p.ldo = ldo; p.ldx = ldx; p.ldxc = ldxc; p.eps = eps;
+  p.store_x = (flags & CDSEG_BLOCK_X_DEAD) ? 0 : 1;
+  p.logits = logits; p.head_w = head_w; p.head_b = head_b; p.out_idx = out_idx; p.classes = num_classes; p.ld_logits = ld_logits;
+  const int aux = want_logits ? (CDSEG_TAIL_AUX_LOGITS | CDSEG_TAIL_AUX_X_SKIPPED)
+                              : (p.store_x ? 0 : CDSEG_TAIL_AUX_X_SKIPPED);
   hipStream_t s = (hipStream_t)stream;
-  if (channels == 32) {
+  if (want_logits) {
+    const int lds = tail_rr_lds_bytes(64) + tail_logits_lds_bytes(64, num_classes);
+    static std::atomic<bool> attr_done{false};
+    if (!attr_done) {
+      if (hipFuncSetAttribute((const void*)tail_rr_kernel<64, true>, hipFuncAttributeMaxDynamicSharedMemorySize,
+                              TAIL_RR_LDS_TWO_PER_CU) != hipSuccess)
+        return CDSEG_ERR_LAUNCH;
+      attr_done = true;
+    }
+    cdseg_route_rec(CDSEG_RK_TAIL_RR_64, 0, 0, 1, 0, 0, 0, aux);
+    hipLaunchKernelGGL((tail_rr_kernel<64, true>), dim3(rr_grid(n, lds)), dim3(RR_WAVES * 64), lds, s, p);
+  } else if (channels == 32) {
     constexpr int lds = RRCfg<32>::TAIL_W + RRCfg<32>::TAIL_P;
-    cdseg_route_rec(CDSEG_RK_TAIL_RR_32, 0, 0, 1, 0, 0, 0, 0);
-    hipLaunchKernelGGL(tail_rr_kernel<32>, dim3(rr_grid(n, lds)), dim3(RR_WAVES * 64), lds, s, p);
+    cdseg_route_rec(CDSEG_RK_TAIL_RR_32, 0, 0, 1, 0, 0, 0, aux);
+    hipLaunchKernelGGL((tail_rr_kernel<32, false>), dim3(rr_grid(n, lds)), dim3(RR_WAVES * 64), lds, s, p);
   } else {
     constexpr int lds = RRCfg<64>::TAIL_W + RRCfg<64>::TAIL_P;
     static std::atomic<bool> attr_done{false};
     if (!attr_done) {
-      if (hipFuncSetAttribute((const void*)tail_rr_kernel<64>, hipFuncAttributeMaxDynamicSharedMemorySize, lds) != hipSuccess)
+      if (hipFuncSetAttribute((const void*)tail_rr_kernel<64, false>, hipFuncAttributeMaxDynamicSharedMemorySize, lds) !=
+          hipSuccess)
         return CDSEG_ERR_LAUNCH;
       attr_done = true;
     }
-    cdseg_route_rec(CDSEG_RK_TAIL_RR_64, 0, 0, 1, 0, 0, 0, 0);
-    hipLaunchKernelGGL(tail_rr_kernel<64>, dim3(rr_grid(n, lds)), dim3(RR_WAVES * 64), lds, s, p);
+    cdseg_route_rec(CDSEG_RK_TAIL_RR_64, 0, 0, 1, 0, 0, 0, aux);
+    hipLaunchKernelGGL((tail_rr_kernel<64, false>), dim3(rr_grid(n, lds)), dim3(RR_WAVES * 64), lds, s, p);
   }
   CDSEG_CHECK_LAUNCH();
   return CDSEG_OK;
+}
+
+extern "C" int cdseg_attn_tail_rr(const void* o, int ldo, const void* tail_img, const float* bp, const float* ln_g,
+                                  const float* ln_b, float eps, const float* b1, const float* b2, float* x, int ldx,
+                                  void* xc, int ldxc, long n, int channels, void* stream) {
+  return cdseg_attn_tail_rr_ex(o, ldo, tail_img, bp, ln_g, ln_b, eps, b1, b2, x, ldx, xc, ldxc, n, channels, 0, nullptr, 0,
+                               nullptr, nullptr, nullptr, 0, stream);
 }
 
 extern "C" int cdseg_cpe_head_rr2(const void* y, int ldy, const void* head_img, const float* bl, const float* lnp_g,
diff --git a/cdsegnet_amd/csrc/runtime.hip b/cdsegnet_amd/csrc/runtime.hip
--- a/cdsegnet_amd/csrc/runtime.hip
+++ b/cdsegnet_amd/csrc/runtime.hip
@@ -4,6 +4,7 @@
 
 #include "common.h"
 #include "deep.h"
+#include "tail_outputs.h"
 #include "workspace.h"
 
 namespace {
@@ -83,6 +84,14 @@
   if (!io->scratch || io->scratch_bytes < L.total) return CDSEG_ERR_WORKSPACE;
   const bool fuse = C <= FUSE_LN_MAX_C;
   int rc;
+  static const bool fused_tail = cdseg_knob("CDSEG_FUSED_TAIL", 1) != 0 && cdseg_knob("CDSEG_FUSED_MLP", 1) != 0;
+  const bool tail_rr = fused_tail && T == CDSEG_BF16 && (C == 32 || C == 64) && d->hidden == 4 * C && d->tail_img;
+  const bool want_logits = io->logits || io->head_w || io->head_b || io->out_idx || io->num_classes || io->ld_logits;
+  if (io->flags & ~CDSEG_BLOCK_X_DEAD) return CDSEG_ERR_ARG;
+  if (want_logits) {
+    if (!tail_rr || io->sat_counter) return CDSEG_ERR_UNSUPPORTED;
+    if ((rc = tail_logits_status(C, io->num_classes, io->ld_logits, io->logits, io->head_w, io->out_idx)) != CDSEG_OK) return rc;
+  }
   int attn_flags = d->attn_flags & CDSEG_ATTN_Q_PRESCALED;
 
   const bool conv_fits = n * 27 * 4 < (1l << 31) && n * (long)C * 2 < (1l << 31) - 65536;
@@ -175,7 +184,6 @@
                                  d->dtype, attn_flags, stream)) != CDSEG_OK)
       return rc;
   }
-  static const bool fused_tail = cdseg_knob("CDSEG_FUSED_TAIL", 1) != 0 && cdseg_knob("CDSEG_FUSED_MLP", 1) != 0;
   if (pingpong) {
     void* xc = (const void*)io->xc_out != (const void*)io->x ? io->xc_out : nullptr;
     return cdseg_attn_tail_rr2(L.o, C, d->tail_img, (const float*)d->proj_b, (const float*)d->norm2_g, (const float*)d->norm2_b,
@@ -190,9 +198,10 @@
   if (fused_tail && T == CDSEG_BF16 && (C == 32 || C == 64) && d->hidden == 4 * C) {
     void* xc = (const void*)io->xc_out != (const void*)io->x ? io->xc_out : nullptr;
     if (d->tail_img)
-      return cdseg_attn_tail_rr(L.o, C, d->tail_img, (const float*)d->proj_b, (const float*)d->norm2_g,
-                                (const float*)d->norm2_b, d->ln_eps, (const float*)d->fc1_b, (const float*)d->fc2_b,
-                                (float*)io->x, C, xc, C, n, C, stream);
+      return cdseg_attn_tail_rr_ex(L.o, C, d->tail_img, (const float*)d->proj_b, (const float*)d->norm2_g,
+                                   (const float*)d->norm2_b, d->ln_eps, (const float*)d->fc1_b, (const float*)d->fc2_b,
+                                   (float*)io->x, C, xc, C, n, C, xc ? (io->flags & CDSEG_BLOCK_X_DEAD) : 0, io->logits,
+                                   io->ld_logits, io->head_w, io->head_b, io->out_idx, io->num_classes, stream);
     return cdseg_attn_tail_fused(L.o, C, d->proj_w, (const float*)d->proj_b, (const float*)d->norm2_g,
                                  (const float*)d->norm2_b, d->ln_eps, d->fc1_w, (const float*)d->fc1_b, d->fc2_w,
                                  (const float*)d->fc2_b, (float*)io->x, C, xc, C, n, C, T, stream);
diff --git a/cdsegnet_amd/csrc/tail_outputs.h b/cdsegnet_amd/csrc/tail_outputs.h
--- /dev/null
+++ b/cdsegnet_amd/csrc/tail_outputs.h
@@ -0,0 +1,18 @@
+#pragma once
+#include <cstdint>
+
+#include "../../include/cdseg.h"
+
+constexpr int tail_rr_lds_bytes(int C) { return 9 * C * C * 2 + 8 * C * 4; }
+constexpr int tail_logits_lds_bytes(int C, int classes) { return classes * (C + 4) * 4 + classes * 4; }
+constexpr int TAIL_RR_LDS_TWO_PER_CU = 80 * 1024;
+
+inline int tail_logits_status(int C, int classes, int ld_logits, const void* logits, const void* head_w, const void* out_idx) {
+  if (!logits || !head_w || classes <= 0) return CDSEG_ERR_ARG;
+  if (C != 64) return CDSEG_ERR_UNSUPPORTED;
+  if (classes % 4 || classes > 32) return CDSEG_ERR_UNSUPPORTED;
+  if (tail_rr_lds_bytes(C) + tail_logits_lds_bytes(C, classes) > TAIL_RR_LDS_TWO_PER_CU) return CDSEG_ERR_UNSUPPORTED;
+  if (ld_logits < classes || (ld_logits & 3) || ((uintptr_t)logits & 15)) return CDSEG_ERR_UNSUPPORTED;
+  if (((uintptr_t)head_w | (uintptr_t)out_idx) & 3) return CDSEG_ERR_ARG;
+  return CDSEG_OK;
+}
diff --git a/cdsegnet_amd/engine.py b/cdsegnet_amd/engine.py
--- a/cdsegnet_amd/engine.py
+++ b/cdsegnet_amd/engine.py
@@ -12,6 +12,21 @@
 
 CURVES = ("z", "z-trans", "hilbert", "hilbert-trans")
 POOL_LONG_MIN_ROWS = 960_000
+LOGITS_IN_TAIL_MIN_ROWS = 65_536
+LOGITS_IN_TAIL_MAX_CLASSES = {64: 20}
+
+
+def block_outputs_read(part, stage, num_stages, last_block, precision, branch="n", has_head=True, diagnostic=False,
+                       native=True):
+    if not last_block or diagnostic or not native or precision in ("fp32", "fp32x3"):
+        return True, True
+    if part == "enc":
+        return (True, True) if stage == num_stages - 1 else (False, True)
+    if stage > 0:
+        return False, True
+    if branch != "n" or not has_head:
+        return True, True
+    return (True, False) if precision.endswith("+head") else (False, True)
 
 
 def _pooling_depth(stride):
@@ -326,6 +341,8 @@
         self.rng_offset = 0
         self._rng_seed = None
         self.use_native_blocks = True
+        self.dead_outputs = True
+        self.logits_in_tail = True
         self.fold_attn_scale = True
         self.speculate_depth = True
         self._depth_hint = {}
@@ -1101,7 +1118,7 @@
             st.xc = self._buf(n, c, self.T)
             ops.gemm(u, w[pre_fc + "2.w"], st.x, bias=w[pre_fc + "2.b"], res=st.x, out2=st.xc)
 
-    def run_block(self, st, mod, pre, tbias=None):
+    def run_block(self, st, mod, pre, tbias=None, live=(True, True), head=None):
         w, lv = self.w, st.level
         n, c = st.x.shape
         if self.native_blocks:
@@ -1112,18 +1129,29 @@
             self.attn_bytes += 4.0 * n * c * st.xc.element_size()
             self._count_conv(n, c, st.xc.element_size())
             desc = self.block_desc[pre]
-            xc_out = st.x if self.T == torch.float32 else self._buf(n, c, self.T)
+            x_live, xc_live = live
+            if self.T == torch.float32 or self._sat is not None:
+                x_live, xc_live, head = True, True, None
             sb = self._scratch_bytes.get((pre, n))
             if sb is None:
                 if len(self._scratch_bytes) > 4096:
                     self._scratch_bytes.clear()
                 sb = self._scratch_bytes[(pre, n)] = ops.block_scratch_bytes(desc, n)
+            if head is not None and ops.block_forward(desc, n, st.x, st.xc, st.x, tbias, lv.nbr(3, True), gidx, widx,
+                                                      patch_start, patch_start.numel() - 1, max_len, self.scratch(sb),
+                                                      logits=head[0], head_w=head[1], head_b=head[2], out_idx=head[3]):
+                st.x = st.xc = None
+                return True
+            xc_out = st.x if (self.T == torch.float32 or not xc_live) else self._buf(n, c, self.T)
+            flags = ops.BLOCK_X_DEAD if not x_live and xc_out is not st.x else 0
             ops.block_forward(desc, n, st.x, st.xc, xc_out, tbias, lv.nbr(3, True), gidx, widx, patch_start,
-                              patch_start.numel() - 1, max_len, self.scratch(sb), sat_counter=self._sat)
+                              patch_start.numel() - 1, max_len, self.scratch(sb), sat_counter=self._sat, flags=flags)
             if self._sat is not None:
                 self.saturation_checked += n * c * (5 if xc_out is not st.x else 4)
             st.xc = xc_out
-            return
+            if flags:
+                st.x = None
+            return False
         qkv = self._buf(n, 3 * c, self.T)
         aflags = ops.ATTN_Q_PRESCALED if self.q_prescaled else 0
         deep_rr = ((pre + ".head_img") in w and (pre + ".tail_img") in w and not ops.cpe_head_fused_ok(st.xc)
@@ -1690,29 +1718,42 @@
         n_curves = shuffled(next(pi))
         tb = self._t_bias(t) if cond else {}
 
+        own_hi = frozenset(("n_head", "c_head")) if self.precision.endswith("+head") else frozenset()
+        prune = self.dead_outputs and self.hi == own_hi and self._sat is None
+        has_head = "n_head.w" in w
+
+        def live(e, part, branch, s, names, name):
+            if not prune:
+                return True, True
+            return block_outputs_read(part, s, getattr(bb, f"{branch}_num_stages"), name == names[-1], self.precision,
+                                      branch=branch, has_head=has_head, diagnostic=self._sat is not None,
+                                      native=e.native_blocks)
+
         def enc_stage(st, branch, s, cum, perm):
             enc = getattr(getattr(bb, f"_{branch}_enc"), f"enc{s}")
             e = self._eng(f"{branch}_enc{s}")
             e._fit(st)
             if s > 0:
                 st = e.run_pooling(plan, st, f"{branch}_enc{s}.down", cum[s], perm)
-            for name, mod in enc._modules.items():
-                if name.startswith("block"):
-                    key = f"{branch}_enc{s}.{name}"
-                    e.run_block(st, mod, key, tb.get(key))
+            names = [name for name in enc._modules if name.startswith("block")]
+            for name in names:
+                key = f"{branch}_enc{s}.{name}"
+                e.run_block(st, enc._modules[name], key, tb.get(key), live=live(e, "enc", branch, s, names, name))
             return st
 
-        def dec_stage(st, branch, s):
+        def dec_stage(st, branch, s, head=None):
             dec = getattr(getattr(bb, f"_{branch}_dec"), f"dec{s}")
             e = self._eng(f"{branch}_dec{s}")
             e._fit(st)
             e._fit(st.parent)
             st = e.run_unpooling(plan, st, f"{branch}_dec{s}.up", dec.up)
-            for name, mod in dec._modules.items():
-                if name.startswith("block"):
-                    key = f"{branch}_dec{s}.{name}"
-                    e.run_block(st, mod, key, tb.get(key))
-            return st
+            names = [name for name in dec._modules if name.startswith("block")]
+            done = False
+            for name in names:
+                key = f"{branch}_dec{s}.{name}"
+                done = e.run_block(st, dec._modules[name], key, tb.get(key), live=live(e, "dec", branch, s, names, name),
+                                   head=head if name == names[-1] else None)
+            return st, bool(done)
 
         if cond:
             p_c1, p_n1, p_n2, p_c2, p_n3, p_n4 = (next(pi) for _ in range(6))
@@ -1769,17 +1810,29 @@
         if cond and want_c:
             self._msi_count("c_decoders")
             for s in reversed(range(bb.c_num_stages - 1)):
-                cst = dec_stage(cst, "c", s)
+                cst, _ = dec_stage(cst, "c", s)
             e = self._eng("c_head")
             e._fit(cst, exact=True)
             c_out = torch.empty((n, w["c_head.w"].shape[0]), dtype=torch.float32, device=dev)
             ops.gemm(cst.xc, e.w["c_head.w"], c_out, bias=e.w["c_head.b"])
+        head, logits, done = None, None, False
+        if (prune and has_head and self.logits_in_tail and self.T != torch.float32 and "n_head" in self.hi
+                and self.native_blocks and bb.n_num_stages > 1 and n >= LOGITS_IN_TAIL_MIN_ROWS
+                and getattr(bb._n_dec.dec0.up, "skip_filter", None) is None):
+            e = self._eng("n_head")
+            classes, last_c = e.w["n_head.w"].shape
+            if classes % 4 == 0 and classes <= LOGITS_IN_TAIL_MAX_CLASSES.get(last_c, 0):
+                logits = torch.empty((n, classes), dtype=torch.float32, device=dev)
+                head = (logits, e.w["n_head.w"], e.w["n_head.b"], plan.perm0)
         for s in reversed(range(bb.n_num_stages - 1)):
-            nst = dec_stage(nst, "n", s)
-        if "n_head.w" in w:
+            nst, done = dec_stage(nst, "n", s, head if s == 0 else None)
+        if done:
+            pass
+        elif "n_head.w" in w:
             e = self._eng("n_head")
             e._fit(nst, exact=True)
-            logits = torch.empty((n, w["n_head.w"].shape[0]), dtype=torch.float32, device=dev)
+            if logits is None:
+                logits = torch.empty((n, w["n_head.w"].shape[0]), dtype=torch.float32, device=dev)
             ops.gemm(nst.xc, e.w["n_head.w"], logits, bias=e.w["n_head.b"], out_idx=plan.perm0)
         else:
             logits = torch.empty((n, nst.x.shape[1]), dtype=torch.float32, device=dev)
diff --git a/cdsegnet_amd/ops.py b/cdsegnet_amd/ops.py
--- a/cdsegnet_amd/ops.py
+++ b/cdsegnet_amd/ops.py
@@ -736,6 +736,19 @@
     return x
 
 
+def attn_tail_rr_ex(o, tail_img, bp, ln_g, ln_b, b1, b2, x, xc=None, eps=1e-5, flags=0, logits=None, head_w=None,
+                    head_b=None, out_idx=None, num_classes=None, ld_logits=None):
+    if logits is not None:
+        num_classes = head_w.shape[0] if num_classes is None else num_classes
+        ld_logits = logits.stride(0) if ld_logits is None else ld_logits
+    check(_lib.load().cdseg_attn_tail_rr_ex(_ptr(o), o.stride(0), _ptr(tail_img), _ptr(bp), _ptr(ln_g), _ptr(ln_b), float(eps),
+                                            _ptr(b1), _ptr(b2), _ptr(x), x.stride(0), _ptr(xc),
+                                            xc.stride(0) if xc is not None else 0, o.shape[0], o.shape[1], int(flags),
+                                            _ptr(logits), int(ld_logits or 0), _ptr(head_w), _ptr(head_b), _ptr(out_idx),
+                                            int(num_classes or 0), _stream()), "attn_tail_rr_ex")
+    return x
+
+
 def _dp(t):
     return None if t is None else t.data_ptr()
 
@@ -771,7 +784,7 @@
 
 
 def block_forward(desc, n, x, xc_in, xc_out, tbias, nbr, gidx, widx, patch_start, num_patches, max_len, scratch,
-                  sat_counter=None):
+                  sat_counter=None, flags=0, logits=None, head_w=None, head_b=None, out_idx=None):
     if _TLS.block_io is None:
         io = _lib.BlockIO()
         _TLS.block_io = (io, ctypes.byref(io))
@@ -782,7 +795,22 @@
     io.num_patches, io.max_len = int(num_patches), int(max_len)
     io.scratch, io.scratch_bytes = scratch.data_ptr(), scratch.numel()
     io.sat_counter = sat_counter.data_ptr() if sat_counter is not None else None
-    check(_lib.load().cdseg_block_forward(desc[1], ref, _stream()), "block_forward")
+    io.flags = int(flags)
+    if logits is None:
+        io.logits = io.head_w = io.head_b = io.out_idx = None
+        io.num_classes = io.ld_logits = 0
+    else:
+        if logits.dtype != torch.float32 or head_w.dtype != torch.float32 or not head_w.is_contiguous() or (
+                head_w.shape[1] != x.shape[1]) or (
+                head_b is not None and head_b.dtype != torch.float32) or (out_idx is not None and out_idx.dtype != torch.int32):
+            raise _lib.CdsegError("block_forward: logits / head_w / head_b are fp32 (head_w contiguous), out_idx int32")
+        io.logits, io.head_w, io.head_b, io.out_idx = logits.data_ptr(), head_w.data_ptr(), _dp(head_b), _dp(out_idx)
+        io.num_classes, io.ld_logits = int(head_w.shape[0]), int(logits.stride(0))
+    status = _lib.load().cdseg_block_forward(desc[1], ref, _stream())
+    if status == _UNSUPPORTED and logits is not None:
+        return False
+    check(status, "block_forward")
+    return True
 
 
 def stem5_ok(cout, dtype):
@@ -853,6 +881,9 @@
 
 
 ATTN_Q_PRESCALED, ATTN_V_BF16 = 1, 2
+BLOCK_X_DEAD = 1
+TAIL_AUX_X_SKIPPED, TAIL_AUX_LOGITS = 1, 2
+_UNSUPPORTED = -4
 
 
 def attention(q, k, v, q_gidx, kv_gidx, widx, patch_start, num_heads, max_len, scale, out, work=0.0, flags=0):
diff --git a/include/cdseg.h b/include/cdseg.h
--- a/include/cdseg.h
+++ b/include/cdseg.h
@@ -286,6 +286,13 @@
 int cdseg_attn_tail_rr(const void* o, int ldo, const void* tail_img, const float* bp, const float* ln_g, const float* ln_b,
                        float eps, const float* b1, const float* b2, float* x, int ldx, void* xc, int ldxc, long n,
                        int channels, void* stream);
+#define CDSEG_BLOCK_X_DEAD 1
+#define CDSEG_TAIL_AUX_X_SKIPPED 1
+#define CDSEG_TAIL_AUX_LOGITS 2
+int cdseg_attn_tail_rr_ex(const void* o, int ldo, const void* tail_img, const float* bp, const float* ln_g, const float* ln_b,
+                          float eps, const float* b1, const float* b2, float* x, int ldx, void* xc, int ldxc, long n,
+                          int channels, int flags, float* logits, int ld_logits, const float* head_w, const float* head_b,
+                          const int32_t* out_idx, int num_classes, void* stream);
 int cdseg_cpe_head_rr2(const void* y, int ldy, const void* head_img, const float* bl, const float* lnp_g, const float* lnp_b,
                        const float* x, int ldx, float* x_out, int ldx_out, const float* colbias, const float* ln1_g,
                        const float* ln1_b, float eps, const float* bqkv, void* qkv, int ldqkv, long n, int channels,
@@ -340,6 +347,13 @@
   void* scratch;
   size_t scratch_bytes;
   unsigned long long* sat_counter;
+  int flags;
+  float* logits;
+  const float* head_w;
+  const float* head_b;
+  const int32_t* out_idx;
+  int num_classes;
+  int ld_logits;
 } cdseg_block_io;
 
 size_t cdseg_block_scratch_bytes(const cdseg_block_desc* desc, long n);
```
